# thiviyanT/torch-rgcn

Measured on AMD Instinct MI355X. Metric: edges/s/GPU (fwd+bwd) 2-layer RGCN, 1M nodes/10M edges/50 rels, h=16, higher is better.
Workload: dtype f32; 1 GPU; S1: N=1000000 nodes, E=10000000 base triples, R0=50 relations (layer R=101), M=21000000 messages/layer, hidden=16, 2 NC layers (horizontal, vertical), fwd+bwd, learnable X

## Files before the change

include/rgcn_hip.h:

```cpp
#ifndef RGCN_HIP_H
#define RGCN_HIP_H

#include <stdint.h>

#ifdef __cplusplus
extern "C" {
#endif

#define RGCN_API __attribute__((visibility("default")))

#define RGCN_OK 0
#define RGCN_EINVAL 1
#define RGCN_ENOMEM 2
#define RGCN_ERANGE 3
#define RGCN_EHIP 4
#define RGCN_EUNSUPPORTED 5

#define RGCN_CHUNK 16

RGCN_API const char *rgcn_version(void);
RGCN_API const char *rgcn_last_error(void);
RGCN_API const char *rgcn_csrc_sha(void);
RGCN_API int rgcn_poison_lds(void *stream);
RGCN_API int rgcn_set_option(const char *name, int32_t value);
RGCN_API int rgcn_get_option(const char *name, int32_t *value);


RGCN_API int rgcn_add_inverse_and_self_host(const int64_t *triples, int64_t E, int64_t N, int64_t R0,
                                            int64_t *out);

RGCN_API int rgcn_lp_augment_host(const int64_t *triples, int64_t E, int64_t N, int64_t R0,
                                  const uint8_t *keep, int64_t *out, int64_t *M_out, int64_t *n_self);

RGCN_API int rgcn_edge_norm_host(const int64_t *triples_plus, int64_t M, int64_t N, int64_t R, int vertical,
                                 int64_t n_swap, int64_t i_tail, float *val);

RGCN_API int rgcn_plan_count_host(const int32_t *dst, const int32_t *rel, int64_t M, int64_t n_dst, int32_t R,
                                  int32_t tile_rows, int32_t max_item_chunks, int64_t *m_pad,
                                  int64_t *n_chunks, int64_t *n_tiles, int64_t *n_items);
RGCN_API int rgcn_plan_fill_host(const int32_t *dst, const int32_t *src, const int32_t *rel, const float *val,
                                 int64_t M, int64_t n_dst, int64_t n_src, int32_t R, int32_t tile_rows,
                                 int32_t max_item_chunks, int32_t *p_src, int32_t *p_dst, float *p_val,
                                 int32_t *p_perm, int32_t *chunk_rel, int32_t *tile_ptr, int32_t *items,
                                 int32_t *run_ptr, int32_t *p_pack);

#define RGCN_U_SHARED 1
#define RGCN_U_FIRST 2
RGCN_API int rgcn_plan_units_host(const int32_t *tile_ptr, int64_t n_tiles, int32_t max_unit_chunks,
                                  int32_t *units, int64_t *n_units, int64_t *n_split);

RGCN_API int rgcn_synthetic_triples_host(int64_t N, int64_t R0, int64_t E, uint64_t seed, int64_t *out);

RGCN_API int rgcn_edge_neighborhood_host(const int64_t *triples, int64_t E, int64_t N, int64_t sample_size,
                                         uint64_t seed, int64_t *picked_edges);

RGCN_API int rgcn_dev_split_triples(const int64_t *triples_plus, int64_t M, int64_t N, int32_t R, int32_t *s,
                                    int32_t *p, int32_t *o, int32_t *err_flag, void *stream);
RGCN_API int rgcn_dev_lp_expand(const int64_t *triples, int64_t E, int64_t N, int32_t R0, const uint8_t *keep,
                                int32_t *s, int32_t *p, int32_t *o, uint8_t *alive, int32_t *err_flag, void *stream);
RGCN_API int rgcn_dev_edge_norm(const int32_t *s, const int32_t *p, const int32_t *o, const uint8_t *alive, int64_t M,
                                int64_t N, int32_t R, int vertical, int64_t n_swap, int32_t *table, float *val,
                                void *stream);
RGCN_API int rgcn_dev_plan_count(const int32_t *dst, const int32_t *rel, const uint8_t *alive, int64_t M, int64_t n_dst,
                                 int32_t R, int32_t tile_rows, int32_t *cells, int32_t *bucket_cnt,
                                 int32_t *bucket_base, int32_t *scan_tmp, int32_t *cells_tmp, void *stream);
RGCN_API int rgcn_dev_plan_fill(const int32_t *dst, const int32_t *src, const int32_t *rel, const float *val,
                                const uint8_t *alive, int64_t M, int64_t n_dst, int64_t n_src, int32_t R,
                                int32_t tile_rows, int32_t *cells, const int32_t *bucket_cnt,
                                const int32_t *bucket_base, int32_t *p_src, int32_t *p_dst, float *p_val,
                                int32_t *p_pack, int32_t *chunk_rel, int32_t *tile_ptr, int32_t *run_ptr,
                                const int32_t *aux, int32_t *p_aux, int32_t *msg_slot, int64_t n_chunks,
                                void *stream);
RGCN_API int rgcn_dev_csr_pair(const int32_t *a, const int32_t *b, const int32_t *rel, const float *val, const uint8_t *alive,
                               int64_t M, int64_t N, int32_t *rowbuf, int32_t *scan_tmp, int32_t *e_other, int32_t *e_rel,
                               float *e_val, void *stream);
RGCN_API int rgcn_dev_plan_finish_nosync(const int32_t *bucket_base, int64_t n_tiles, int32_t R, int64_t m_pad_ub,
                                         int32_t *p_src, int32_t *p_dst, float *p_val, int32_t *p_pack, int32_t *p_aux,
                                         const int32_t *tile_ptr, int32_t *units, int32_t *items, int64_t n_items_ub,
                                         int32_t max_item_chunks, void *stream);

RGCN_API int rgcn_basis_aggregate_f32(const float *X, const float *comps, float *out, const int32_t *rowptr,
                                      const int32_t *p_src, const int32_t *p_rel, const float *p_val,
                                      int64_t n_rows, int32_t R, int32_t B, int32_t d, int32_t n_b_in,
                                      void *stream);
RGCN_API int rgcn_basis_dcomps_f32(const float *X, const float *D, float *dcomps, const int32_t *p_src,
                                   const int32_t *p_dst, const float *p_val, const int32_t *chunk_rel,
                                   const int32_t *items, int64_t n_items, int32_t R, int32_t B, int32_t d,
                                   int32_t n_copies, void *stream);
RGCN_API int rgcn_basis_dcomps_csr_supported(int32_t R, int32_t B, int32_t d);
RGCN_API int rgcn_basis_dcomps_csr_f32(const float *X, const float *D, float *dcomps, const int32_t *rowptr, const int32_t *p_src,
                                       const int32_t *p_rel, const float *p_val, int64_t n_rows, int32_t R, int32_t B, int32_t d,
                                       void *workspace, void *stream);
RGCN_API int64_t rgcn_basis_sum_workspace_bytes(int32_t R, int32_t B);


#define RGCN_F_RELU 1
#define RGCN_F_WPACKED 2
RGCN_API int rgcn_spmm_f32(const float *X, const float *W, const float *bias, float *out, const int32_t *p_src,
                           const int32_t *p_dst, const float *p_val, const int32_t *p_pack,
                           const int32_t *chunk_rel, const int32_t *units, int64_t n_units, int64_t n_split,
                           int32_t tile_rows, int64_t n_dst, int64_t n_src, int32_t R, int32_t d_in,
                           int32_t d_out, int32_t flags, void *stream);

RGCN_API int rgcn_pack_w16_f32(const float *W, float *Wp, int32_t R, void *stream);
RGCN_API int rgcn_pack_w_blocks_f32(const float *W, float *Wp, int32_t R, int32_t d_in, int32_t d_out, void *stream);

RGCN_API int rgcn_spmm_scatter_f32(const float *X, const float *Wp, float *Y, const int32_t *p_src,
                                   const float *p_val, const int32_t *p_pos, const int32_t *chunk_rel,
                                   const int32_t *items, int64_t n_items, int32_t d, void *stream);
RGCN_API int rgcn_segment_sum_f32(const float *Y, const int32_t *rowptr, const float *bias, float *out,
                                  int64_t n_rows, int32_t d, int32_t flags, void *stream);
RGCN_API int rgcn_segment_gather_sum_f32(const float *Y, const int32_t *perm, const int32_t *rowptr, const float *bias,
                                         float *out, int64_t n_rows, int32_t d, int32_t flags, void *stream);
RGCN_API int rgcn_segment_gather_sum_units_f32(const float *Y, const int32_t *perm, const int32_t *units, int64_t n_units,
                                               int64_t n_split, const float *bias, float *out, int64_t n_rows, int32_t d,
                                               int32_t flags, void *stream);

RGCN_API int rgcn_wgrad_f32(const float *X, const float *G, float *dW, const int32_t *p_src,
                            const int32_t *p_dst, const float *p_val, const int32_t *chunk_rel,
                            const int32_t *items, int64_t n_items, int64_t n_dst, int64_t n_src, int32_t R,
                            int32_t d_in, int32_t d_out, void *stream);

RGCN_API int rgcn_wgrad_tiled_f32(const float *X, const float *G, float *dW, const int32_t *p_src,
                                  const int32_t *p_dst, const float *p_val, const int32_t *chunk_rel,
                                  const int32_t *run_ptr, int64_t n_tiles, int32_t tile_rows, int64_t n_dst,
                                  int64_t n_src, int32_t R, int32_t d_in, int32_t d_out,
                                  int32_t tiles_per_item, void *stream);

#define RGCN_F_DW_ATOMIC 4
#define RGCN_F_TRANSPOSE_W 8
#define RGCN_F_DIAG4 16
#define RGCN_F_PARTIAL 32
#define RGCN_F_ACCUMULATE 64
RGCN_API int64_t rgcn_bwd_fused_scratch_floats(int64_t n_tiles, int32_t R);
RGCN_API int64_t rgcn_bwd_lean_slot_bytes(int64_t n_chunks);
RGCN_API int rgcn_bwd_lean_prepare_f32(const int32_t *p_pack, const int32_t *chunk_rel, int64_t n_chunks, void *slots, int32_t *hdr,
                                       void *stream);
RGCN_API int rgcn_bwd_lean_prepare_unpacked_f32(const int32_t *p_src, const int32_t *p_dst, const float *p_val, int32_t tile_rows,
                                                const int32_t *chunk_rel, int64_t n_chunks, void *slots, int32_t *hdr, void *stream);
RGCN_API int rgcn_bwd_lean_supported(int32_t tile_rows);
RGCN_API int rgcn_bwd_lean_f32(const float *G, const float *X, const float *Wt_packed, float *dX, float *dW, float *scratch,
                               const void *slots, const int32_t *hdr, const int32_t *run_ptr, int64_t n_tiles, int32_t tile_rows,
                               int64_t n_dst, int32_t R, int32_t flags, void *stream);
RGCN_API int32_t rgcn_bwd_blk_max_rows(int32_t R, int32_t flags);
RGCN_API int rgcn_bwd_blk_supported(int32_t tile_rows, int32_t R, int32_t flags);
RGCN_API int64_t rgcn_bwd_blk_rec_bytes(int64_t n_chunks);
RGCN_API int rgcn_bwd_blk_prepare_f32(const int32_t *p_pack, const int32_t *p_src, const int32_t *p_dst, const float *p_val,
                                      int32_t tile_rows, const int32_t *chunk_rel, int64_t n_chunks, void *rec, void *stream);
RGCN_API int rgcn_bwd_blk_f32(const float *G, const float *X, const float *Wt_packed, float *dX, float *dW, const void *rec,
                              const int32_t *run_ptr, int64_t n_tiles, int32_t tile_rows, int64_t n_dst, int32_t R, int32_t flags,
                              float *dbias, int64_t n_src, const int32_t *units, int64_t n_units, int64_t n_split, void *stream);
RGCN_API int32_t rgcn_bwd_own_waves(void);
RGCN_API int32_t rgcn_bwd_own_units(void);
RGCN_API int32_t rgcn_bwd_own_max_rows(void);
RGCN_API int rgcn_bwd_own_f32(const float *G, const float *X, const float *Wt_packed, float *dX, float *dW, const void *rec,
                              const int32_t *own_ptr, const int32_t *unit_rel, int64_t n_tiles, int32_t tile_rows, int64_t n_dst,
                              int32_t R, int32_t flags, float *dbias, int64_t n_src, void *stream);
RGCN_API int rgcn_bwd_own_bf16(const uint16_t *G, const uint16_t *X, const float *Wt_packed, uint16_t *dX, float *dW, const void *rec,
                               const int32_t *own_ptr, const int32_t *unit_rel, int64_t n_tiles, int32_t tile_rows, int64_t n_dst,
                               int32_t R, int32_t flags, float *dbias, int64_t n_src, void *stream);
RGCN_API int64_t rgcn_softwin_tmp_bytes(int64_t n);
RGCN_API int rgcn_softwin_order(const int32_t *dst, const int32_t *src, const int32_t *rel, const uint8_t *alive, int64_t M, int64_t n_dst,
                                int64_t n_src, int32_t R, int32_t tile_rows, uint64_t *keys, uint64_t *keys_sorted, int32_t *order,
                                int32_t *order_sorted, int32_t *bucket_cnt, int32_t *bucket_base, int32_t *bucket_first, void *tmp,
                                int64_t tmp_bytes, void *stream);
RGCN_API int rgcn_softwin_fill(const int32_t *dst, const int32_t *src, const float *val, const uint64_t *keys_sorted, const int32_t *order_sorted,
                               int64_t n_live, int64_t n_dst, int64_t n_src, int32_t R, int32_t tile_rows, const int32_t *bucket_base,
                               const int32_t *bucket_first, int64_t m_pad, const int32_t *parts, const int32_t *unit_base,
                               const int32_t *unit_owner, const int32_t *unit_local, int32_t own_waves, int32_t *s_src, int32_t *s_dst, float *s_val,
                               uint64_t *ckeys, uint64_t *ckeys_sorted, int32_t *cidx, int32_t *cidx_sorted, int32_t *crel, int32_t *group_cnt,
                               int32_t *p_src, int32_t *p_dst, float *p_val, int32_t *chunk_rel, int32_t *group_ptr, void *tmp, int64_t tmp_bytes,
                               void *stream);
RGCN_API int32_t rgcn_spmm_blk_max_rows(void);
RGCN_API int rgcn_spmm_blk_f32(const float *X, const float *W_packed, const float *bias, float *out, const void *rec,
                               const int32_t *run_ptr, int64_t n_tiles, int32_t tile_rows, int64_t n_dst, int32_t R, int32_t flags,
                               const int32_t *units, int64_t n_units, int64_t n_split, void *stream);
RGCN_API int rgcn_spmm_blk_bf16(const uint16_t *X, const float *W_packed, const float *bias, uint16_t *out, float *scratch, const void *rec,
                                const int32_t *run_ptr, int64_t n_tiles, int32_t tile_rows, int64_t n_dst, int64_t n_src, int32_t R,
                                int32_t flags, const int32_t *units, int64_t n_units, int64_t n_split, void *stream);
RGCN_API int rgcn_spmm_bf16(const uint16_t *X, const float *W_packed, const float *bias, uint16_t *out, float *scratch,
                            const int32_t *p_pack, const int32_t *chunk_rel, const int32_t *units, int64_t n_units, int64_t n_split,
                            int32_t tile_rows, int64_t n_dst, int64_t n_src, int32_t d_in, int32_t d_out, int32_t flags, void *stream);
RGCN_API int rgcn_wgrad_bf16(const uint16_t *X, const uint16_t *G, float *dW, const int32_t *p_src, const int32_t *p_dst,
                             const float *p_val, const int32_t *chunk_rel, const int32_t *items, int64_t n_items, int32_t R,
                             int32_t d_in, int32_t d_out, void *stream);
RGCN_API int rgcn_colsum_bf16(const uint16_t *G, float *db, float *scratch, int64_t n, int32_t d, void *stream);
RGCN_API int rgcn_bwd_scatter_dw_f32(const float *G, const float *X, const float *Wt_packed, float *Y, float *dW,
                                     const int32_t *p_src, const int32_t *p_dst, const float *p_val,
                                     const int32_t *chunk_rel, const int32_t *items, int64_t n_items, int32_t R, int32_t d,
                                     int32_t flags, void *stream);
RGCN_API int rgcn_pack_w16t_f32(const float *W, float *Wp, int32_t R, void *stream);
RGCN_API int rgcn_pack_w16_pair_f32(const float *W, float *Wp, float *Wtp, int32_t R, void *stream);

RGCN_API int rgcn_featureless_fwd_f32(const float *table, const float *bias, float *out, const int32_t *p_src,
                                      const int32_t *p_dst, const float *p_val, const int32_t *chunk_rel,
                                      const int32_t *units, int64_t n_units, int64_t n_split, int32_t tile_rows,
                                      int64_t n_dst, int64_t n_src, int32_t R, int32_t d_out, void *stream);

RGCN_API int rgcn_spmm_csr_d16_supported(int32_t R);
RGCN_API int rgcn_spmm_csr_d16_f32(const float *X, const float *W, const float *bias, float *out, const int32_t *units, int64_t n_units,
                                   int64_t n_split, const int32_t *e_src, const int32_t *e_rel, const float *e_val, int64_t n_rows,
                                   int32_t R, int32_t flags, void *stream);
RGCN_API int rgcn_block_supported(int32_t bi, int32_t bo);
RGCN_API int rgcn_block_spmm_f32(const float *X, const float *blocks, const float *bias, float *out, const int32_t *units,
                                 const int32_t *rowptr, int64_t n_units, int64_t n_split, const int32_t *e_src,
                                 const int32_t *e_rel, const float *e_val, int64_t n_rows, int32_t n_rel_blocks, int32_t nb,
                                 int32_t bi, int32_t bo, int32_t flags, void *stream);

RGCN_API int rgcn_block_wgrad_f32(const float *X, const float *G, float *dblocks, const int32_t *p_src, const int32_t *p_dst,
                                  const float *p_val, const int32_t *chunk_rel, const int32_t *items, int64_t n_items,
                                  int32_t n_rel_blocks, int32_t nb, int32_t bi, int32_t bo, void *stream);

RGCN_API int rgcn_diag_spmm_f32(const float *X, const float *w, const float *bias, float *out, const int32_t *units,
                                int64_t n_units, int64_t n_split, const int32_t *e_src, const int32_t *e_rel,
                                const float *e_val, int64_t n_rows, int32_t R, int32_t d, void *stream);

RGCN_API int rgcn_diag_wgrad_f32(const float *X, const float *G, float *dw, const int32_t *p_src, const int32_t *p_dst,
                                 const float *p_val, const int32_t *chunk_rel, const int32_t *items, int64_t n_items,
                                 int32_t R, int32_t d, void *stream);

RGCN_API int rgcn_featureless_wgrad_f32(const float *G, float *dtable, const int32_t *p_src,
                                        const int32_t *p_dst, const float *p_val, const int32_t *chunk_rel,
                                        int64_t n_chunks, int64_t n_dst, int64_t n_src, int32_t R,
                                        int32_t d_out, void *stream);
RGCN_API int rgcn_featureless_csr_fwd_f32(const float *table, const float *bias, float *out, const int32_t *units, int64_t n_units,
                                          int64_t n_split, const int32_t *e_src, const int32_t *e_rel, const float *e_val,
                                          int64_t n_rows, int64_t n_src, int32_t R, int32_t d, int32_t relu, void *stream);
RGCN_API int rgcn_featureless_csr_wgrad_f32(const float *G, float *dtable, const int32_t *rowptr, const int32_t *e_src,
                                            const int32_t *e_rel, const float *e_val, int64_t n_entries, int64_t n_rows, int64_t n_src,
                                            int32_t R, int32_t d, void *stream);

RGCN_API int64_t rgcn_colsum_scratch_floats(int64_t n, int32_t d);
RGCN_API int rgcn_colsum_f32(const float *G, float *db, float *scratch, int64_t n, int32_t d, void *stream);

RGCN_API int rgcn_fbasis_fwd_f32(const float *bases, const float *comps, float *Y, const int32_t *e_rel,
                                 const float *e_val, const int32_t *units, int64_t n_units, int64_t n_nodes,
                                 int32_t R, int32_t B, int32_t d, int32_t basis_major, void *stream);
RGCN_API int rgcn_fbasis_bwd_f32(const float *bases, const float *comps, const float *G, float *dbases, float *T,
                                 const int32_t *e_dst, const int32_t *e_rel, const float *e_val,
                                 const int32_t *units, int64_t n_units, int64_t n_split, int64_t n_nodes, int32_t R,
                                 int32_t B, int32_t d, int32_t basis_major, void *stream);
RGCN_API int rgcn_fbasis_small_supported(int32_t R, int32_t B, int32_t d);
RGCN_API int rgcn_fbasis_small_bwd_f32(const float *G, const float *table, const float *comps, float *dbases, float *dcomps,
                                       const int32_t *rowptr, const int32_t *p_src, const int32_t *p_rel, const float *p_val,
                                       int64_t n_rows, int32_t R, int32_t B, int32_t d, int32_t basis_major, void *stream);
RGCN_API int rgcn_fbasis_bwd_dc_supported(int32_t R, int32_t B, int32_t d);
RGCN_API int rgcn_fbasis_bwd_dc_f32(const float *bases, const float *comps, const float *G, float *dbases, float *dcomps,
                                    const int32_t *e_dst, const int32_t *e_rel, const float *e_val, const int32_t *units,
                                    int64_t n_units, int64_t n_split, int64_t n_nodes, int32_t R, int32_t B, int32_t d,
                                    int32_t basis_major, void *stream);
RGCN_API int rgcn_gather_rows_sum_f32(const float *Y, const int32_t *perm, const int32_t *units, int64_t n_units,
                                      int64_t n_split, const float *bias, float *out, int64_t n_rows, int32_t w,
                                      int32_t relu, void *stream);

RGCN_API int rgcn_fbasis_tile_supported(int32_t R, int32_t B, int32_t d, int64_t n_nodes);
RGCN_API int rgcn_fbasis_tile_ystride(int32_t d);
RGCN_API int rgcn_fbasis_tile_fwd_f32(const float *bases, const float *comps, float *Y, const int32_t *rowptr, const int32_t *e_rel,
                                      const float *e_val, int64_t n_messages, int64_t n_nodes, int32_t R, int32_t B, int32_t d,
                                      int32_t mode, void *stream);
RGCN_API int rgcn_gather_rows_sum4_f32(const float *Y, int32_t ys, const int32_t *perm, const int32_t *units, int64_t n_units,
                                       int64_t n_split, const float *bias, float *out, int64_t n_rows, int32_t w, int32_t out_stride,
                                       int32_t relu, void *stream);
RGCN_API int rgcn_fbasis_tile_bwd_f32(const float *bases, const float *comps, const float *G, int32_t g_stride, float *dbases, float *dcomps,
                                      const int32_t *rowptr, const int32_t *e_dst, const int32_t *e_rel, const float *e_val,
                                      int64_t n_messages, int64_t n_nodes, int32_t R, int32_t B, int32_t d, int32_t mode, void *stream);
RGCN_API int rgcn_fbasis_tile_bwd_fused_gn(int32_t R, int32_t B, int32_t d, int64_t n_nodes);

RGCN_API int rgcn_fbasis_tile_fwd_bf16(const uint16_t *bases, const float *comps, float *Y, const int32_t *rowptr, const int32_t *e_rel,
                                       const float *e_val, int64_t n_messages, int64_t n_nodes, int32_t R, int32_t B, int32_t d,
                                       int32_t mode, void *stream);
RGCN_API int rgcn_gather_rows_sum4_bf16(const float *Y, int32_t ys, const int32_t *perm, const int32_t *units, int64_t n_units,
                                        int64_t n_split, const float *bias, uint16_t *out, float *scratch, int64_t n_rows, int32_t w,
                                        int32_t out_stride, int32_t relu, void *stream);
RGCN_API int rgcn_fbasis_tile_bwd_bf16(const uint16_t *bases, const float *comps, const uint16_t *G, int32_t g_stride, uint16_t *dbases,
                                       float *dcomps, const int32_t *rowptr, const int32_t *e_dst, const int32_t *e_rel, const float *e_val,
                                       int64_t n_messages, int64_t n_nodes, int32_t R, int32_t B, int32_t d, int32_t mode, void *stream);

RGCN_API int rgcn_ce_head_f32(const float *logits, const int32_t *row_label, const int32_t *lab_rows, float *loss, float *dlogits,
                              int64_t N, int32_t C, int32_t ld, int32_t n_lab, void *stream);

RGCN_API int rgcn_bce_head_workspace_bytes(void);
RGCN_API int rgcn_bce_head_f32(const float *scores, const float *labels, float *loss, float *dscores, void *workspace, int64_t T,
                               void *stream);

RGCN_API int rgcn_resize3_f32(const float *src, float *dst, int64_t A, int32_t B, int32_t C, int32_t Bd, int32_t Cd, const float *src1,
                              float *dst1, int32_t n1, int32_t n1d, void *stream);

#define RGCN_G_TRANS_A 1
#define RGCN_G_TRANS_B 2
RGCN_API int64_t rgcn_gemm_scratch_floats(int64_t M, int64_t N, int64_t K, int32_t split_k);
RGCN_API int rgcn_gemm_f32(const float *A, const float *B, const float *bias, float *C, float *scratch, int64_t M,
                           int64_t N, int64_t K, int64_t lda, int64_t ldb, int64_t ldc, int32_t flags, int32_t split_k,
                           void *stream);

RGCN_API int rgcn_rel_rows_f32(const float *Xs, const float *W, float *Y, const int32_t *p_src, const float *p_val,
                               const int32_t *chunk_rel, const int32_t *items, int64_t n_items, int32_t R, int32_t d_in,
                               int32_t d_out, void *stream);
RGCN_API int rgcn_rel_wgrad_f32(const float *Xs, const float *G, float *dW, const int32_t *p_src, const int32_t *p_dst,
                                const float *p_val, const int32_t *chunk_rel, const int32_t *items, int64_t n_items,
                                int32_t R, int32_t d_in, int32_t d_out, void *stream);
RGCN_API int rgcn_segment_gather_sum_wide_f32(const float *Y, const int32_t *perm, const int32_t *rowptr, const float *bias,
                                              float *out, int64_t n_rows, int32_t d, int32_t flags, void *stream);

RGCN_API int rgcn_distmult_fwd_f32(const int64_t *triples, int64_t T, const float *nodes, const float *rel,
                                   const float *sbias, const float *pbias, const float *obias, float *scores,
                                   int64_t n_nodes, int32_t n_rel, int32_t d, int32_t *err_flag, int32_t *rank_counts,
                                   int32_t *ranks, void *stream);
RGCN_API int rgcn_distmult_csr_place(const int64_t *triples, int64_t T, int64_t N, int32_t n_rel, const int32_t *ranks,
                                     int32_t *rank_counts, int32_t *scan_tmp, const float *gs, int32_t *entries, void *stream);
RGCN_API int rgcn_distmult_bwd_f32(const int64_t *triples, int64_t T, const float *nodes, const float *rel,
                                   const float *gs, float *dnodes, float *drel, float *dsbias, float *dpbias,
                                   float *dobias, int64_t n_nodes, int32_t n_rel, int32_t d, void *stream);
RGCN_API int rgcn_distmult_bwd_nodes_f32(const int32_t *rowptr_s, const int32_t *rowptr_o, const int32_t *entries, const float *nodes,
                                         const float *rel, float *dnodes, int64_t n_nodes, int32_t d, void *stream);

RGCN_API int rgcn_distmult_bwd_all_supported(int32_t n_rel, int32_t d);
RGCN_API int rgcn_distmult_bwd_all_f32(const int32_t *rowptr_s, const int32_t *rowptr_o, const int32_t *entries, const float *nodes,
                                       const float *rel, float *dnodes, float *drel, float *dsbias, float *dpbias, float *dobias,
                                       int64_t n_nodes, int32_t n_rel, int32_t d, void *stream);

RGCN_API int rgcn_distmult_score_all_f32(const int64_t *batch, int64_t Q, int32_t head, const float *nodes,
                                         const float *rel, const float *sbias, const float *pbias,
                                         const float *obias, float *qvec, float *qbias, float *scores,
                                         int64_t n_nodes, int32_t n_rel, int32_t d, void *stream);
RGCN_API int rgcn_rank_filter_f32(float *scores, int64_t Q, int64_t n_nodes, const int32_t *filt_q,
                                  const int32_t *filt_n, int64_t F, void *stream);
RGCN_API int rgcn_rank_count_f32(const float *scores, const int64_t *batch, int64_t Q, int32_t head,
                                 int64_t n_nodes, int64_t *greater, int64_t *ties, void *stream);

#ifdef __cplusplus
}
#endif
#endif
```

torch-rgcn_amd/csrc/rgcn_bwd_blk.hip:

```cpp
#include <stdlib.h>
#include <string.h>

#include <algorithm>

#include "rgcn_device.h"

namespace {

constexpr int BLK_NW = 16;
#ifndef RGCN_BLK_FWD_U
#define RGCN_BLK_FWD_U 1
#endif
constexpr int BLK_FWD_U = RGCN_BLK_FWD_U;
#ifndef RGCN_BLK_FWD_NW
#define RGCN_BLK_FWD_NW 16
#endif
constexpr int BLK_FWD_NW = RGCN_BLK_FWD_NW;
constexpr int BLK_FWD_TQS = 16 / BLK_FWD_NW;
#ifndef RGCN_BLK_BWD_U
#define RGCN_BLK_BWD_U 3
#endif
constexpr int BLK_BWD_U = RGCN_BLK_BWD_U;
constexpr int BLK_REC = 176;
constexpr int BLK_REC_ROWS = 128;
// ... 63 lines not shown
  extern __shared__ __attribute__((aligned(16))) char lds[];
  const int tid = threadIdx.x;
  const int wave = __builtin_amdgcn_readfirstlane(tid >> 6), lane = tid & 63;
  const unsigned xt_off = (unsigned)tile_rows * 128u;
  const unsigned xs_off = (unsigned)tile_rows * 192u;
  float4 *dxz = reinterpret_cast<float4 *>(lds);
  const double2 *dxd2 = reinterpret_cast<const double2 *>(lds);
  float4 *xt4 = reinterpret_cast<float4 *>(lds + xt_off);
  float *xs = reinterpret_cast<float *>(lds + xs_off) + wave * BW_SCR2;
  constexpr int DWR = DIAG4 ? 64 : 256;
  float *dwl = reinterpret_cast<float *>(lds + xs_off) + NW * BW_SCR2;
  int *ctl = reinterpret_cast<int *>(dwl + (size_t)R * DWR);
  int *dirty = ctl + 4;

  auto unit_of = [&](int u) {
    if (units) return units[u];
    return int4{u, run_ptr[(size_t)u * (R + 1)], run_ptr[(size_t)u * (R + 1) + R], 0};
  };
  int un = blockIdx.x;
  int4 unit = unit_of(un);
  int t = __builtin_amdgcn_readfirstlane(unit.x);
  int row0 = t * tile_rows;
  int nrows = min(tile_rows, n_dst - row0);
  int c0 = __builtin_amdgcn_readfirstlane(unit.y);
  int c1 = __builtin_amdgcn_readfirstlane(unit.z);
  int shared = __builtin_amdgcn_readfirstlane(unit.w) & RGCN_U_SHARED;
  int nq = (c1 - c0 + U - 1) / U;
  auto static_quads = [](int n) { return max(1, min(4, (3 * n) / (4 * BLK_NW))); };
  int ns = static_quads(nq);
  float4 gs = make_float4(0.f, 0.f, 0.f, 0.f);
  const long long g_n4 = dbias ? (long long)n_src * 4 : 0, g_step = (long long)gridDim.x * NT;
  long long g_i = (long long)blockIdx.x * NT + tid;
  {
#pragma unroll
    for (int q = 0; q < TQ; ++q) {
      const int idx = tid + q * NT;
      if (idx < tile_rows * 4) {
        float4 x0 = make_float4(0.f, 0.f, 0.f, 0.f);
        if (idx < nrows * 4) x0 = reinterpret_cast<const float4 *>(X + (size_t)row0 * 16)[idx];
        xt4[idx] = x0;
      }
    }
    for (int i = tid; i < tile_rows * 8; i += NT) dxz[i] = make_float4(0.f, 0.f, 0.f, 0.f);
    for (int i = tid; i < R * (DWR / 4); i += NT) reinterpret_cast<float4 *>(dwl)[i] = make_float4(0.f, 0.f, 0.f, 0.f);
    for (int i = tid; i < R + 4; i += NT) ctl[i] = i == 0 ? NW * (ns + 1) : 0;
  }
  __syncthreads();

  const int m = lane & 15, k = lane >> 4;
  const unsigned kofs = (unsigned)k << 4;
  const unsigned dx_lane = (unsigned)m * 8u;
  const unsigned xrd = xt_off + (unsigned)m * 4u;
  float *xs_wr = xs + m * 16 + 4 * ((k + (m >> 2)) & 3);
  const float *xs_rd = xs + (4 * k) * 16 + 4 * (((m >> 2) + k) & 3) + (m & 3);
  const unsigned slot_lane = (unsigned)m * 8u;
  const unsigned rows_lane = (unsigned)BLK_REC_ROWS + (unsigned)k * 8u;
  const unsigned w_lane = (unsigned)lane * 16u;

  f32x4 hold = f32x4{0.f, 0.f, 0.f, 0.f};
  int cur_r = -1;
  auto flush_hold = [&]() {
    if (cur_r >= 0 && (ABL & 4)) {
      *reinterpret_cast<f32x4 *>(dwl + (size_t)cur_r * 256 + lane * 4) = hold;
    } else if (cur_r >= 0) {
      if (DIAG4) {
        if ((m >> 2) == k) lds_cas_add4(dwl + (size_t)cur_r * 64 + (4 * k + (m & 3)) * 4, hold);
      } else {
        lds_cas_add4(dwl + (size_t)cur_r * 256 + lane * 4, hold);
      }
      if (lane == 0) lds_st(dirty + cur_r, 1);
    }
  };

  uint2 sl_n[U], rw_n[U];
  int hd_n[U];
  auto request_idx = [&](int c, int last) {
#pragma unroll
    for (int j = 0; j < U; ++j) {
      const int cc = min(c + j, last);
      const char *r = rec + (size_t)cc * BLK_REC;
      sl_n[j] = *reinterpret_cast<const uint2 *>(r + slot_lane);
      rw_n[j] = *reinterpret_cast<const uint2 *>(r + rows_lane);
      hd_n[j] = *reinterpret_cast<const int *>(r + BLK_REC_HDR);
    }
  };
  int q_cur = wave * ns, q_nxt = 1 < ns ? wave * ns + 1 : NW * ns + wave, q_pos = 2;
  if (q_cur < nq) request_idx(c0 + q_cur * U, c1 - 1);
  BLK_DBG(const long long dbg_t0 = BLK_T(); long long dbg_wait = 0; long long dbg_epi = 0; long long dbg_ta = 0; long long dbg_tb = 0;)

  for (;;) {
    const int last = c1 - 1;
    while (q_cur < nq) {
      const int c = c0 + q_cur * U;
      unsigned w0_[U];
      uint2 rw_[U];
      float v_[U];
      int hd_[U];
      float4 g_[U], w_[U];
#pragma unroll
      for (int j = 0; j < U; ++j) {
        w0_[j] = sl_n[j].x;
        rw_[j] = rw_n[j];
        v_[j] = (c + j <= last) ? __builtin_bit_cast(float, sl_n[j].y) : 0.f;
        hd_[j] = __builtin_amdgcn_readfirstlane(hd_n[j]);
      }
#pragma unroll
      for (int j = 0; j < U; ++j) asm volatile("" : "+v"(w0_[j]), "+v"(v_[j]));
      __builtin_amdgcn_sched_barrier(0);
#pragma unroll
      for (int j = 0; j < U; ++j) {
        const unsigned og = w0_[j] | kofs;
        g_[j] = *reinterpret_cast<const float4 *>(reinterpret_cast<const char *>(G) + og);
        w_[j] = *reinterpret_cast<const float4 *>(reinterpret_cast<const char *>(Wtp) + (size_t)hd_[j] * 1024 + w_lane);
      }
      __builtin_amdgcn_sched_barrier(0);
      if (q_nxt < nq) request_idx(c0 + q_nxt * U, last);
      int q_nn = q_pos < ns ? wave * ns + q_pos : NW * ns + wave;
      if (q_pos > ns && lane == 0) q_nn = __hip_atomic_fetch_add(ctl, 1, __ATOMIC_RELAXED, __HIP_MEMORY_SCOPE_WORKGROUP);
      ++q_pos;
      __builtin_amdgcn_sched_barrier(0);
      if (ABL & 16) {
#pragma unroll
        for (int j = 0; j < U; ++j) asm volatile("" :: "v"(g_[j].x), "v"(g_[j].y), "v"(g_[j].z), "v"(g_[j].w), "v"(w_[j].x), "v"(w_[j].w), "v"(rw_[j].x), "v"(rw_[j].y), "v"(v_[j]));
        q_cur = q_nxt;
        q_nxt = __builtin_amdgcn_readfirstlane(q_nn);
        continue;
      }
      f32x4 sc[U], acc[U];
#pragma unroll
      for (int j = 0; j < U; ++j) {
        sc[j] = f32x4{g_[j].x * v_[j], g_[j].y * v_[j], g_[j].z * v_[j], g_[j].w * v_[j]};
        acc[j] = f32x4{0.f, 0.f, 0.f, 0.f};
      }
#pragma unroll
      for (int j = 0; j < U; ++j) acc[j] = __builtin_amdgcn_mfma_f32_16x16x4f32(sc[j][0], w_[j].x, acc[j], 0, 0, 0);
#pragma unroll
      for (int j = 0; j < U; ++j) acc[j] = __builtin_amdgcn_mfma_f32_16x16x4f32(sc[j][1], w_[j].y, acc[j], 0, 0, 0);
#pragma unroll
      for (int j = 0; j < U; ++j) acc[j] = __builtin_amdgcn_mfma_f32_16x16x4f32(sc[j][2], w_[j].z, acc[j], 0, 0, 0);
#pragma unroll
      for (int j = 0; j < U; ++j) acc[j] = __builtin_amdgcn_mfma_f32_16x16x4f32(sc[j][3], w_[j].w, acc[j], 0, 0, 0);
      unsigned ro[U][4];
#pragma unroll
      for (int j = 0; j < U; ++j) {
        ro[j][0] = rw_[j].x & 0xFFFFu;
        ro[j][1] = rw_[j].x >> 16;
        ro[j][2] = rw_[j].y & 0xFFFFu;
        ro[j][3] = rw_[j].y >> 16;
      }
      if (!(ABL & 2)) {
        f32x4 aw[U];
#pragma unroll
        for (int h = 0; h < U; h += 2) {
          float bv[2][4], av[2][4];
#pragma unroll
          for (int jj = 0; jj < 2; ++jj) {
            const int j = h + jj;
            if (j >= U) break;
            if (ABL & 32) {
#pragma unroll
              for (int t4 = 0; t4 < 4; ++t4) { bv[jj][t4] = sc[j][t4]; av[jj][t4] = __builtin_bit_cast(float, ro[j][t4]); }
            } else {
            asm volatile("" ::: "memory");
            *reinterpret_cast<f32x4 *>(xs_wr) = sc[j];
            asm volatile("" ::: "memory");
#pragma unroll
            for (int t4 = 0; t4 < 4; ++t4) bv[jj][t4] = xs_rd[16 * t4];
#pragma unroll
            for (int t4 = 0; t4 < 4; ++t4) av[jj][t4] = *reinterpret_cast<const float *>(lds + (xrd + ro[j][t4]));
            asm volatile("" ::: "memory");
            }
          }
#pragma unroll
          for (int jj = 0; jj < 2; ++jj)
            if (h + jj < U) aw[h + jj] = f32x4{0.f, 0.f, 0.f, 0.f};
#pragma unroll
          for (int t4 = 0; t4 < 4; ++t4)
#pragma unroll
            for (int jj = 0; jj < 2; ++jj)
              if (h + jj < U) aw[h + jj] = __builtin_amdgcn_mfma_f32_16x16x4f32(av[jj][t4], bv[jj][t4], aw[h + jj], 0, 0, 0);
        }
#pragma unroll
        for (int j = 0; j < U; ++j) {
          if (c + j > last) break;
          const int rj = hd_[j];
          if (rj != cur_r) {
            flush_hold();
            cur_r = rj;
            hold = aw[j];
          } else {
            hold += aw[j];
          }
        }
      }
      if (ABL & 8) {
#pragma unroll
        for (int j = 0; j < U; ++j) asm volatile("" :: "v"(acc[j][0]), "v"(acc[j][1]), "v"(acc[j][2]), "v"(acc[j][3]));
      } else {
#pragma unroll
        for (int j = 0; j < U; ++j)
#pragma unroll
          for (int e = 0; e < 4; ++e)
            __hip_atomic_fetch_add(static_cast<double *>(__builtin_assume_aligned(lds + (dx_lane + 2u * ro[j][e]), 8)), (double)acc[j][e], __ATOMIC_RELAXED,
                                   __HIP_MEMORY_SCOPE_WORKGROUP);
      }
      __builtin_amdgcn_sched_barrier(0);
      q_cur = q_nxt;
      q_nxt = __builtin_amdgcn_readfirstlane(q_nn);
    }
    flush_hold();
    cur_r = -1;
    const int unn = un + (int)gridDim.x;
    float4 xn[TQ];
#pragma unroll
    for (int q = 0; q < TQ; ++q) xn[q] = make_float4(0.f, 0.f, 0.f, 0.f);
    int c0n = 0, c1n = 0, nqn = 0, row0n = 0, nrn = 0, tn = 0, sharedn = 0, nsn = 1;
    if (unn < n_units) {
      const int4 unx = unit_of(unn);
      tn = __builtin_amdgcn_readfirstlane(unx.x);
      row0n = tn * tile_rows;
      nrn = min(tile_rows, n_dst - row0n);
      c0n = __builtin_amdgcn_readfirstlane(unx.y);
      c1n = __builtin_amdgcn_readfirstlane(unx.z);
      sharedn = __builtin_amdgcn_readfirstlane(unx.w) & RGCN_U_SHARED;
      nqn = (c1n - c0n + U - 1) / U;
      nsn = static_quads(nqn);
#pragma unroll
      for (int q = 0; q < TQ; ++q)
        if (tid + q * NT < nrn * 4) xn[q] = reinterpret_cast<const float4 *>(X + (size_t)row0n * 16)[tid + q * NT];
      if (wave * nsn < nqn) request_idx(c0n + wave * nsn * U, c1n - 1);
    }
    float4 gn = make_float4(0.f, 0.f, 0.f, 0.f);
    if (g_i < g_n4) gn = reinterpret_cast<const float4 *>(G)[g_i];
    g_i += g_step;
    BLK_DBG(dbg_ta = BLK_T();)
    lds_barrier();
    BLK_DBG(dbg_tb = BLK_T(); dbg_wait += dbg_tb - dbg_ta;)
    gs.x += gn.x; gs.y += gn.y; gs.z += gn.z; gs.w += gn.w;
#pragma unroll
    for (int q = 0; q < TQ; ++q) asm volatile("" : "+v"(xn[q].x), "+v"(xn[q].y), "+v"(xn[q].z), "+v"(xn[q].w));
#pragma unroll
    for (int q = 0; q < TQ; ++q) {
      const int idx = tid + q * NT;
      if (idx < nrows * 4) {
        const double2 d0 = dxd2[2 * idx], d1 = dxd2[2 * idx + 1];
        float4 a = make_float4((float)d0.x, (float)d0.y, (float)d1.x, (float)d1.y);
        if (RELU) {
          const float4 x = xt4[idx];
          a.x = x.x > 0.f ? a.x : 0.f; a.y = x.y > 0.f ? a.y : 0.f; a.z = x.z > 0.f ? a.z : 0.f; a.w = x.w > 0.f ? a.w : 0.f;
        }
        float4 *o = reinterpret_cast<float4 *>(dX + (size_t)row0 * 16) + idx;
        if (shared) {
          atomicAdd(&o->x, a.x); atomicAdd(&o->y, a.y); atomicAdd(&o->z, a.z); atomicAdd(&o->w, a.w);
        } else {
          *o = a;
        }
      }
    }
    if (unn >= n_units) break;
#pragma unroll
    for (int q = 0; q < TQ; ++q) {
      const int idx = tid + q * NT;
      if (idx < tile_rows * 4) {
        dxz[2 * idx] = make_float4(0.f, 0.f, 0.f, 0.f);
        dxz[2 * idx + 1] = make_float4(0.f, 0.f, 0.f, 0.f);
        xt4[idx] = xn[q];
      }
    }
    if (tid == 0) ctl[0] = NW * (nsn + 1);
    lds_barrier();
    BLK_DBG(dbg_epi += BLK_T() - dbg_tb;)
    un = unn; t = tn; row0 = row0n; nrows = nrn; c0 = c0n; c1 = c1n; nq = nqn; shared = sharedn;
    ns = nsn;
    q_cur = wave * ns; q_nxt = 1 < ns ? wave * ns + 1 : NW * ns + wave; q_pos = 2;
  }
  BLK_DBG(if (lane == 0 && blockIdx.x < 256) { unsigned long long *d = rgcn_blk_dbg + 4 * (blockIdx.x * BLK_NW + wave); d[0] += (unsigned long long)dbg_wait;
                                               d[1] += (unsigned long long)dbg_epi; d[2] += (unsigned long long)(BLK_T() - dbg_t0); d[3] += 1ull; })
  if (dbias) {
    for (; g_i < g_n4; g_i += g_step) {
      const float4 gn = reinterpret_cast<const float4 *>(G)[g_i];
      gs.x += gn.x; gs.y += gn.y; gs.z += gn.z; gs.w += gn.w;
    }
#pragma unroll
    for (int sft = 4; sft < 64; sft <<= 1) {
      gs.x += __shfl_xor(gs.x, sft); gs.y += __shfl_xor(gs.y, sft); gs.z += __shfl_xor(gs.z, sft); gs.w += __shfl_xor(gs.w, sft);
    }
    if (lane < 4) *reinterpret_cast<float4 *>(xs + 4 * lane) = gs;
    __syncthreads();
    if (tid < 16) {
      float a = 0.f;
      const float *all = reinterpret_cast<const float *>(lds + xs_off);
      for (int i = 0; i < NW; ++i) a += all[i * BW_SCR2 + tid];
      atomicAdd(dbias + tid, a);
    }
  }
  for (int i = tid; i < R * DWR; i += NT) {
    const int r = i / DWR, e = i & 3;
    const int ln = DIAG4 ? 16 * ((i >> 4) & 3) + 4 * ((i >> 4) & 3) + ((i >> 2) & 3) : (i >> 2) & 63;
    if (lds_ld(dirty + r)) atomicAdd(dWout + (size_t)r * 256 + (4 * (ln >> 4) + e) * 16 + (ln & 15), dwl[i]);
  }
}


template <bool RELU, int TQ, int BF = 0>
__global__ __launch_bounds__(64 * BLK_FWD_NW) void spmm_blk_d16_kernel(
    const float *__restrict__ X, const float *__restrict__ Wp, const float *__restrict__ bias, float *__restrict__ out,
    const char *__restrict__ rec, const int *__restrict__ run_ptr, int n_tiles, int tile_rows, int n_dst, int R,
    const int4 *__restrict__ units, int n_units) {
  constexpr int U = BLK_FWD_U, NW = BLK_FWD_NW, NT = 64 * BLK_FWD_NW;
  extern __shared__ __attribute__((aligned(16))) char lds[];
  const int tid = threadIdx.x;
  const int wave = __builtin_amdgcn_readfirstlane(tid >> 6), lane = tid & 63;
  float4 *tz = reinterpret_cast<float4 *>(lds);
  const double2 *td2 = reinterpret_cast<const double2 *>(lds);
  int *ctl = reinterpret_cast<int *>(lds + (size_t)tile_rows * 128u);

  auto unit_of = [&](int u) {
    if (units) return units[u];
    return int4{u, run_ptr[(size_t)u * (R + 1)], run_ptr[(size_t)u * (R + 1) + R], 0};
  };
  auto static_quads = [](int n) { return max(1, min(4, (3 * n) / (4 * BLK_FWD_NW))); };
  int un = blockIdx.x;
  int4 unit = unit_of(un);
  int row0 = __builtin_amdgcn_readfirstlane(unit.x) * tile_rows;
  int nrows = min(tile_rows, n_dst - row0);
  int c0 = __builtin_amdgcn_readfirstlane(unit.y), c1 = __builtin_amdgcn_readfirstlane(unit.z);
  int uflags = __builtin_amdgcn_readfirstlane(unit.w);
  int nq = (c1 - c0 + U - 1) / U;
  int ns = static_quads(nq);
  for (int i = tid; i < tile_rows * 8; i += NT) tz[i] = make_float4(0.f, 0.f, 0.f, 0.f);
  if (tid == 0) ctl[0] = NW * (ns + 1);
  __syncthreads();

  const int m = lane & 15, k = lane >> 4;
  const unsigned kofs = (unsigned)k << 4;
  const unsigned t_lane = (unsigned)m * 8u;
  const unsigned slot_lane = (unsigned)m * 8u;
  const unsigned rows_lane = (unsigned)BLK_REC_ROWS + (unsigned)k * 8u;
  const unsigned w_lane = (unsigned)lane * 16u;
  float4 bv = make_float4(0.f, 0.f, 0.f, 0.f);
  if (bias) bv = reinterpret_cast<const float4 *>(bias)[tid & 3];

  uint2 sl_n[U], rw_n[U];
  int hd_n[U];
  auto request_idx = [&](int c, int last) {
#pragma unroll
    for (int j = 0; j < U; ++j) {
      const int cc = min(c + j, last);
      const char *r = rec + (size_t)cc * BLK_REC;
      sl_n[j] = *reinterpret_cast<const uint2 *>(r + slot_lane);
      rw_n[j] = *reinterpret_cast<const uint2 *>(r + rows_lane);
      hd_n[j] = *reinterpret_cast<const int *>(r + BLK_REC_HDR);
    }
  };
  int q_cur = wave * ns, q_nxt = 1 < ns ? wave * ns + 1 : NW * ns + wave, q_pos = 2;
  if (q_cur < nq) request_idx(c0 + q_cur * U, c1 - 1);

  for (;;) {
    const int last = c1 - 1;
    while (q_cur < nq) {
      const int c = c0 + q_cur * U;
      unsigned w0_[U];
      uint2 rw_[U];
      float v_[U];
      int hd_[U];
      float4 g_[U], w_[U];
#pragma unroll
      for (int j = 0; j < U; ++j) {
        w0_[j] = sl_n[j].x;
        rw_[j] = rw_n[j];
        v_[j] = (c + j <= last) ? __builtin_bit_cast(float, sl_n[j].y) : 0.f;
        hd_[j] = __builtin_amdgcn_readfirstlane(hd_n[j]);
      }
#pragma unroll
      for (int j = 0; j < U; ++j) asm volatile("" : "+v"(w0_[j]), "+v"(v_[j]));
      __builtin_amdgcn_sched_barrier(0);
#pragma unroll
      for (int j = 0; j < U; ++j) {
        if constexpr ((BF & 1) != 0) {
          g_[j] = bf16x4_widen(*reinterpret_cast<const uint2 *>(reinterpret_cast<const char *>(X) + ((w0_[j] >> 1) | (kofs >> 1))));
        } else {
          const unsigned og = w0_[j] | kofs;
          g_[j] = *reinterpret_cast<const float4 *>(reinterpret_cast<const char *>(X) + og);
        }
        w_[j] = *reinterpret_cast<const float4 *>(reinterpret_cast<const char *>(Wp) + (size_t)hd_[j] * 1024 + w_lane);
      }
      __builtin_amdgcn_sched_barrier(0);
      if (q_nxt < nq) request_idx(c0 + q_nxt * U, last);
      int q_nn = q_pos < ns ? wave * ns + q_pos : NW * ns + wave;
      if (q_pos > ns && lane == 0) q_nn = __hip_atomic_fetch_add(ctl, 1, __ATOMIC_RELAXED, __HIP_MEMORY_SCOPE_WORKGROUP);
      ++q_pos;
      __builtin_amdgcn_sched_barrier(0);
      f32x4 sc[U], acc[U];
#pragma unroll
      for (int j = 0; j < U; ++j) {
        sc[j] = f32x4{g_[j].x * v_[j], g_[j].y * v_[j], g_[j].z * v_[j], g_[j].w * v_[j]};
        acc[j] = f32x4{0.f, 0.f, 0.f, 0.f};
      }
#pragma unroll
      for (int j = 0; j < U; ++j) acc[j] = __builtin_amdgcn_mfma_f32_16x16x4f32(sc[j][0], w_[j].x, acc[j], 0, 0, 0);
#pragma unroll
      for (int j = 0; j < U; ++j) acc[j] = __builtin_amdgcn_mfma_f32_16x16x4f32(sc[j][1], w_[j].y, acc[j], 0, 0, 0);
#pragma unroll
      for (int j = 0; j < U; ++j) acc[j] = __builtin_amdgcn_mfma_f32_16x16x4f32(sc[j][2], w_[j].z, acc[j], 0, 0, 0);
#pragma unroll
      for (int j = 0; j < U; ++j) acc[j] = __builtin_amdgcn_mfma_f32_16x16x4f32(sc[j][3], w_[j].w, acc[j], 0, 0, 0);
#pragma unroll
      for (int j = 0; j < U; ++j) {
        const unsigned ro[4] = {rw_[j].x & 0xFFFFu, rw_[j].x >> 16, rw_[j].y & 0xFFFFu, rw_[j].y >> 16};
#pragma unroll
        for (int e = 0; e < 4; ++e)
          __hip_atomic_fetch_add(static_cast<double *>(__builtin_assume_aligned(lds + (t_lane + 2u * ro[e]), 8)), (double)acc[j][e], __ATOMIC_RELAXED,
                                 __HIP_MEMORY_SCOPE_WORKGROUP);
      }
      __builtin_amdgcn_sched_barrier(0);
      q_cur = q_nxt;
      q_nxt = __builtin_amdgcn_readfirstlane(q_nn);
    }
    const int unn = un + (int)gridDim.x;
    int c0n = 0, c1n = 0, nqn = 0, row0n = 0, nrn = 0, flagsn = 0, nsn = 1;
    if (unn < n_units) {
      const int4 unx = unit_of(unn);
      row0n = __builtin_amdgcn_readfirstlane(unx.x) * tile_rows;
      nrn = min(tile_rows, n_dst - row0n);
      c0n = __builtin_amdgcn_readfirstlane(unx.y);
      c1n = __builtin_amdgcn_readfirstlane(unx.z);
      flagsn = __builtin_amdgcn_readfirstlane(unx.w);
      nqn = (c1n - c0n + U - 1) / U;
      nsn = static_quads(nqn);
      if (wave * nsn < nqn) request_idx(c0n + wave * nsn * U, c1n - 1);
    }
    lds_barrier();
#pragma unroll
    for (int j = 0; j < U; ++j) asm volatile("" : "+v"(sl_n[j].x), "+v"(sl_n[j].y), "+v"(rw_n[j].x), "+v"(rw_n[j].y), "+v"(hd_n[j]));
    const bool shared = uflags & RGCN_U_SHARED;
    const bool with_bias = !shared || (uflags & RGCN_U_FIRST);
#pragma unroll
    for (int q = 0; q < TQ; ++q) {
      const int idx = tid + q * NT;
      if (idx < nrows * 4) {
        const double2 d0 = td2[2 * idx], d1 = td2[2 * idx + 1];
        float4 a = make_float4((float)d0.x, (float)d0.y, (float)d1.x, (float)d1.y);
        if (with_bias) { a.x += bv.x; a.y += bv.y; a.z += bv.z; a.w += bv.w; }
        if constexpr ((BF & 2) != 0) {
          if (RELU) { a.x = fmaxf(a.x, 0.f); a.y = fmaxf(a.y, 0.f); a.z = fmaxf(a.z, 0.f); a.w = fmaxf(a.w, 0.f); }
          reinterpret_cast<uint2 *>(out)[(size_t)row0 * 4 + idx] = bf16x4_round(a);
        } else {
        float4 *o = reinterpret_cast<float4 *>(out + (size_t)row0 * 16) + idx;
        if (shared) {
          atomicAdd(&o->x, a.x); atomicAdd(&o->y, a.y); atomicAdd(&o->z, a.z); atomicAdd(&o->w, a.w);
        } else {
          if (RELU) { a.x = fmaxf(a.x, 0.f); a.y = fmaxf(a.y, 0.f); a.z = fmaxf(a.z, 0.f); a.w = fmaxf(a.w, 0.f); }
          *o = a;
        }
        }
      }
    }
    if (unn >= n_units) break;
#pragma unroll
    for (int q = 0; q < TQ; ++q) {
      const int idx = tid + q * NT;
      if (idx < tile_rows * 4) {
        tz[2 * idx] = make_float4(0.f, 0.f, 0.f, 0.f);
        tz[2 * idx + 1] = make_float4(0.f, 0.f, 0.f, 0.f);
      }
    }
    if (tid == 0) ctl[0] = NW * (nsn + 1);
    lds_barrier();
    un = unn; row0 = row0n; nrows = nrn; c0 = c0n; c1 = c1n; nq = nqn; uflags = flagsn;
    ns = nsn;
    q_cur = wave * ns; q_nxt = 1 < ns ? wave * ns + 1 : NW * ns + wave; q_pos = 2;
  }
}


}

extern "C" int64_t rgcn_bwd_blk_rec_bytes(int64_t n_chunks) { return n_chunks * (int64_t)BLK_REC; }

extern "C" int rgcn_bwd_blk_prepare_f32(const int32_t *p_pack, const int32_t *p_src, const int32_t *p_dst, const float *p_val,
                                        int32_t tile_rows, const int32_t *chunk_rel, int64_t n_chunks, void *rec, void *stream) {
  if (n_chunks < 0 || tile_rows <= 0 || tile_rows > 1023 || (!p_pack && n_chunks && (!p_src || !p_dst || !p_val)) ||
      (p_pack && tile_rows > 255) || (n_chunks && (!chunk_rel || !rec))) {
    rgcn_set_error("bwd_blk_prepare: bad argument");
    return RGCN_EINVAL;
  }
  if (!n_chunks) return RGCN_OK;
  const long long n = n_chunks * RGCN_CHUNK;
  hipLaunchKernelGGL(bwd_blk_prep_kernel, dim3((unsigned)((n + WG - 1) / WG)), dim3(WG), 0, (hipStream_t)stream,
                     reinterpret_cast<const int2 *>(p_pack), p_src, p_dst, p_val, tile_rows, chunk_rel, static_cast<char *>(rec),
                     (long long)n_chunks);
  HIP_TRY(hipGetLastError());
  return RGCN_OK;
}

extern "C" int32_t rgcn_bwd_blk_max_rows(int32_t R, int32_t flags) {
  if (R <= 0 || R >= 0xFFFF) return 0;
  const long long fixed = (long long)bwd_blk_lds(R, (flags & RGCN_F_DIAG4) != 0, 0);
  const long long rows = (BLK_LDS_MAX - fixed) / 192;
  return (int32_t)std::max<long long>(0, std::min<long long>(512, rows));
}

extern "C" int rgcn_bwd_blk_supported(int32_t tile_rows, int32_t R, int32_t flags) {
  return tile_rows > 0 && tile_rows <= rgcn_bwd_blk_max_rows(R, flags);
}

extern "C" int rgcn_bwd_blk_f32(const float *G, const float *X, const float *Wt_packed, float *dX, float *dW, const void *rec,
                                const int32_t *run_ptr, int64_t n_tiles, int32_t tile_rows, int64_t n_dst, int32_t R, int32_t flags,
                                float *dbias, int64_t n_src, const int32_t *units, int64_t n_units, int64_t n_split, void *stream) {
  if (!G || !X || !Wt_packed || !dX || !dW || !rec || !run_ptr || n_tiles <= 0 || tile_rows <= 0 || n_dst <= 0 || R <= 0 ||
      (units && ((n_units < n_tiles && !(flags & (RGCN_F_ACCUMULATE | RGCN_F_PARTIAL))) || n_split < 0 || n_units > INT32_MAX || n_units <= 0))) {
    rgcn_set_error("bwd_blk: bad argument");
    return RGCN_EINVAL;
  }
  if ((flags & (RGCN_F_ACCUMULATE | RGCN_F_PARTIAL)) && (!units || n_split)) { rgcn_set_error("bwd_blk: a slab (RGCN_F_PARTIAL / RGCN_F_ACCUMULATE) is an explicit list of whole-tile work units"); return RGCN_EINVAL; }
  if (!units) { n_units = n_tiles; n_split = 0; }
  if (!rgcn_bwd_blk_supported(tile_rows, R, flags)) {
    rgcn_set_error("bwd_blk: tile_rows = %d / R = %d: 192 bytes per row + 16 KiB + R KiB (R / 4 KiB with RGCN_F_DIAG4) of LDS do not fit (at most %d rows)",
                   tile_rows, R, rgcn_bwd_blk_max_rows(R, flags));
    return RGCN_EUNSUPPORTED;
  }
  const bool relu = (flags & RGCN_F_RELU) != 0, diag4 = (flags & RGCN_F_DIAG4) != 0;
  const int tq = tile_rows > 256 ? 2 : 1;
  const size_t lds = bwd_blk_lds(R, diag4, tile_rows);
  hipStream_t st = (hipStream_t)stream;
  static int n_cu = 0;
  if (!n_cu) {
    int dev = 0, v = 0;
    HIP_TRY(hipGetDevice(&dev));
    HIP_TRY(hipDeviceGetAttribute(&v, hipDeviceAttributeMultiprocessorCount, dev));
    n_cu = v > 0 ? v : 256;
  }
  if (dbias && (n_src <= 0 || n_src >= (int64_t(1) << 29))) { rgcn_set_error("bwd_blk: dbias needs 0 < n_src < 2^29"); return RGCN_EINVAL; }
  if (flags & RGCN_F_ACCUMULATE) {
  } else if (dbias == dW + (size_t)R * 256) {
    HIP_TRY(zero_async(dW, ((size_t)R * 256 + 16) * sizeof(float), st));
  } else {
    HIP_TRY(zero_async(dW, (size_t)R * 256 * sizeof(float), st));
    if (dbias) HIP_TRY(zero_async(dbias, 16 * sizeof(float), st));
  }
  if (n_split) HIP_TRY(zero_async(dX, (size_t)n_dst * 16 * sizeof(float), st));
  const unsigned n_blocks = (unsigned)std::min<int64_t>(n_units, n_cu);
  auto launch = [&](auto kern, bool &raised) -> hipError_t {
    if (lds > 64 * 1024 && !raised) {
      hipError_t e = hipFuncSetAttribute(reinterpret_cast<const void *>(kern), hipFuncAttributeMaxDynamicSharedMemorySize, BLK_LDS_MAX);
      if (e != hipSuccess) return e;
      raised = true;
    }
    hipLaunchKernelGGL(kern, dim3(n_blocks), dim3(64 * BLK_NW), lds, st, G, X, Wt_packed, dX, dW, static_cast<const char *>(rec), run_ptr,
                       (int)n_tiles, tile_rows, (int)n_dst, R, dbias, (int)n_src, reinterpret_cast<const int4 *>(units), (int)n_units);
    return hipGetLastError();
  };
#ifdef RGCN_ABLATIONS
  {
    const int ABLV = rgcn_option_value(RGCN_OPT_BWD_ABL);
    static bool a0 = false, a1 = false, a2 = false, a3 = false, a4 = false, a5 = false, a6 = false, a7 = false;
    if (tq != 1 || diag4) { rgcn_set_error("bwd_blk (ablation library): only dense weights on tiles of up to 256 rows"); return RGCN_EUNSUPPORTED; }
    if (ABLV == 2) HIP_TRY(launch(bwd_blk_d16_kernel<false, false, 1, 2>, a0));
    else if (ABLV == 8) HIP_TRY(launch(bwd_blk_d16_kernel<false, false, 1, 8>, a1));
    else if (ABLV == 10) HIP_TRY(launch(bwd_blk_d16_kernel<false, false, 1, 10>, a2));
    else if (ABLV == 16) HIP_TRY(launch(bwd_blk_d16_kernel<false, false, 1, 16>, a3));
    else if (ABLV == 4) HIP_TRY(launch(bwd_blk_d16_kernel<false, false, 1, 4>, a4));
    else if (ABLV == 32) HIP_TRY(launch(bwd_blk_d16_kernel<false, false, 1, 32>, a5));
    else if (ABLV == 36) HIP_TRY(launch(bwd_blk_d16_kernel<false, false, 1, 36>, a6));
    else HIP_TRY(launch(bwd_blk_d16_kernel<false, false, 1, 0>, a7));
    return RGCN_OK;
  }
#else
  static bool r0 = false, r1 = false, r2 = false, r3 = false, r4 = false, r5 = false, r6 = false, r7 = false;
  if (tq == 2 && diag4 && relu) HIP_TRY(launch(bwd_blk_d16_kernel<true, true, 2>, r0));
  else if (tq == 2 && diag4) HIP_TRY(launch(bwd_blk_d16_kernel<false, true, 2>, r1));
  else if (tq == 2 && relu) HIP_TRY(launch(bwd_blk_d16_kernel<true, false, 2>, r2));
  else if (tq == 2) HIP_TRY(launch(bwd_blk_d16_kernel<false, false, 2>, r3));
  else if (diag4 && relu) HIP_TRY(launch(bwd_blk_d16_kernel<true, true, 1>, r4));
  else if (diag4) HIP_TRY(launch(bwd_blk_d16_kernel<false, true, 1>, r5));
  else if (relu) HIP_TRY(launch(bwd_blk_d16_kernel<true, false, 1>, r6));
  else HIP_TRY(launch(bwd_blk_d16_kernel<false, false, 1>, r7));
#endif
  return RGCN_OK;
}

extern "C" int32_t rgcn_spmm_blk_max_rows(void) { return 1023; }

extern "C" int rgcn_spmm_blk_f32(const float *X, const float *W_packed, const float *bias, float *out, const void *rec,
                                 const int32_t *run_ptr, int64_t n_tiles, int32_t tile_rows, int64_t n_dst, int32_t R, int32_t flags,
                                 const int32_t *units, int64_t n_units, int64_t n_split, void *stream) {
  if (!X || !W_packed || !out || !rec || !run_ptr || n_tiles <= 0 || tile_rows <= 0 || n_dst <= 0 || R <= 0 || n_dst > INT32_MAX ||
      (units && (n_units < n_tiles || n_split < 0 || n_units > INT32_MAX))) {
    rgcn_set_error("spmm_blk: bad argument");
    return RGCN_EINVAL;
  }
  if (tile_rows > rgcn_spmm_blk_max_rows()) { rgcn_set_error("spmm_blk: tiles of at most %d rows (got %d)", rgcn_spmm_blk_max_rows(), tile_rows); return RGCN_EUNSUPPORTED; }
  if (!units) { n_units = n_tiles; n_split = 0; }
  const bool relu = (flags & RGCN_F_RELU) != 0;
  if (relu && n_split) { rgcn_set_error("spmm_blk: relu in the epilogue needs tiles that are not cut into shared pieces"); return RGCN_EUNSUPPORTED; }
  hipStream_t st = (hipStream_t)stream;
  static int n_cu = 0;
  if (!n_cu) {
    int dev = 0, v = 0;
    HIP_TRY(hipGetDevice(&dev));
    HIP_TRY(hipDeviceGetAttribute(&v, hipDeviceAttributeMultiprocessorCount, dev));
    n_cu = v > 0 ? v : 256;
  }
  if (n_split) HIP_TRY(zero_async(out, (size_t)n_dst * 16 * sizeof(float), st));
  const size_t lds = (size_t)tile_rows * 128 + 64;
  const unsigned n_blocks = (unsigned)std::min<int64_t>(n_units, n_cu);
  auto launch = [&](auto kern, bool &raised) -> hipError_t {
    if (lds > 64 * 1024 && !raised) {
      hipError_t e = hipFuncSetAttribute(reinterpret_cast<const void *>(kern), hipFuncAttributeMaxDynamicSharedMemorySize, BLK_LDS_MAX);
      if (e != hipSuccess) return e;
      raised = true;
    }
    hipLaunchKernelGGL(kern, dim3(n_blocks), dim3(64 * BLK_FWD_NW), lds, st, X, W_packed, bias, out, static_cast<const char *>(rec), run_ptr, (int)n_tiles,
                       tile_rows, (int)n_dst, R, reinterpret_cast<const int4 *>(units), (int)n_units);
    return hipGetLastError();
  };
  static bool r[8] = {false, false, false, false, false, false, false, false};
  const int tq = (tile_rows + 255) / 256;
  if (relu) {
    if (tq == 1) HIP_TRY(launch(spmm_blk_d16_kernel<true, 1 * BLK_FWD_TQS>, r[0]));
    else if (tq == 2) HIP_TRY(launch(spmm_blk_d16_kernel<true, 2 * BLK_FWD_TQS>, r[1]));
    else if (tq == 3) HIP_TRY(launch(spmm_blk_d16_kernel<true, 3 * BLK_FWD_TQS>, r[2]));
    else HIP_TRY(launch(spmm_blk_d16_kernel<true, 4 * BLK_FWD_TQS>, r[3]));
  } else {
    if (tq == 1) HIP_TRY(launch(spmm_blk_d16_kernel<false, 1 * BLK_FWD_TQS>, r[4]));
    else if (tq == 2) HIP_TRY(launch(spmm_blk_d16_kernel<false, 2 * BLK_FWD_TQS>, r[5]));
    else if (tq == 3) HIP_TRY(launch(spmm_blk_d16_kernel<false, 3 * BLK_FWD_TQS>, r[6]));
    else HIP_TRY(launch(spmm_blk_d16_kernel<false, 4 * BLK_FWD_TQS>, r[7]));
  }
  return RGCN_OK;
}

namespace {
__global__ __launch_bounds__(WG) void round_rows_bf16_kernel(const float4 *__restrict__ src, uint2 *__restrict__ dst, long long n4) {
  for (long long i = (long long)blockIdx.x * WG + threadIdx.x; i < n4; i += (long long)gridDim.x * WG) dst[i] = bf16x4_round(src[i]);
}
}

extern "C" int rgcn_spmm_blk_bf16(const uint16_t *X, const float *W_packed, const float *bias, uint16_t *out, float *scratch, const void *rec,
                                  const int32_t *run_ptr, int64_t n_tiles, int32_t tile_rows, int64_t n_dst, int64_t n_src, int32_t R,
                                  int32_t flags, const int32_t *units, int64_t n_units, int64_t n_split, void *stream) {
  if (!X || !W_packed || !out || !rec || !run_ptr || n_tiles <= 0 || tile_rows <= 0 || n_dst <= 0 || R <= 0 || n_dst > INT32_MAX ||
      n_src <= 0 || n_src >= (int64_t(1) << 26) || (units && (n_units < n_tiles || n_split < 0 || n_units > INT32_MAX))) {
    rgcn_set_error("spmm_blk_bf16: bad argument (the records address source rows as src << 6 in 32 bits: n_src < 2^26)");
    return RGCN_EINVAL;
  }
  if (tile_rows > rgcn_spmm_blk_max_rows()) { rgcn_set_error("spmm_blk_bf16: tiles of at most %d rows (got %d)", rgcn_spmm_blk_max_rows(), tile_rows); return RGCN_EUNSUPPORTED; }
  if (!units) { n_units = n_tiles; n_split = 0; }
  const bool relu = (flags & RGCN_F_RELU) != 0;
  if (relu && n_split) { rgcn_set_error("spmm_blk_bf16: relu in the epilogue needs tiles that are not cut into shared pieces"); return RGCN_EUNSUPPORTED; }
  if (n_split && !scratch) { rgcn_set_error("spmm_blk_bf16: a plan with hub pieces needs the fp32 scratch (n_dst x 16 floats)"); return RGCN_EINVAL; }
  hipStream_t st = (hipStream_t)stream;
  static int n_cu = 0;
  if (!n_cu) {
    int dev = 0, v = 0;
    HIP_TRY(hipGetDevice(&dev));
    HIP_TRY(hipDeviceGetAttribute(&v, hipDeviceAttributeMultiprocessorCount, dev));
    n_cu = v > 0 ? v : 256;
  }
  float *dst32 = n_split ? scratch : reinterpret_cast<float *>(out);
  if (n_split) HIP_TRY(zero_async(scratch, (size_t)n_dst * 16 * sizeof(float), st));
  const size_t lds = (size_t)tile_rows * 128 + 64;
  const unsigned n_blocks = (unsigned)std::min<int64_t>(n_units, n_cu);
  const float *Xf = reinterpret_cast<const float *>(X);
  auto launch = [&](auto kern, bool &raised) -> hipError_t {
    if (lds > 64 * 1024 && !raised) {
      hipError_t e = hipFuncSetAttribute(reinterpret_cast<const void *>(kern), hipFuncAttributeMaxDynamicSharedMemorySize, BLK_LDS_MAX);
      if (e != hipSuccess) return e;
      raised = true;
    }
    hipLaunchKernelGGL(kern, dim3(n_blocks), dim3(64 * BLK_FWD_NW), lds, st, Xf, W_packed, bias, dst32, static_cast<const char *>(rec), run_ptr,
                       (int)n_tiles, tile_rows, (int)n_dst, R, reinterpret_cast<const int4 *>(units), (int)n_units);
    return hipGetLastError();
  };
  static bool r[12] = {false, false, false, false, false, false, false, false, false, false, false, false};
  const int tq = (tile_rows + 255) / 256;
  if (n_split) {
    if (tq == 1) HIP_TRY(launch(spmm_blk_d16_kernel<false, 1 * BLK_FWD_TQS, 1>, r[0]));
    else if (tq == 2) HIP_TRY(launch(spmm_blk_d16_kernel<false, 2 * BLK_FWD_TQS, 1>, r[1]));
    else if (tq == 3) HIP_TRY(launch(spmm_blk_d16_kernel<false, 3 * BLK_FWD_TQS, 1>, r[2]));
    else HIP_TRY(launch(spmm_blk_d16_kernel<false, 4 * BLK_FWD_TQS, 1>, r[3]));
    const long long n4 = n_dst * 4;
    hipLaunchKernelGGL(round_rows_bf16_kernel, dim3((unsigned)std::min<long long>((n4 + WG - 1) / WG, 4096)), dim3(WG), 0, st,
                       reinterpret_cast<const float4 *>(scratch), reinterpret_cast<uint2 *>(out), n4);
    HIP_TRY(hipGetLastError());
  } else if (relu) {
    if (tq == 1) HIP_TRY(launch(spmm_blk_d16_kernel<true, 1 * BLK_FWD_TQS, 3>, r[4]));
    else if (tq == 2) HIP_TRY(launch(spmm_blk_d16_kernel<true, 2 * BLK_FWD_TQS, 3>, r[5]));
    else if (tq == 3) HIP_TRY(launch(spmm_blk_d16_kernel<true, 3 * BLK_FWD_TQS, 3>, r[6]));
    else HIP_TRY(launch(spmm_blk_d16_kernel<true, 4 * BLK_FWD_TQS, 3>, r[7]));
  } else {
    if (tq == 1) HIP_TRY(launch(spmm_blk_d16_kernel<false, 1 * BLK_FWD_TQS, 3>, r[8]));
    else if (tq == 2) HIP_TRY(launch(spmm_blk_d16_kernel<false, 2 * BLK_FWD_TQS, 3>, r[9]));
    else if (tq == 3) HIP_TRY(launch(spmm_blk_d16_kernel<false, 3 * BLK_FWD_TQS, 3>, r[10]));
    else HIP_TRY(launch(spmm_blk_d16_kernel<false, 4 * BLK_FWD_TQS, 3>, r[11]));
  }
  return RGCN_OK;
}

#ifdef RGCN_ABLATIONS
extern "C" __attribute__((visibility("default"))) int rgcn_blk_debug_read(unsigned long long *out4, int reset) {
  static unsigned long long h[4 * BLK_DBG_WAVES];
  HIP_TRY(hipDeviceSynchronize());
  HIP_TRY(hipMemcpyFromSymbol(h, HIP_SYMBOL(rgcn_blk_dbg), sizeof(h)));
  for (int i = 0; i < 4; ++i) out4[i] = 0;
  for (int w = 0; w < BLK_DBG_WAVES; ++w)
    for (int i = 0; i < 4; ++i) out4[i] += h[4 * w + i];
  if (reset) { memset(h, 0, sizeof(h)); HIP_TRY(hipMemcpyToSymbol(HIP_SYMBOL(rgcn_blk_dbg), h, sizeof(h))); }
  return RGCN_OK;
}
#endif
```

torch-rgcn_amd/csrc/rgcn_bwd_own.hip:

```cpp
#include <stdlib.h>
#include <string.h>

#include <algorithm>

#include "rgcn_device.h"

namespace {

constexpr int OWN_REC = 176;
constexpr int OWN_REC_ROWS = 128;
constexpr int OWN_REC_HDR = 160;
constexpr int OWN_LDS_MAX = 160 * 1024;
#ifndef RGCN_OWN_NW
#define RGCN_OWN_NW 16
#define RGCN_OWN_K 8
#define RGCN_OWN_U 2
#endif
constexpr int OWN_NW = RGCN_OWN_NW;
constexpr int OWN_K = RGCN_OWN_K;
constexpr int OWN_U = RGCN_OWN_U;
constexpr int OWN_MAX_ROWS = (OWN_LDS_MAX - OWN_NW * BW_SCR2 * 4 - 64) / 192;

typedef float own_acc32 __attribute__((ext_vector_type(32)));

size_t bwd_own_lds(int rows) { return (size_t)rows * 192 + (size_t)OWN_NW * BW_SCR2 * 4 + 64; }

template <bool RELU, int NW, int K, int ABL = 0, bool BF = false>
__global__ __launch_bounds__(64 * NW) void bwd_own_d16_kernel(
    const float *__restrict__ G, const float *__restrict__ X, const float *__restrict__ Wtp, float *__restrict__ dX,
    float *__restrict__ dWout, const char *__restrict__ rec, const int *__restrict__ own_ptr, int n_tiles, int tile_rows, int n_dst,
    float *__restrict__ dbias, int n_src, const int *__restrict__ unit_rel) {
  constexpr int U = OWN_U, NT = 64 * NW;
  constexpr int TQ = (OWN_MAX_ROWS * 4 + NT - 1) / NT;
  static_assert(K <= 9, "8 indexed accumulators + 1");
  constexpr bool EXT = K == 9;
  extern __shared__ __attribute__((aligned(16))) char lds[];
  const int tid = threadIdx.x;
  const int wave = __builtin_amdgcn_readfirstlane(tid >> 6), lane = tid & 63;
  const unsigned xt_off = (unsigned)tile_rows * 128u;
  const unsigned xs_off = (unsigned)tile_rows * 192u;
  float4 *dxz = reinterpret_cast<float4 *>(lds);
  const double2 *dxd2 = reinterpret_cast<const double2 *>(lds);
  float4 *xt4 = reinterpret_cast<float4 *>(lds + xt_off);
  float *xs = reinterpret_cast<float *>(lds + xs_off) + wave * BW_SCR2;

  int t = blockIdx.x;
  int row0 = t * tile_rows;
  int nrows = min(tile_rows, n_dst - row0);
  int c0 = own_ptr[(size_t)t * NW + wave], c1 = own_ptr[(size_t)t * NW + wave + 1];
  c0 = __builtin_amdgcn_readfirstlane(c0);
  c1 = __builtin_amdgcn_readfirstlane(c1);
  float4 gs = make_float4(0.f, 0.f, 0.f, 0.f);
  const long long g_n4 = dbias ? (long long)n_src * 4 : 0, g_step = (long long)gridDim.x * NT;
  long long g_i = (long long)blockIdx.x * NT + tid;
#pragma unroll
  for (int q = 0; q < TQ; ++q) {
    const int idx = tid + q * NT;
    if (idx < tile_rows * 4) {
      float4 x0 = make_float4(0.f, 0.f, 0.f, 0.f);
      if (idx < nrows * 4) {
        if constexpr (BF) x0 = bf16x4_widen(reinterpret_cast<const uint2 *>(X)[(size_t)row0 * 4 + idx]);
        else x0 = reinterpret_cast<const float4 *>(X + (size_t)row0 * 16)[idx];
      }
      xt4[idx] = x0;
    }
  }
  for (int i = tid; i < tile_rows * 8; i += NT) dxz[i] = make_float4(0.f, 0.f, 0.f, 0.f);
  __syncthreads();

  const int m = lane & 15, k = lane >> 4;
  const unsigned kofs = (unsigned)k << 4;
  const unsigned dx_lane = (unsigned)m * 8u;
  const unsigned xrd = xt_off + (unsigned)m * 4u;
  float *xs_wr = xs + m * 16 + 4 * ((k + (m >> 2)) & 3);
  const float *xs_rd = xs + (4 * k) * 16 + 4 * (((m >> 2) + k) & 3) + (m & 3);
  const unsigned slot_lane = (unsigned)m * 8u;
  const unsigned rows_lane = (unsigned)OWN_REC_ROWS + (unsigned)k * 8u;
  const unsigned w_lane = (unsigned)lane * 16u;

  own_acc32 accs;
#pragma unroll
  for (int i = 0; i < 32; ++i) accs[i] = 0.f;
  f32x4 acc8 = f32x4{0.f, 0.f, 0.f, 0.f};

  uint2 sl_n[U], rw_n[U];
  int hd_n[U];
  auto request_idx = [&](int c, int last) {
#pragma unroll
    for (int j = 0; j < U; ++j) {
      const int cc = min(c + j, last);
      const char *r = rec + (size_t)cc * OWN_REC;
      sl_n[j] = *reinterpret_cast<const uint2 *>(r + slot_lane);
      rw_n[j] = *reinterpret_cast<const uint2 *>(r + rows_lane);
      hd_n[j] = *reinterpret_cast<const int *>(r + OWN_REC_HDR);
    }
  };
  if (c0 < c1) request_idx(c0, c1 - 1);

  for (;;) {
    const int last = c1 - 1;
    for (int c = c0; c < c1; c += U) {
      unsigned w0_[U];
      uint2 rw_[U];
      float v_[U];
      int hd_[U];
      float4 g_[U], w_[U];
#pragma unroll
      for (int j = 0; j < U; ++j) {
        w0_[j] = sl_n[j].x;
        rw_[j] = rw_n[j];
        v_[j] = (c + j <= last) ? __builtin_bit_cast(float, sl_n[j].y) : 0.f;
        hd_[j] = __builtin_amdgcn_readfirstlane(hd_n[j]);
      }
#pragma unroll
      for (int j = 0; j < U; ++j) asm volatile("" : "+v"(w0_[j]), "+v"(v_[j]));
      __builtin_amdgcn_sched_barrier(0);
#pragma unroll
      for (int j = 0; j < U; ++j) {
        if constexpr (BF) {
          g_[j] = bf16x4_widen(*reinterpret_cast<const uint2 *>(reinterpret_cast<const char *>(G) + ((w0_[j] >> 1) | (kofs >> 1))));
        } else {
          const unsigned og = w0_[j] | kofs;
          g_[j] = *reinterpret_cast<const float4 *>(reinterpret_cast<const char *>(G) + og);
        }
        w_[j] = *reinterpret_cast<const float4 *>(reinterpret_cast<const char *>(Wtp) + (size_t)(hd_[j] & 0xFFFF) * 1024 + w_lane);
      }
      __builtin_amdgcn_sched_barrier(0);
      if (c + U < c1) request_idx(c + U, last);
      __builtin_amdgcn_sched_barrier(0);
      if (ABL & 16) {
#pragma unroll
        for (int j = 0; j < U; ++j) asm volatile("" :: "v"(g_[j].x), "v"(g_[j].y), "v"(g_[j].z), "v"(g_[j].w), "v"(w_[j].x), "v"(w_[j].w), "v"(rw_[j].x), "v"(rw_[j].y), "v"(v_[j]));
        continue;
      }
      f32x4 sc[U], acc[U];
#pragma unroll
      for (int j = 0; j < U; ++j) {
        sc[j] = f32x4{g_[j].x * v_[j], g_[j].y * v_[j], g_[j].z * v_[j], g_[j].w * v_[j]};
        acc[j] = f32x4{0.f, 0.f, 0.f, 0.f};
      }
#pragma unroll
      for (int j = 0; j < U; ++j) acc[j] = __builtin_amdgcn_mfma_f32_16x16x4f32(sc[j][0], w_[j].x, acc[j], 0, 0, 0);
#pragma unroll
      for (int j = 0; j < U; ++j) acc[j] = __builtin_amdgcn_mfma_f32_16x16x4f32(sc[j][1], w_[j].y, acc[j], 0, 0, 0);
#pragma unroll
      for (int j = 0; j < U; ++j) acc[j] = __builtin_amdgcn_mfma_f32_16x16x4f32(sc[j][2], w_[j].z, acc[j], 0, 0, 0);
#pragma unroll
      for (int j = 0; j < U; ++j) acc[j] = __builtin_amdgcn_mfma_f32_16x16x4f32(sc[j][3], w_[j].w, acc[j], 0, 0, 0);
      unsigned ro[U][4];
#pragma unroll
      for (int j = 0; j < U; ++j) {
        ro[j][0] = rw_[j].x & 0xFFFFu;
        ro[j][1] = rw_[j].x >> 16;
        ro[j][2] = rw_[j].y & 0xFFFFu;
        ro[j][3] = rw_[j].y >> 16;
      }
#pragma unroll
      for (int h = 0; h < U && !(ABL & 2); h += 2) {
        constexpr int P = 2;
        float bv[P][4], av[P][4];
#pragma unroll
        for (int jj = 0; jj < P; ++jj) {
          const int j = h + jj;
          if (j >= U) break;
          asm volatile("" ::: "memory");
          *reinterpret_cast<f32x4 *>(xs_wr) = sc[j];
          asm volatile("" ::: "memory");
#pragma unroll
          for (int t4 = 0; t4 < 4; ++t4) bv[jj][t4] = xs_rd[16 * t4];
#pragma unroll
          for (int t4 = 0; t4 < 4; ++t4) av[jj][t4] = *reinterpret_cast<const float *>(lds + (xrd + ro[j][t4]));
          asm volatile("" ::: "memory");
        }
#pragma unroll
        for (int jj = 0; jj < P; ++jj) {
          if (h + jj >= U) break;
          const int lr = (ABL & 4) ? 0 : (int)((unsigned)hd_[h + jj] >> 16);
          const bool ext = EXT && lr >= 8;
          const int li = 4 * (lr & 7);
          const f32x4 in0 = f32x4{accs[li], accs[li + 1], accs[li + 2], accs[li + 3]};
          f32x4 aw = EXT ? f32x4{ext ? acc8[0] : in0[0], ext ? acc8[1] : in0[1], ext ? acc8[2] : in0[2], ext ? acc8[3] : in0[3]} : in0;
#pragma unroll
          for (int t4 = 0; t4 < 4; ++t4) aw = __builtin_amdgcn_mfma_f32_16x16x4f32(av[jj][t4], bv[jj][t4], aw, 0, 0, 0);
          accs[li] = ext ? in0[0] : aw[0];
          accs[li + 1] = ext ? in0[1] : aw[1];
          accs[li + 2] = ext ? in0[2] : aw[2];
          accs[li + 3] = ext ? in0[3] : aw[3];
          if (EXT) acc8 = f32x4{ext ? aw[0] : acc8[0], ext ? aw[1] : acc8[1], ext ? aw[2] : acc8[2], ext ? aw[3] : acc8[3]};
        }
      }
#pragma unroll
      for (int j = 0; j < U && !(ABL & 8); ++j)
#pragma unroll
        for (int e = 0; e < 4; ++e)
          __hip_atomic_fetch_add(static_cast<double *>(__builtin_assume_aligned(lds + (dx_lane + 2u * ro[j][e]), 8)), (double)acc[j][e], __ATOMIC_RELAXED,
                                 __HIP_MEMORY_SCOPE_WORKGROUP);
      __builtin_amdgcn_sched_barrier(0);
    }
    const int tn = t + (int)gridDim.x;
    int c0n = 0, c1n = 0, row0n = 0, nrn = 0;
    float4 xn[TQ];
#pragma unroll
    for (int q = 0; q < TQ; ++q) xn[q] = make_float4(0.f, 0.f, 0.f, 0.f);
    if (tn < n_tiles) {
      row0n = tn * tile_rows;
      nrn = min(tile_rows, n_dst - row0n);
      c0n = __builtin_amdgcn_readfirstlane(own_ptr[(size_t)tn * NW + wave]);
      c1n = __builtin_amdgcn_readfirstlane(own_ptr[(size_t)tn * NW + wave + 1]);
#pragma unroll
      for (int q = 0; q < TQ; ++q)
        if (tid + q * NT < nrn * 4) {
          if constexpr (BF) {
            const uint2 u = reinterpret_cast<const uint2 *>(X)[(size_t)row0n * 4 + tid + q * NT];
            xn[q] = make_float4(__uint_as_float(u.x), __uint_as_float(u.y), 0.f, 0.f);
          } else {
            xn[q] = reinterpret_cast<const float4 *>(X + (size_t)row0n * 16)[tid + q * NT];
          }
        }
      if (c0n < c1n) request_idx(c0n, c1n - 1);
    }
    float4 gn = make_float4(0.f, 0.f, 0.f, 0.f);
    if (g_i < g_n4) {
      if constexpr (BF) gn = bf16x4_widen(reinterpret_cast<const uint2 *>(G)[g_i]);
      else gn = reinterpret_cast<const float4 *>(G)[g_i];
    }
    g_i += g_step;
    lds_barrier();
    gs.x += gn.x; gs.y += gn.y; gs.z += gn.z; gs.w += gn.w;
#pragma unroll
    for (int q = 0; q < TQ; ++q) asm volatile("" : "+v"(xn[q].x), "+v"(xn[q].y), "+v"(xn[q].z), "+v"(xn[q].w));
#pragma unroll
    for (int q = 0; q < TQ; ++q) {
      const int idx = tid + q * NT;
      if (idx < nrows * 4) {
        const double2 d0 = dxd2[2 * idx], d1 = dxd2[2 * idx + 1];
        float4 a = make_float4((float)d0.x, (float)d0.y, (float)d1.x, (float)d1.y);
        if (RELU) {
          const float4 x = xt4[idx];
          a.x = x.x > 0.f ? a.x : 0.f; a.y = x.y > 0.f ? a.y : 0.f; a.z = x.z > 0.f ? a.z : 0.f; a.w = x.w > 0.f ? a.w : 0.f;
        }
        if constexpr (BF) reinterpret_cast<uint2 *>(dX)[(size_t)row0 * 4 + idx] = bf16x4_round(a);
        else reinterpret_cast<float4 *>(dX + (size_t)row0 * 16)[idx] = a;
      }
    }
    if (tn >= n_tiles) break;
#pragma unroll
    for (int q = 0; q < TQ; ++q) {
      const int idx = tid + q * NT;
      if (idx < tile_rows * 4) {
        dxz[2 * idx] = make_float4(0.f, 0.f, 0.f, 0.f);
        dxz[2 * idx + 1] = make_float4(0.f, 0.f, 0.f, 0.f);
        if constexpr (BF) xt4[idx] = bf16x4_widen(uint2{__float_as_uint(xn[q].x), __float_as_uint(xn[q].y)});
        else xt4[idx] = xn[q];
      }
    }
    lds_barrier();
    t = tn; row0 = row0n; nrows = nrn; c0 = c0n; c1 = c1n;
  }
  if (dbias) {
    for (; g_i < g_n4; g_i += g_step) {
      float4 gn;
      if constexpr (BF) gn = bf16x4_widen(reinterpret_cast<const uint2 *>(G)[g_i]);
      else gn = reinterpret_cast<const float4 *>(G)[g_i];
      gs.x += gn.x; gs.y += gn.y; gs.z += gn.z; gs.w += gn.w;
    }
#pragma unroll
    for (int sft = 4; sft < 64; sft <<= 1) {
      gs.x += __shfl_xor(gs.x, sft); gs.y += __shfl_xor(gs.y, sft); gs.z += __shfl_xor(gs.z, sft); gs.w += __shfl_xor(gs.w, sft);
    }
    __syncthreads();
    if (lane < 4) *reinterpret_cast<float4 *>(xs + 4 * lane) = gs;
    __syncthreads();
    if (tid < 16) {
      float a = 0.f;
      const float *all = reinterpret_cast<const float *>(lds + xs_off);
      for (int i = 0; i < NW; ++i) a += all[i * BW_SCR2 + tid];
      atomicAdd(dbias + tid, a);
    }
  }
#pragma unroll
  for (int li = 0; li < K; ++li) {
    const int r = __builtin_amdgcn_readfirstlane(unit_rel[wave * K + li]);
    if (r >= 0) {
      float *o = dWout + (size_t)r * 256 + (4 * k) * 16 + m;
      atomicAdd(o, li < 8 ? accs[(4 * li) & 31] : acc8[0]);
      atomicAdd(o + 16, li < 8 ? accs[(4 * li + 1) & 31] : acc8[1]);
      atomicAdd(o + 32, li < 8 ? accs[(4 * li + 2) & 31] : acc8[2]);
      atomicAdd(o + 48, li < 8 ? accs[(4 * li + 3) & 31] : acc8[3]);
    }
  }
}

}

extern "C" int32_t rgcn_bwd_own_waves(void) { return OWN_NW; }
extern "C" int32_t rgcn_bwd_own_units(void) { return OWN_NW * OWN_K; }
extern "C" int32_t rgcn_bwd_own_max_rows(void) { return OWN_MAX_ROWS; }

extern "C" int rgcn_bwd_own_f32(const float *G, const float *X, const float *Wt_packed, float *dX, float *dW, const void *rec,
                                const int32_t *own_ptr, const int32_t *unit_rel, int64_t n_tiles, int32_t tile_rows, int64_t n_dst,
                                int32_t R, int32_t flags, float *dbias, int64_t n_src, void *stream) {
  if (!G || !X || !Wt_packed || !dX || !dW || !rec || !own_ptr || !unit_rel || n_tiles <= 0 || tile_rows <= 0 || n_dst <= 0 || R <= 0 ||
      R > 0xFFFF || n_dst > INT32_MAX || n_tiles * (int64_t)OWN_NW >= INT32_MAX) {
    rgcn_set_error("bwd_own: bad argument");
    return RGCN_EINVAL;
  }
  if (tile_rows > rgcn_bwd_own_max_rows()) {
    rgcn_set_error("bwd_own: tiles of at most %d rows (got %d)", rgcn_bwd_own_max_rows(), tile_rows);
    return RGCN_EUNSUPPORTED;
  }
  if (dbias && (n_src <= 0 || n_src >= (int64_t(1) << 29))) { rgcn_set_error("bwd_own: dbias needs 0 < n_src < 2^29"); return RGCN_EINVAL; }
  hipStream_t st = (hipStream_t)stream;
  static int n_cu = 0;
  if (!n_cu) {
    int dev = 0, v = 0;
    HIP_TRY(hipGetDevice(&dev));
    HIP_TRY(hipDeviceGetAttribute(&v, hipDeviceAttributeMultiprocessorCount, dev));
    n_cu = v > 0 ? v : 256;
  }
  if (dbias == dW + (size_t)R * 256) {
    HIP_TRY(zero_async(dW, ((size_t)R * 256 + 16) * sizeof(float), st));
  } else {
    HIP_TRY(zero_async(dW, (size_t)R * 256 * sizeof(float), st));
    if (dbias) HIP_TRY(zero_async(dbias, 16 * sizeof(float), st));
  }
  const size_t lds = bwd_own_lds(tile_rows);
  const unsigned n_blocks = (unsigned)std::min<int64_t>(n_tiles, n_cu);
  auto launch = [&](auto kern, bool &raised) -> hipError_t {
    if (lds > 64 * 1024 && !raised) {
      hipError_t e = hipFuncSetAttribute(reinterpret_cast<const void *>(kern), hipFuncAttributeMaxDynamicSharedMemorySize, OWN_LDS_MAX);
      if (e != hipSuccess) return e;
      raised = true;
    }
    hipLaunchKernelGGL(kern, dim3(n_blocks), dim3(64 * OWN_NW), lds, st, G, X, Wt_packed, dX, dW, static_cast<const char *>(rec), own_ptr, (int)n_tiles,
                       tile_rows, (int)n_dst, dbias, (int)n_src, unit_rel);
    return hipGetLastError();
  };
#ifdef RGCN_ABLATIONS
  {
    const int ABLV = rgcn_option_value(RGCN_OPT_BWD_ABL);
    static bool a[8] = {false, false, false, false, false, false, false, false};
    if (ABLV == 2) HIP_TRY(launch(bwd_own_d16_kernel<false, OWN_NW, OWN_K, 2>, a[1]));
    else if (ABLV == 4) HIP_TRY(launch(bwd_own_d16_kernel<false, OWN_NW, OWN_K, 4>, a[3]));
    else if (ABLV == 8) HIP_TRY(launch(bwd_own_d16_kernel<false, OWN_NW, OWN_K, 8>, a[4]));
    else if (ABLV == 16) HIP_TRY(launch(bwd_own_d16_kernel<false, OWN_NW, OWN_K, 16>, a[5]));
    else if (ABLV == 6) HIP_TRY(launch(bwd_own_d16_kernel<false, OWN_NW, OWN_K, 6>, a[6]));
    else HIP_TRY(launch(bwd_own_d16_kernel<false, OWN_NW, OWN_K, 0>, a[7]));
    return RGCN_OK;
  }
#endif
  static bool r0 = false, r1 = false;
  if (flags & RGCN_F_RELU) HIP_TRY(launch(bwd_own_d16_kernel<true, OWN_NW, OWN_K>, r0));
  else HIP_TRY(launch(bwd_own_d16_kernel<false, OWN_NW, OWN_K>, r1));
  return RGCN_OK;
}

extern "C" int rgcn_bwd_own_bf16(const uint16_t *G, const uint16_t *X, const float *Wt_packed, uint16_t *dX, float *dW, const void *rec,
                                 const int32_t *own_ptr, const int32_t *unit_rel, int64_t n_tiles, int32_t tile_rows, int64_t n_dst,
                                 int32_t R, int32_t flags, float *dbias, int64_t n_src, void *stream) {
  if (!G || !X || !Wt_packed || !dX || !dW || !rec || !own_ptr || !unit_rel || n_tiles <= 0 || tile_rows <= 0 || n_dst <= 0 || R <= 0 ||
      R > 0xFFFF || n_dst > INT32_MAX || n_tiles * (int64_t)OWN_NW >= INT32_MAX || n_src <= 0 || n_src >= (int64_t(1) << 26) || flags != 0) {
    rgcn_set_error("bwd_own_bf16: bad argument (the records address G rows as src << 6 in 32 bits: n_src < 2^26; no flags)");
    return RGCN_EINVAL;
  }
  if (tile_rows > rgcn_bwd_own_max_rows()) {
    rgcn_set_error("bwd_own_bf16: tiles of at most %d rows (got %d)", rgcn_bwd_own_max_rows(), tile_rows);
    return RGCN_EUNSUPPORTED;
  }
  hipStream_t st = (hipStream_t)stream;
  static int n_cu = 0;
  if (!n_cu) {
    int dev = 0, v = 0;
    HIP_TRY(hipGetDevice(&dev));
    HIP_TRY(hipDeviceGetAttribute(&v, hipDeviceAttributeMultiprocessorCount, dev));
    n_cu = v > 0 ? v : 256;
  }
  if (dbias == dW + (size_t)R * 256) {
    HIP_TRY(zero_async(dW, ((size_t)R * 256 + 16) * sizeof(float), st));
  } else {
    HIP_TRY(zero_async(dW, (size_t)R * 256 * sizeof(float), st));
    if (dbias) HIP_TRY(zero_async(dbias, 16 * sizeof(float), st));
  }
  const size_t lds = bwd_own_lds(tile_rows);
  const unsigned n_blocks = (unsigned)std::min<int64_t>(n_tiles, n_cu);
  auto launch = [&](auto kern, bool &raised) -> hipError_t {
    if (lds > 64 * 1024 && !raised) {
      hipError_t e = hipFuncSetAttribute(reinterpret_cast<const void *>(kern), hipFuncAttributeMaxDynamicSharedMemorySize, OWN_LDS_MAX);
      if (e != hipSuccess) return e;
      raised = true;
    }
    hipLaunchKernelGGL(kern, dim3(n_blocks), dim3(64 * OWN_NW), lds, st, reinterpret_cast<const float *>(G), reinterpret_cast<const float *>(X),
                       Wt_packed, reinterpret_cast<float *>(dX), dW, static_cast<const char *>(rec), own_ptr, (int)n_tiles, tile_rows, (int)n_dst,
                       dbias, (int)n_src, unit_rel);
    return hipGetLastError();
  };
  static bool r1 = false;
  HIP_TRY(launch(bwd_own_d16_kernel<false, OWN_NW, OWN_K, 0, true>, r1));
  return RGCN_OK;
}
```

torch-rgcn_amd/torch_rgcn/_native.py:

```python
import ctypes
import threading
import os

import numpy as np
import torch

from . import routes

_LIB_PATH = os.environ.get("RGCN_HIP_LIB") or os.path.join(os.path.dirname(os.path.abspath(__file__)), "lib", "librgcn_hip.so")
_lib = None

OK, EINVAL, ENOMEM, ERANGE, EHIP, EUNSUPPORTED = range(6)
CHUNK = 16

c_i64, c_i32, c_int, c_void_p = ctypes.c_int64, ctypes.c_int32, ctypes.c_int, ctypes.c_void_p


class NativeLibraryError(RuntimeError):
    pass


def lib():
    global _lib
    if _lib is None:
        if not os.path.exists(_LIB_PATH):
            raise NativeLibraryError(
                f"{_LIB_PATH} not found: build it with `python -c 'import __graft_entry__ as g; g.build()'` "
                "(hipcc --offload-arch=gfx950). torch_rgcn has no CPU/eager fallback.")
        L = ctypes.CDLL(_LIB_PATH)
        L.rgcn_version.restype = ctypes.c_char_p
        L.rgcn_csrc_sha.restype = ctypes.c_char_p
        L.rgcn_bwd_fused_scratch_floats.restype = ctypes.c_int64
        L.rgcn_bwd_lean_slot_bytes.restype = ctypes.c_int64
        L.rgcn_bwd_blk_rec_bytes.restype = ctypes.c_int64
        L.rgcn_softwin_tmp_bytes.restype = ctypes.c_int64
        L.rgcn_colsum_scratch_floats.restype = ctypes.c_int64
        L.rgcn_gemm_scratch_floats.restype = ctypes.c_int64
        L.rgcn_basis_sum_workspace_bytes.restype = ctypes.c_int64
        L.rgcn_last_error.restype = ctypes.c_char_p
        _lib = L
        defaults = {}

        def sink(name, value):
            if name not in defaults:
                cur = ctypes.c_int32(0)
                L.rgcn_get_option(name.encode(), ctypes.byref(cur))
                defaults[name] = cur.value
            v = defaults[name] if value is None else value
            if L.rgcn_set_option(name.encode(), c_i32(v)) != OK:
                raise NativeLibraryError(f"route {name} = {v}: {L.rgcn_last_error().decode()}")
        routes._native_sink = sink
        routes.push_native()
    return _lib


def version():
    return lib().rgcn_version().decode()


def csrc_sha():
    return lib().rgcn_csrc_sha().decode()


def _check(rc, what):
    if rc == OK:
        return
    msg = lib().rgcn_last_error().decode()
    if rc in (ERANGE, EINVAL):
        raise AssertionError(f"{what}: {msg}")
    if rc == ENOMEM:
        raise MemoryError(f"{what}: {msg}")
    raise NativeLibraryError(f"{what}: {msg} (code {rc})")


def _np(a, dtype):
    return np.ascontiguousarray(a, dtype=dtype)


def _hp(a):
    return None if a is None else c_void_p(a.ctypes.data)


def _dp(t):
    return None if t is None else c_void_p(t.data_ptr())


_PROF = None
_PROF_ON = True


def profile_start():
    global _PROF, _PROF_ON
    _PROF, _PROF_ON = {}, True


def profile_enable(on):
    global _PROF_ON
    _PROF_ON = bool(on)


def profile_stop():
    global _PROF
    rec, _PROF = _PROF or {}, None
    torch.cuda.synchronize()
    return {k: [a.elapsed_time(b) for a, b in v] for k, v in rec.items()}


class _Timed:
    def __init__(self, name):
        self.name = name

    def __enter__(self):
        self.a = torch.cuda.Event(enable_timing=True)
        self.a.record()

    def __exit__(self, *exc):
        b = torch.cuda.Event(enable_timing=True)
        b.record()
        if _PROF is not None:
            _PROF.setdefault(self.name, []).append((self.a, b))


def _timed(name):
    return _NOCTX if (_PROF is None or not _PROF_ON or torch.cuda.is_current_stream_capturing()) else _Timed(name)


_RAW_STREAM = getattr(torch._C, "_cuda_getCurrentRawStream", None)


def _stream(device):
    if _RAW_STREAM is not None:
        idx = device.index
        return c_void_p(_RAW_STREAM(torch.cuda.current_device() if idx is None else idx))
    return c_void_p(torch.cuda.current_stream(device).cuda_stream)


class _NoCtx:
    def __enter__(self):
        return None

    def __exit__(self, *exc):
        return False


_NOCTX = _NoCtx()


def _on(device):
    idx = device.index
    if idx is None or idx == torch.cuda.current_device():
        return _NOCTX
    return torch.cuda.device(device)



def add_inverse_and_self_host(triples, num_nodes, num_rels):
    t = _np(triples, np.int64).reshape(-1, 3)
    out = np.empty((2 * t.shape[0] + num_nodes, 3), np.int64)
    _check(lib().rgcn_add_inverse_and_self_host(_hp(t), c_i64(t.shape[0]), c_i64(num_nodes), c_i64(num_rels),
                                                _hp(out)), "add_inverse_and_self")
    return out


def lp_augment_host(triples, num_nodes, num_rels, keep=None):
    t = _np(triples, np.int64).reshape(-1, 3)
    E = t.shape[0]
    out = np.empty((3 * E + num_nodes, 3), np.int64)
    k = None if keep is None else _np(keep, np.uint8)
    M, ns = c_i64(0), c_i64(0)
    _check(lib().rgcn_lp_augment_host(_hp(t), c_i64(E), c_i64(num_nodes), c_i64(num_rels), _hp(k), _hp(out),
                                      ctypes.byref(M), ctypes.byref(ns)), "lp_augment")
    return out[:M.value], ns.value


def edge_norm_host(triples_plus, num_nodes, num_rels, vertical, n_swap, i_tail):
    t = _np(triples_plus, np.int64).reshape(-1, 3)
    val = np.empty(t.shape[0], np.float32)
    _check(lib().rgcn_edge_norm_host(_hp(t), c_i64(t.shape[0]), c_i64(num_nodes), c_i64(num_rels),
                                     c_int(int(bool(vertical))), c_i64(n_swap), c_i64(i_tail), _hp(val)),
           "edge_norm")
    return val


def synthetic_triples_host(num_nodes, num_rels, num_edges, seed=0):
    out = np.empty((num_edges, 3), np.int64)
    _check(lib().rgcn_synthetic_triples_host(c_i64(num_nodes), c_i64(num_rels), c_i64(num_edges),
                                             ctypes.c_uint64(seed), _hp(out)), "synthetic_triples")
    return out


def edge_neighborhood_host(triples, num_nodes, sample_size, seed):
    triples = np.ascontiguousarray(triples, np.int64)
    out = np.empty(sample_size, np.int64)
    _check(lib().rgcn_edge_neighborhood_host(_hp(triples), c_i64(triples.shape[0]), c_i64(num_nodes),
                                             c_i64(sample_size), ctypes.c_uint64(seed), _hp(out)), "edge_neighborhood")
    return out


class HostPlan:
    __slots__ = ("src", "dst", "val", "perm", "chunk_rel", "tile_ptr", "items", "run_ptr", "pack", "units", "units_host", "_cache", "n_units", "n_split", "max_run_chunks", "n_dst", "n_src", "num_rels",
                 "tile_rows", "n_tiles", "n_chunks", "m_pad", "n_items", "n_messages")


def build_plan_host(dst, src, rel, val, n_dst, n_src, num_rels, tile_rows, max_item_chunks=64, want_perm=False,
                    want_runs=False, want_pack=False, max_unit_chunks=256):
    dst = _np(dst, np.int32)
    src = _np(src, np.int32)
    rel = _np(rel, np.int32)
    val = _np(val, np.float32)
    M = dst.shape[0]
    assert src.shape[0] == M and rel.shape[0] == M and val.shape[0] == M
    m_pad, n_chunks, n_tiles, n_items = c_i64(0), c_i64(0), c_i64(0), c_i64(0)
    L = lib()
    _check(L.rgcn_plan_count_host(_hp(dst), _hp(rel), c_i64(M), c_i64(n_dst), c_i32(num_rels), c_i32(tile_rows),
                                  c_i32(max_item_chunks), ctypes.byref(m_pad), ctypes.byref(n_chunks),
                                  ctypes.byref(n_tiles), ctypes.byref(n_items)), "plan_count")
    p = HostPlan()
    p.n_dst, p.n_src, p.num_rels, p.tile_rows = n_dst, n_src, num_rels, tile_rows
    p.n_tiles, p.n_chunks, p.m_pad, p.n_items, p.n_messages = n_tiles.value, n_chunks.value, m_pad.value, n_items.value, M
    p.src = np.empty(max(p.m_pad, 1), np.int32)
    p.dst = np.empty(max(p.m_pad, 1), np.int32)
    p.val = np.empty(max(p.m_pad, 1), np.float32)
    p.perm = np.empty(max(p.m_pad, 1), np.int32) if want_perm else None
    p.chunk_rel = np.empty(max(p.n_chunks, 1), np.int32)
    p.tile_ptr = np.zeros(p.n_tiles + 1, np.int32)
    p.items = np.empty((max(p.n_items, 1), 2), np.int32)
    p.run_ptr = np.zeros(max(p.n_tiles, 1) * (num_rels + 1), np.int32) if want_runs else None
    can_pack = want_pack and n_src < (1 << 24) and tile_rows <= 255
    p.pack = np.empty((max(p.m_pad, 1), 2), np.int32) if can_pack else None
    _check(L.rgcn_plan_fill_host(_hp(dst), _hp(src), _hp(rel), _hp(val), c_i64(M), c_i64(n_dst), c_i64(n_src),
                                 c_i32(num_rels), c_i32(tile_rows), c_i32(max_item_chunks), _hp(p.src), _hp(p.dst),
                                 _hp(p.val), _hp(p.perm), _hp(p.chunk_rel), _hp(p.tile_ptr), _hp(p.items),
                                 _hp(p.run_ptr), _hp(p.pack)), "plan_fill")
    nu, ns = c_i64(0), c_i64(0)
    _check(L.rgcn_plan_units_host(_hp(p.tile_ptr), c_i64(p.n_tiles), c_i32(max_unit_chunks), None, ctypes.byref(nu),
                                  ctypes.byref(ns)), "plan_units")
    p.n_units, p.n_split = nu.value, ns.value
    p.units = np.zeros((max(p.n_units, 1), 4), np.int32)
    p.units_host = p.units
    p._cache = {}
    _check(L.rgcn_plan_units_host(_hp(p.tile_ptr), c_i64(p.n_tiles), c_i32(max_unit_chunks), _hp(p.units),
                                  ctypes.byref(nu), ctypes.byref(ns)), "plan_units")
    if p.n_chunks:
        cr = p.chunk_rel[:p.n_chunks]
        edges = np.flatnonzero(np.diff(cr) != 0)
        runs = np.diff(np.concatenate(([-1], edges, [p.n_chunks - 1])))
        p.max_run_chunks = int(runs.max())
    else:
        p.max_run_chunks = 0
    return p



class DevicePlan:

    def __init__(self, hp, device):
        self.device = torch.device(device)
        up = lambda a: torch.from_numpy(a).to(self.device, non_blocking=False)
        self.src, self.dst, self.val = up(hp.src), up(hp.dst), up(hp.val)
        self.chunk_rel, self.tile_ptr, self.items = up(hp.chunk_rel), up(hp.tile_ptr), up(hp.items)
        self.run_ptr = None if hp.run_ptr is None else up(hp.run_ptr)
        self.pack = None if hp.pack is None else up(hp.pack)
        self.units = up(hp.units)
        self.units_host = hp.units
        for k in ("n_dst", "n_src", "num_rels", "tile_rows", "n_tiles", "n_chunks", "m_pad", "n_items", "n_messages",
                  "n_units", "n_split", "max_run_chunks"):
            setattr(self, k, getattr(hp, k))

    def nbytes(self):
        return sum(t.numel() * t.element_size() for t in (self.src, self.dst, self.val, self.chunk_rel,
                                                           self.tile_ptr, self.items))



def _i32(n, device):
    return torch.empty(max(int(n), 1), dtype=torch.int32, device=device)


_DEFERRED = []
_PINNED_FREE = []


def _deferred_mode():
    return routes.get("deferred_checks", "0") == "1"


def dev_check_err(err_flag, what, exc=AssertionError):
    if not _deferred_mode():
        if int(err_flag.item()):
            raise exc(f"{what}: node or relation index out of range")
        return
    if torch.cuda.is_current_stream_capturing():
        return
    host = _PINNED_FREE.pop() if _PINNED_FREE else torch.empty(1, dtype=torch.int32, pin_memory=True)
    host.copy_(err_flag[:1], non_blocking=True)
    ev = torch.cuda.Event()
    ev.record()
    _DEFERRED.append((ev, host, what, exc))
    check_deferred_errors(wait=False)


def check_deferred_errors(wait=True):
    keep = []
    err = None
    for ev, host, what, exc in _DEFERRED:
        if wait:
            ev.synchronize()
        if ev.query():
            if int(host[0]) and err is None:
                err = exc(f"{what}: node or relation index out of range")
            _PINNED_FREE.append(host)
        else:
            keep.append((ev, host, what, exc))
    _DEFERRED[:] = keep
    if err is not None:
        raise err


def dev_split_triples(triples_plus, num_nodes, num_rels):
    t = triples_plus.contiguous()
    M, dev = t.shape[0], t.device
    s, p, o, err = _i32(M, dev), _i32(M, dev), _i32(M, dev), _i32(1, dev)
    with _on(dev):
        _check(lib().rgcn_dev_split_triples(_dp(t), c_i64(M), c_i64(num_nodes), c_i32(num_rels), _dp(s), _dp(p), _dp(o),
                                            _dp(err), _stream(dev)), "dev_split_triples")
    return s[:M], p[:M], o[:M], err


def dev_lp_expand(triples, num_nodes, num_rels0, keep):
    t = triples.contiguous()
    E, dev = t.shape[0], t.device
    M = 3 * E + num_nodes
    s, p, o, err = _i32(M, dev), _i32(M, dev), _i32(M, dev), _i32(1, dev)
    alive = torch.empty(M, dtype=torch.uint8, device=dev)
    k = None if keep is None else keep.to(torch.uint8).contiguous()
    with _on(dev):
        _check(lib().rgcn_dev_lp_expand(_dp(t), c_i64(E), c_i64(num_nodes), c_i32(num_rels0), _dp(k), _dp(s), _dp(p),
                                        _dp(o), _dp(alive), _dp(err), _stream(dev)), "dev_lp_expand")
    return s, p, o, alive, err


def dev_edge_norm(s, p, o, alive, num_nodes, num_rels, vertical, n_swap):
    M, dev = s.shape[0], s.device
    table = _i32(num_nodes * num_rels, dev)
    val = torch.empty(max(M, 1), dtype=torch.float32, device=dev)
    with _on(dev):
        _check(lib().rgcn_dev_edge_norm(_dp(s), _dp(p), _dp(o), _dp(alive), c_i64(M), c_i64(num_nodes), c_i32(num_rels),
                                        c_int(int(bool(vertical))), c_i64(n_swap), _dp(table), _dp(val), _stream(dev)),
               "dev_edge_norm")
    return val[:M]


class BuiltPlan:
    """Same fields as DevicePlan, produced on the device."""


def build_plan_device(dst, src, rel, val, alive, n_dst, n_src, num_rels, tile_rows, n_live, max_item_chunks=64,
                      want_runs=False, want_pack=False, max_unit_chunks=256, aux=None, sync_free=False):
    dev = dst.device
    M = dst.shape[0]
    n_tiles = (n_dst + tile_rows - 1) // tile_rows
    nbk = n_tiles * num_rels
    cells = _i32(nbk * tile_rows, dev)
    tall = tile_rows > 1024
    cells_tmp = _i32(nbk * tile_rows, dev) if tall else None
    bucket_cnt, bucket_base = _i32(nbk, dev), _i32(nbk + 1, dev)
    scan_tmp = _i32(max(nbk, nbk * tile_rows if tall else 0) // 1024 + 4, dev)
    L = lib()
    with _on(dev):
        _check(L.rgcn_dev_plan_count(_dp(dst), _dp(rel), _dp(alive), c_i64(M), c_i64(n_dst), c_i32(num_rels),
                                     c_i32(tile_rows), _dp(cells), _dp(bucket_cnt), _dp(bucket_base), _dp(scan_tmp),
                                     _dp(cells_tmp), _stream(dev)), "dev_plan_count")
    if sync_free:
        m_pad = (M + 15 * min(nbk, M) + CHUNK - 1) // CHUNK * CHUNK
    else:
        m_pad = int(bucket_base[nbk].item())
    p = BuiltPlan()
    p.device = dev
    p.n_dst, p.n_src, p.num_rels, p.tile_rows = n_dst, n_src, num_rels, tile_rows
    p.n_tiles, p.m_pad, p.n_chunks, p.n_messages = n_tiles, m_pad, m_pad // CHUNK, int(n_live)
    p.src, p.dst = _i32(m_pad, dev), _i32(m_pad, dev)
    p.val = torch.empty(max(m_pad, 1), dtype=torch.float32, device=dev)
    can_pack = want_pack and n_src < (1 << 24) and tile_rows <= 255
    p.pack = torch.empty((max(m_pad, 1), 2), dtype=torch.int32, device=dev) if can_pack else None
    p.chunk_rel = _i32(p.n_chunks, dev)
    p.tile_ptr = _i32(n_tiles + 1, dev)
    p.run_ptr = _i32(n_tiles * (num_rels + 1), dev) if want_runs else None
    p.aux = _i32(m_pad, dev) if aux is not None else None
    with _on(dev):
        _check(L.rgcn_dev_plan_fill(_dp(dst), _dp(src), _dp(rel), _dp(val), _dp(alive), c_i64(M), c_i64(n_dst),
                                    c_i64(n_src), c_i32(num_rels), c_i32(tile_rows), _dp(cells), _dp(bucket_cnt),
                                    _dp(bucket_base), _dp(p.src), _dp(p.dst), _dp(p.val), _dp(p.pack), _dp(p.chunk_rel),
                                    _dp(p.tile_ptr), _dp(p.run_ptr), _dp(aux), _dp(p.aux), None, c_i64(p.n_chunks),
                                    _stream(dev)), "dev_plan_fill")
    if sync_free:
        p.n_units, p.n_split, p.units_host = n_tiles, 0, None
        p.units = torch.empty((max(n_tiles, 1), 4), dtype=torch.int32, device=dev)
        p.max_run_chunks = 1 << 30
        if n_tiles == 1:
            p.n_items = p.n_chunks // max_item_chunks + num_rels
            p.items = torch.empty((max(p.n_items, 1), 2), dtype=torch.int32, device=dev)
        else:
            p.n_items, p.items = 0, None
        with _on(dev):
            _check(L.rgcn_dev_plan_finish_nosync(_dp(bucket_base), c_i64(n_tiles), c_i32(num_rels), c_i64(m_pad), _dp(p.src),
                                                 _dp(p.dst), _dp(p.val), _dp(p.pack), _dp(p.aux), _dp(p.tile_ptr), _dp(p.units),
                                                 _dp(p.items), c_i64(max(p.n_items, 1)), c_i32(max_item_chunks), _stream(dev)),
                   "dev_plan_finish_nosync")
        if p.items is None:
            p.items = _i32(2, dev).view(1, 2)
        return p
    tp_host = p.tile_ptr[:n_tiles + 1].cpu().numpy()
    nu, ns = c_i64(0), c_i64(0)
    _check(L.rgcn_plan_units_host(_hp(tp_host), c_i64(n_tiles), c_i32(max_unit_chunks), None, ctypes.byref(nu),
                                  ctypes.byref(ns)), "plan_units")
    units = np.zeros((max(nu.value, 1), 4), np.int32)
    _check(L.rgcn_plan_units_host(_hp(tp_host), c_i64(n_tiles), c_i32(max_unit_chunks), _hp(units), ctypes.byref(nu),
                                  ctypes.byref(ns)), "plan_units")
    p.n_units, p.n_split = nu.value, ns.value
    p.units_host = units
    p.units = torch.from_numpy(units).to(dev)
    p.max_run_chunks = int((int(bucket_cnt[:nbk].max().item()) + CHUNK - 1) // CHUNK) if nbk else 0
    if n_tiles == 1:
        base = (bucket_base[:nbk + 1].cpu().numpy() // CHUNK).astype(np.int64)
        items = [(c, min(c + max_item_chunks, base[r + 1])) for r in range(num_rels)
                 for c in range(base[r], base[r + 1], max_item_chunks)]
        p.n_items = len(items)
        p.items = torch.tensor(items if items else [[0, 0]], dtype=torch.int32, device=dev)
    else:
        p.n_items, p.items = 0, _i32(2, dev).view(1, 2)
    return p


def own_relations(counts, n_waves, per_wave):
    import heapq
    counts = np.asarray(counts, dtype=np.int64)
    R = len(counts)
    slots = n_waves * per_wave
    if R > slots:
        return None
    parts = np.ones(R, np.int64)
    target = max(1.0, float(counts.sum()) / n_waves)
    heap = [(-float(counts[r]), r) for r in range(R)]
    heapq.heapify(heap)
    units = R
    while units < slots and heap:
        size, r = heap[0]
        if -size <= 0.5 * target:
            break
        parts[r] += 1
        units += 1
        heapq.heapreplace(heap, (-float(counts[r]) / parts[r], r))
    unit_base = np.cumsum(parts) - parts
    U = int(parts.sum())
    usize = np.concatenate([np.full(parts[r], counts[r] / parts[r]) for r in range(R)]) if R else np.zeros(0)
    urel = np.repeat(np.arange(R), parts)
    load, used = [0.0] * n_waves, [0] * n_waves
    owner, local = np.zeros(U, np.int64), np.zeros(U, np.int64)
    unit_rel = np.full(slots, -1, np.int32)
    for u in sorted(range(U), key=lambda u: (-usize[u], u)):
        w = min((i for i in range(n_waves) if used[i] < per_wave), key=lambda i: (load[i], i))
        owner[u], local[u] = w, used[w]
        unit_rel[w * per_wave + used[w]] = urel[u]
        used[w] += 1
        load[w] += usize[u]
    mean = max(1.0, float(sum(load)) / n_waves)
    return parts, unit_base, owner, local, unit_rel, max(load) / mean


def build_softwin_plan_device(dst, src, rel, val, alive, n_dst, n_src, num_rels, tile_rows, own_waves=0, own_per_wave=0):
    dev = dst.device
    M = dst.shape[0]
    n_tiles = (n_dst + tile_rows - 1) // tile_rows
    nbk = n_tiles * num_rels
    n_groups = n_tiles * max(own_waves, 1)
    L = lib()
    tmp_bytes = int(L.rgcn_softwin_tmp_bytes(c_i64(max(M, nbk + 1, n_groups + 1, M // CHUNK + min(nbk, M) + 1))))
    tmp = torch.empty(tmp_bytes, dtype=torch.uint8, device=dev)
    keys = torch.empty(2 * max(M, 1), dtype=torch.int64, device=dev)
    order = torch.empty(2 * max(M, 1), dtype=torch.int32, device=dev)
    bucket_cnt, bucket_base, bucket_first = _i32(nbk + 1, dev), _i32(nbk + 1, dev), _i32(nbk + 1, dev)
    with _on(dev):
        _check(L.rgcn_softwin_order(_dp(dst), _dp(src), _dp(rel), _dp(alive), c_i64(M), c_i64(n_dst), c_i64(n_src), c_i32(num_rels), c_i32(tile_rows),
                                    _dp(keys[:max(M, 1)]), _dp(keys[max(M, 1):]), _dp(order[:max(M, 1)]), _dp(order[max(M, 1):]), _dp(bucket_cnt),
                                    _dp(bucket_base), _dp(bucket_first), _dp(tmp), c_i64(tmp_bytes), _stream(dev)), "softwin_order")
    rel_counts = bucket_cnt[:nbk].view(n_tiles, num_rels).sum(0, dtype=torch.int64)
    host = torch.cat([bucket_base[nbk:nbk + 1].long(), bucket_first[nbk:nbk + 1].long(), bucket_cnt[:nbk].max().view(1).long(), rel_counts]).cpu().numpy()
    m_pad, n_live, max_cnt = int(host[0]), int(host[1]), int(host[2])
    own = None
    if own_waves:
        own = own_relations(host[3:], own_waves, own_per_wave)
        if own is None:
            return None
    n_chunks = m_pad // CHUNK
    p = BuiltPlan()
    p.device = dev
    p.n_dst, p.n_src, p.num_rels, p.tile_rows = n_dst, n_src, num_rels, tile_rows
    p.n_tiles, p.m_pad, p.n_chunks, p.n_messages = n_tiles, m_pad, n_chunks, n_live
    p.src, p.dst = _i32(m_pad, dev), _i32(m_pad, dev)
    p.val = torch.empty(max(m_pad, 1), dtype=torch.float32, device=dev)
    p.chunk_rel = _i32(n_chunks, dev)
    group_ptr = _i32(n_groups + 1, dev)
    stage = _i32(2 * max(m_pad, 1), dev)
    stage_val = torch.empty(max(m_pad, 1), dtype=torch.float32, device=dev)
    ckeys = torch.empty(2 * max(n_chunks, 1), dtype=torch.int64, device=dev)
    cidx, crel, group_cnt = _i32(2 * max(n_chunks, 1), dev), _i32(n_chunks, dev), _i32(n_groups + 1, dev)
    tabs = [None] * 4
    if own is not None:
        tabs = [torch.from_numpy(np.ascontiguousarray(a, dtype=np.int32)).to(dev) for a in own[:4]]
    nc1, mp1 = max(n_chunks, 1), max(m_pad, 1)
    with _on(dev):
        _check(L.rgcn_softwin_fill(_dp(dst), _dp(src), _dp(val), _dp(keys[max(M, 1):]), _dp(order[max(M, 1):]), c_i64(n_live), c_i64(n_dst), c_i64(n_src),
                                   c_i32(num_rels), c_i32(tile_rows), _dp(bucket_base), _dp(bucket_first), c_i64(m_pad), _dp(tabs[0]), _dp(tabs[1]),
                                   _dp(tabs[2]), _dp(tabs[3]), c_i32(own_waves), _dp(stage[:mp1]), _dp(stage[mp1:]), _dp(stage_val), _dp(ckeys[:nc1]),
                                   _dp(ckeys[nc1:]), _dp(cidx[:nc1]), _dp(cidx[nc1:]), _dp(crel), _dp(group_cnt), _dp(p.src), _dp(p.dst), _dp(p.val),
                                   _dp(p.chunk_rel), _dp(group_ptr), _dp(tmp), c_i64(tmp_bytes), _stream(dev)), "softwin_fill")
    p.tile_ptr = group_ptr[::max(own_waves, 1)].contiguous()
    p.run_ptr = torch.zeros(n_tiles * (num_rels + 1), dtype=torch.int32, device=dev)
    p.run_ptr[0::num_rels + 1] = p.tile_ptr[:-1]
    p.run_ptr[num_rels::num_rels + 1] = p.tile_ptr[1:]
    if own is not None:
        p.own_ptr = group_ptr
        p.unit_rel = torch.from_numpy(own[4]).to(dev)
        p.own_waves, p.own_per_wave, p.own_balance = own_waves, own_per_wave, float(own[5])
    p.pack, p.aux = None, None
    p.soft_windows = True
    p.units_host = np.zeros((0, 4), np.int32)
    p.n_units, p.n_split, p.units = n_tiles, 0, None
    p.n_items, p.items = 0, _i32(2, dev).view(1, 2)
    p.max_run_chunks = (max_cnt + CHUNK - 1) // CHUNK
    return p


def build_softwin_plan(dst, src, rel, val, alive, n_dst, n_src, num_rels, tile_rows, own_waves=0, own_per_wave=0):
    dev = dst.device
    if dev.type == "cuda" and routes.get("softwin_build", "device") != "torch":
        return build_softwin_plan_device(dst, src, rel, val, alive, n_dst, n_src, num_rels, tile_rows, own_waves, own_per_wave)
    M = dst.shape[0]
    n_tiles = (n_dst + tile_rows - 1) // tile_rows
    nbk = n_tiles * num_rels
    live = None if alive is None else (alive != 0)
    d64, s64, r64 = dst.long(), src.long(), rel.long()
    bucket = torch.div(d64, tile_rows, rounding_mode="floor") * num_rels + r64
    key = bucket * n_src + s64
    if live is not None:
        key = torch.where(live, key, torch.full_like(key, nbk * n_src))
    perm = torch.argsort(key)
    n_live = M if live is None else int(live.sum().item())
    perm = perm[:n_live]
    bs = bucket[perm]
    cnt = torch.bincount(bs, minlength=nbk)
    padded = (cnt + (CHUNK - 1)) // CHUNK * CHUNK
    base = torch.cumsum(padded, 0) - padded
    first = torch.cumsum(cnt, 0) - cnt
    slot = base[bs] + (torch.arange(n_live, device=dev) - first[bs])
    m_pad = int(padded.sum().item())
    n_chunks = m_pad // CHUNK
    S = torch.zeros(max(m_pad, 1), dtype=torch.int32, device=dev)
    D = torch.full((max(m_pad, 1),), -1, dtype=torch.int32, device=dev)
    V = torch.zeros(max(m_pad, 1), dtype=torch.float32, device=dev)
    S[slot], D[slot], V[slot] = src[perm].to(torch.int32), dst[perm].to(torch.int32), val[perm]
    cb = torch.repeat_interleave(torch.arange(nbk, device=dev), padded // CHUNK, output_size=n_chunks)
    ctile = torch.div(cb, num_rels, rounding_mode="floor")
    own = None
    if own_waves:
        live_rel = r64 if live is None else r64[live]
        own = own_relations(torch.bincount(live_rel, minlength=num_rels).cpu().numpy(), own_waves, own_per_wave)
        if own is None:
            return None
        parts_t, ubase_t = torch.from_numpy(own[0]).to(dev), torch.from_numpy(own[1]).to(dev)
        owner_t, local_t = torch.from_numpy(own[2]).to(dev), torch.from_numpy(own[3]).to(dev)
        crel0 = cb % num_rels
        first_chunk = torch.cumsum(padded // CHUNK, 0) - padded // CHUNK
        cunit = ubase_t[crel0] + (torch.arange(n_chunks, device=dev) - first_chunk[cb]) % parts_t[crel0]
        cgroup = ctile * own_waves + owner_t[cunit]
    else:
        cgroup = ctile
    cperm = torch.argsort(cgroup * n_src + S[:m_pad:CHUNK].long())
    idx = (cperm[:, None] * CHUNK + torch.arange(CHUNK, device=dev)[None, :]).reshape(-1)
    p = BuiltPlan()
    p.device = dev
    p.n_dst, p.n_src, p.num_rels, p.tile_rows = n_dst, n_src, num_rels, tile_rows
    p.n_tiles, p.m_pad, p.n_chunks, p.n_messages = n_tiles, m_pad, n_chunks, n_live
    if m_pad:
        p.src, p.dst, p.val = S[idx].contiguous(), D[idx].contiguous(), V[idx].contiguous()
    else:
        p.src, p.dst, p.val = S, D, V
    crel = cb % num_rels
    if own is not None:
        crel = crel | (local_t[cunit] << 16)
        gcnt = torch.bincount(cgroup, minlength=n_tiles * own_waves)
        p.own_ptr = torch.cat([torch.zeros(1, dtype=torch.int64, device=dev), torch.cumsum(gcnt, 0)]).to(torch.int32)
        p.unit_rel = torch.from_numpy(own[4]).to(dev)
        p.own_waves, p.own_per_wave, p.own_balance = own_waves, own_per_wave, float(own[5])
    p.chunk_rel = crel[cperm].to(torch.int32).contiguous() if n_chunks else _i32(0, dev)
    tcnt = torch.bincount(ctile, minlength=n_tiles)
    tend = torch.cumsum(tcnt, 0)
    p.tile_ptr = torch.cat([torch.zeros(1, dtype=torch.int64, device=dev), tend]).to(torch.int32)
    p.run_ptr = torch.zeros(n_tiles * (num_rels + 1), dtype=torch.int32, device=dev)
    p.run_ptr[0::num_rels + 1] = (tend - tcnt).to(torch.int32)
    p.run_ptr[num_rels::num_rels + 1] = tend.to(torch.int32)
    p.pack, p.aux = None, None
    p.soft_windows = True
    p.units_host = np.zeros((0, 4), np.int32)
    p.n_units, p.n_split, p.units = n_tiles, 0, None
    p.n_items, p.items = 0, _i32(2, dev).view(1, 2)
    p.max_run_chunks = int(padded.max().item()) // CHUNK if nbk else 0
    return p


class CsrPlan:
    """destination-major CSR (rowptr, src, rel, val) built on the device: the layout of the basis kernels"""


def build_csr_device(dst, src, rel, val, alive, n_rows, sync_free=False, want_slot=True):
    dev = dst.device
    M = dst.shape[0]
    rowbuf = torch.zeros(n_rows + 2, dtype=torch.int32, device=dev)
    cells, cells_tmp = rowbuf[1:], _i32(n_rows + 1, dev)
    bucket_cnt, bucket_base, scan_tmp = _i32(1, dev), _i32(2, dev), _i32(n_rows // 1024 + 4, dev)
    L = lib()
    with _on(dev):
        _check(L.rgcn_dev_plan_count(_dp(dst), None, _dp(alive), c_i64(M), c_i64(n_rows), c_i32(1), c_i32(n_rows),
                                     _dp(cells), _dp(bucket_cnt), _dp(bucket_base), _dp(scan_tmp), _dp(cells_tmp),
                                     _stream(dev)), "dev_plan_count")
    m_pad = (M + CHUNK - 1) // CHUNK * CHUNK
    p = CsrPlan()
    p.n_rows = n_rows
    p.msg_slot = torch.full((max(M, 1),), -1, dtype=torch.int32, device=dev)[:M] if want_slot else None
    p.n_messages = None
    p.src, pdst, p.rel = _i32(m_pad, dev), _i32(m_pad, dev), _i32(m_pad, dev)
    p.val = torch.empty(max(m_pad, 1), dtype=torch.float32, device=dev)
    tile_ptr = _i32(2, dev)
    with _on(dev):
        _check(L.rgcn_dev_plan_fill(_dp(dst), _dp(src), None, _dp(val), _dp(alive), c_i64(M), c_i64(n_rows),
                                    c_i64(n_rows), c_i32(1), c_i32(n_rows), _dp(cells), _dp(bucket_cnt), _dp(bucket_base),
                                    _dp(p.src), _dp(pdst), _dp(p.val), None, None, _dp(tile_ptr), None,
                                    _dp(rel), _dp(p.rel), _dp(p.msg_slot), c_i64(m_pad // CHUNK), _stream(dev)),
               "dev_plan_fill")
    p.rowptr = rowbuf[: n_rows + 1]
    p.sync_free = sync_free
    p.units = None
    return p


def build_csr_pair_device(a, b, rel, val, alive, n_rows):
    dev = a.device
    M = a.shape[0]
    rowbuf = _i32(2 * n_rows + 2, dev)
    scan_tmp = _i32((2 * n_rows + 1) // 1024 + 4, dev)
    e_other, e_rel = _i32(2 * M, dev), _i32(2 * M, dev)
    e_val = torch.empty(max(2 * M, 1), dtype=torch.float32, device=dev)
    with _on(dev):
        _check(lib().rgcn_dev_csr_pair(_dp(a), _dp(b), _dp(rel), _dp(val), _dp(alive), c_i64(M), c_i64(n_rows), _dp(rowbuf),
                                       _dp(scan_tmp), _dp(e_other), _dp(e_rel), _dp(e_val), _stream(dev)), "dev_csr_pair")
    out = []
    for k in range(2):
        p = CsrPlan()
        p.n_rows = n_rows
        p.msg_slot, p.n_messages = None, None
        p.src, p.rel, p.val = e_other, e_rel, e_val
        p.rowptr = rowbuf[k * (n_rows + 1): k * (n_rows + 1) + n_rows + 1]
        p.sync_free, p.per_call, p.units = True, True, None
        out.append(p)
    return out[0], out[1]


def row_units(rowptr, n_rows, max_len):
    dev = rowptr.device
    rp = rowptr[: n_rows + 1].to(torch.int64)
    deg = rp[1:] - rp[:-1]
    pieces = torch.clamp((deg + max_len - 1) // max_len, min=1)
    n_units = int(pieces.sum().item())
    row = torch.repeat_interleave(torch.arange(n_rows, device=dev), pieces, output_size=n_units)
    first = torch.cumsum(pieces, 0) - pieces
    k = torch.arange(n_units, device=dev) - first[row]
    begin = rp[row] + k * max_len
    end = torch.minimum(begin + max_len, rp[row + 1])
    shared = pieces[row] > 1
    flags = shared.to(torch.int64) * 1 + (shared & (k == 0)).to(torch.int64) * 2
    units = torch.stack([row, begin, end, flags], dim=1).to(torch.int32).contiguous()
    return units, n_units, int(shared.sum().item())


class FBasisPlan:
    __slots__ = ("e_dst", "e_rel", "e_val", "n_messages", "units_src", "perm_dst", "units_dst", "perm_rel", "units_rel",
                 "n_nodes", "num_rels", "rowptr_src", "max_src_degree")


def build_fbasis_plan(csr_src, csr_dst, n_nodes, num_rels, max_len=1024):
    p = FBasisPlan()
    M = int(csr_src.rowptr[n_nodes].item())
    p.n_messages, p.n_nodes, p.num_rels = M, n_nodes, num_rels
    p.e_dst, p.e_rel, p.e_val = csr_src.src, csr_src.rel, csr_src.val
    p.rowptr_src = csr_src.rowptr
    rp = csr_src.rowptr[: n_nodes + 1]
    p.max_src_degree = int((rp[1:] - rp[:-1]).max().item()) if n_nodes > 0 else 0
    p.units_src = row_units(csr_src.rowptr, n_nodes, max_len)
    live = csr_src.msg_slot >= 0
    perm = torch.zeros(max(M, 1), dtype=torch.int32, device=csr_src.rowptr.device)
    perm[csr_dst.msg_slot[live].long()] = csr_src.msg_slot[live]
    p.perm_dst = perm
    p.units_dst = row_units(csr_dst.rowptr, n_nodes, max_len)
    rel = csr_src.rel[:M].long()
    p.perm_rel = torch.argsort(rel, stable=True).to(torch.int32)
    rel_ptr = torch.zeros(num_rels + 1, dtype=torch.int64, device=rel.device)
    rel_ptr[1:] = torch.cumsum(torch.bincount(rel, minlength=num_rels), 0)
    p.units_rel = row_units(rel_ptr, num_rels, int(min(2 * max_len, max(64, M // 16384))))
    return p


def fbasis_supported(B, d):
    if B < 4:
        return False
    dp = 4
    while dp < d and dp < 64:
        dp <<= 1
    ngrp = 64 // dp
    return d <= 16 and B <= 64 and 4 * ((B + 4 * ngrp - 1) // (4 * ngrp)) <= 16


def fbasis_fwd(table, comps, bias, plan, basis_major=False, relu=False):
    bases = table
    _req(bases, "bases"); _req(comps, "comps"); _req(bias, "bias")
    N, B, d = (bases.shape[1], bases.shape[0], bases.shape[2]) if basis_major else bases.shape
    dev = bases.device
    Y = torch.empty(max(plan.n_messages, 1), d, device=dev, dtype=torch.float32)
    out = torch.empty(N, d, device=dev, dtype=torch.float32)
    units, n_units, _ = plan.units_src
    with _on(dev), _timed("fbasis_fwd"):
        _check(lib().rgcn_fbasis_fwd_f32(_dp(bases), _dp(comps), _dp(Y), _dp(plan.e_rel), _dp(plan.e_val), _dp(units),
                                         c_i64(n_units), c_i64(N), c_i32(comps.shape[0]), c_i32(B), c_i32(d),
                                         c_i32(1 if basis_major else 0), _stream(dev)), "fbasis_fwd")
        units, n_units, n_split = plan.units_dst
        fused = bool(relu) and n_split == 0
        _check(lib().rgcn_gather_rows_sum_f32(_dp(Y), _dp(plan.perm_dst), _dp(units), c_i64(n_units), c_i64(n_split),
                                              _dp(bias), _dp(out), c_i64(N), c_i32(d), c_i32(1 if fused else 0), _stream(dev)), "gather_rows_sum")
    return (out, fused) if relu else out


def fbasis_bwd(table, comps, g, plan, need_bases=True, need_comps=True, basis_major=False):
    bases = table
    _req(bases, "bases"); _req(comps, "comps"); _req(g, "grad")
    N, B, d = (bases.shape[1], bases.shape[0], bases.shape[2]) if basis_major else bases.shape
    R = comps.shape[0]
    dev = bases.device
    dB = torch.empty_like(bases) if need_bases else None
    dC = torch.empty(R, B, device=dev, dtype=torch.float32) if need_comps else None
    units, n_units, n_split = plan.units_src
    if need_comps and not routes.flag("deterministic") and \
            lib().rgcn_fbasis_bwd_dc_supported(c_i32(R), c_i32(B), c_i32(d)):
        with _on(dev), _timed("fbasis_bwd"):
            _check(lib().rgcn_fbasis_bwd_dc_f32(_dp(bases), _dp(comps), _dp(g), _dp(dB), _dp(dC), _dp(plan.e_dst), _dp(plan.e_rel),
                                                _dp(plan.e_val), _dp(units), c_i64(n_units), c_i64(n_split), c_i64(N), c_i32(R),
                                                c_i32(B), c_i32(d), c_i32(1 if basis_major else 0), _stream(dev)), "fbasis_bwd_dc")
# ... 345 lines not shown
        live = dst >= 0
        inv = torch.zeros(max(n_msg, 1), dtype=torch.int32, device=dev)
        inv[aux[live].long()] = torch.arange(p.m_pad, device=dev, dtype=torch.int32)[live]
        p._inv = inv
    return p._inv


def _segment_gather_sum(Y, perm, csr, bias, out, relu):
    units, n_units, n_split = _csr_units(csr)
    if units is not None and n_split:
        _check(lib().rgcn_segment_gather_sum_units_f32(_dp(Y), _dp(perm), _dp(units), c_i64(n_units), c_i64(n_split), _dp(bias), _dp(out),
                                                       c_i64(csr.n_rows), c_i32(16), c_i32(0), _stream(Y.device)), "segment_gather_sum_units")
        return relu
    _check(lib().rgcn_segment_gather_sum_f32(_dp(Y), _dp(perm), _dp(csr.rowptr), _dp(bias), _dp(out), c_i64(csr.n_rows), c_i32(16),
                                             c_i32(F_RELU if relu else 0), _stream(Y.device)), "segment_gather_sum")
    return False


def spmm_two_pass(X, W, bias, scatter_plan, csr, relu=False):
    _req(X, "features"); _req(W, "weights"); _req(bias, "bias")
    Wp = pack_w16(W)
    p = scatter_plan
    n_msg = int(csr.rowptr[-1].item()) if csr.n_messages is None else csr.n_messages
    out = torch.empty((csr.n_rows, 16), device=X.device, dtype=torch.float32)
    gather = routes.get("twopass", "gather") == "gather"
    if gather:
        _slot_perm(p, n_msg, X.device)
        Y = torch.empty((max(p.dst.shape[0], 1), 16), device=X.device, dtype=torch.float32)
    else:
        Y = torch.empty((max(n_msg, 1), 16), device=X.device, dtype=torch.float32)
    with _on(X.device), _timed("spmm_scatter"):
        _check(lib().rgcn_spmm_scatter_f32(_dp(X), _dp(Wp), _dp(Y), _dp(p.src), _dp(p.val), None if gather else _dp(p.aux),
                                           _dp(p.chunk_rel), _dp(p.items), c_i64(p.n_items), c_i32(16), _stream(X.device)),
               "spmm_scatter")
    with _on(X.device), _timed("segment_sum"):
        if gather:
            relu = _segment_gather_sum(Y, p._inv, csr, bias, out, relu)
        else:
            _check(lib().rgcn_segment_sum_f32(_dp(Y), _dp(csr.rowptr), _dp(bias), _dp(out), c_i64(csr.n_rows), c_i32(16),
                                              c_i32(F_RELU if relu else 0), _stream(X.device)), "segment_sum")
            relu = False
    return out.relu_() if relu else out


def spmm_wide_two_pass(X, W, bias, scatter_plan, csr, relu=False):
    _req(X, "features"); _req(W, "weights"); _req(bias, "bias")
    p, dev = scatter_plan, X.device
    R, d_in, d_out = W.shape
    n_msg = int(csr.rowptr[-1].item()) if csr.n_messages is None else csr.n_messages
    perm = _slot_perm(p, n_msg, dev)
    Y = torch.empty((max(p.dst.shape[0], 1), d_out), device=dev, dtype=torch.float32)
    out = torch.empty((csr.n_rows, d_out), device=dev, dtype=torch.float32)
    with _on(dev), _timed("rel_rows"):
        _check(lib().rgcn_rel_rows_f32(_dp(X), _dp(W), _dp(Y), _dp(p.src), _dp(p.val), _dp(p.chunk_rel), _dp(p.items),
                                       c_i64(p.n_items), c_i32(R), c_i32(d_in), c_i32(d_out), _stream(dev)), "rel_rows")
    with _on(dev), _timed("segment_sum_wide"):
        _check(lib().rgcn_segment_gather_sum_wide_f32(_dp(Y), _dp(perm), _dp(csr.rowptr), _dp(bias), _dp(out), c_i64(csr.n_rows),
                                                      c_i32(d_out), c_i32(F_RELU if relu else 0), _stream(dev)),
               "segment_gather_sum_wide")
    return out


def wgrad_wide(X, G, scatter_plan, num_rels):
    _req(X, "features"); _req(G, "grad_output")
    p = scatter_plan
    dW = torch.empty((num_rels, X.shape[1], G.shape[1]), device=X.device, dtype=torch.float32)
    with _on(X.device), _timed("rel_wgrad"):
        _check(lib().rgcn_rel_wgrad_f32(_dp(X), _dp(G), _dp(dW), _dp(p.src), _dp(p.dst), _dp(p.val), _dp(p.chunk_rel),
                                        _dp(p.items), c_i64(p.n_items), c_i32(num_rels), c_i32(X.shape[1]), c_i32(G.shape[1]),
                                        _stream(X.device)), "rel_wgrad")
    return dW


def bwd_two_pass_fused(G, X, W, scatter_plan, csr, relu=False):
    _req(G, "grad_output"); _req(X, "features"); _req(W, "weights")
    p = scatter_plan
    dev = G.device
    Wtp = pack_w16t(W)
    n_msg = int(csr.rowptr[-1].item()) if csr.n_messages is None else csr.n_messages
    _slot_perm(p, n_msg, dev)
    Y = torch.empty((max(p.dst.shape[0], 1), 16), device=dev, dtype=torch.float32)
    dW = torch.empty_like(W)
    dX = torch.empty((csr.n_rows, 16), device=dev, dtype=torch.float32)
    with _on(dev), _timed("bwd_scatter_dw"):
        _check(lib().rgcn_bwd_scatter_dw_f32(_dp(G), _dp(X), _dp(Wtp), _dp(Y), _dp(dW), _dp(p.src), _dp(p.dst), _dp(p.val),
                                             _dp(p.chunk_rel), _dp(p.items), c_i64(p.n_items), c_i32(W.shape[0]), c_i32(16),
                                             c_i32(F_RELU if relu else 0), _stream(dev)), "bwd_scatter_dw")
    with _on(dev), _timed("segment_sum"):
        _segment_gather_sum(Y, p._inv, csr, None, dX, False)
    return dX, dW


def wgrad(X, G, plan, num_rels):
    _req(X, "features"); _req(G, "grad_output")
    d_in, d_out = X.shape[1], G.shape[1]
    assert X.shape[0] == plan.n_src and G.shape[0] == plan.n_dst
    dW = torch.empty((num_rels, d_in, d_out), device=X.device, dtype=torch.float32)
    with _on(X.device), _timed("wgrad"):
        _check(lib().rgcn_wgrad_f32(_dp(X), _dp(G), _dp(dW), _dp(plan.src), _dp(plan.dst), _dp(plan.val),
                                    _dp(plan.chunk_rel), _dp(plan.items), c_i64(plan.n_items), c_i64(plan.n_dst),
                                    c_i64(plan.n_src), c_i32(num_rels), c_i32(d_in), c_i32(d_out),
                                    _stream(X.device)), "wgrad")
    return dW


def wgrad_tiled(X, G, plan, num_rels, tiles_per_item=4):
    _req(X, "features"); _req(G, "grad_output")
    assert plan.run_ptr is not None and X.shape[0] == plan.n_src and G.shape[0] == plan.n_dst
    dW = torch.empty((num_rels, X.shape[1], G.shape[1]), device=X.device, dtype=torch.float32)
    with _on(X.device), _timed("wgrad"):
        _check(lib().rgcn_wgrad_tiled_f32(_dp(X), _dp(G), _dp(dW), _dp(plan.src), _dp(plan.dst), _dp(plan.val),
                                          _dp(plan.chunk_rel), _dp(plan.run_ptr), c_i64(plan.n_tiles),
                                          c_i32(plan.tile_rows), c_i64(plan.n_dst), c_i64(plan.n_src),
                                          c_i32(num_rels), c_i32(X.shape[1]), c_i32(G.shape[1]),
                                          c_i32(tiles_per_item), _stream(X.device)), "wgrad_tiled")
    return dW


F_DW_ATOMIC = 4
F_TRANSPOSE_W = 8


def pack_w16t(W):
    return _packed_w16(W)[1]


def bwd_route():
    return routes.get("bwd_kernel", "blk")


_BLK_MIN_NODES = 32768
_BLK_MIN_NODES_SPARSE = 4096


def bwd_blk_rows(n_nodes, num_rels, deterministic=False, device=None, diag4=False, sparse=False):
    if bwd_route() != "blk" or deterministic or n_nodes < (_BLK_MIN_NODES_SPARSE if sparse else _BLK_MIN_NODES):
        return 0
    cap = int(lib().rgcn_bwd_blk_max_rows(c_i32(num_rels), c_i32(F_DIAG4 if diag4 else 0)))
    cap = min(cap, int(routes.get("bwd_blk_cap", "512")))
    if cap < 64:
        return 0
    n_cu = torch.cuda.get_device_properties(device if device is not None else torch.cuda.current_device()).multi_processor_count
    per_cu = -(-n_nodes // (n_cu * cap))
    rows = -(-n_nodes // (n_cu * per_cu))
    return max(rows, min(cap, 128))


def poison_lds(device=None):
    dev = torch.device("cuda", torch.cuda.current_device()) if device is None else torch.device(device)
    with _on(dev):
        _check(lib().rgcn_poison_lds(_stream(dev)), "poison_lds")


def spmm_blk_rows(n_nodes, device=None):
    if n_nodes < _BLK_MIN_NODES or routes.get("spmm_csr", "1") == "0":
        return 0
    cap = min(1000, int(lib().rgcn_spmm_blk_max_rows()), int(routes.get("fwd_rows_cap", "1000")))
    n_cu = torch.cuda.get_device_properties(device if device is not None else torch.cuda.current_device()).multi_processor_count
    per_cu = -(-n_nodes // (n_cu * cap))
    return -(-n_nodes // (n_cu * per_cu))


def spmm_blk(X, W, bias, plan, relu=False):
    _req(X, "features"); _req(W, "weights"); _req(bias, "bias")
    assert W.shape[1:] == (16, 16) and X.shape == (plan.n_src, 16)
    dev = X.device
    Wp = pack_w16(W)
    out = torch.empty((plan.n_dst, 16), device=dev, dtype=torch.float32)
    rec = _blk_rec(plan)
    units, n_units, n_split = _blk_units(plan)
    if relu and n_split:
        raise NativeLibraryError("spmm_blk: relu in the epilogue needs a plan without hub pieces")
    with _on(dev), _timed("spmm_blk"):
        _check(lib().rgcn_spmm_blk_f32(_dp(X), _dp(Wp), _dp(bias), _dp(out), _dp(rec), _dp(plan.run_ptr), c_i64(plan.n_tiles),
                                       c_i32(plan.tile_rows), c_i64(plan.n_dst), c_i32(W.shape[0]), c_i32(F_RELU if relu else 0),
                                       _dp(units), c_i64(n_units), c_i64(n_split), _stream(dev)), "spmm_blk")
    return out


def spmm_bf16(X, W, bias, plan, relu=False):
    _req(X, "features", torch.bfloat16); _req(W, "weights"); _req(bias, "bias")
    R, d_in, d_out = W.shape
    assert X.shape == (plan.n_src, d_in) and R == plan.num_rels and plan.pack is not None
    Wp = pack_w16(W) if (d_in, d_out) == (16, 16) else pack_w_blocks(W)
    out = torch.empty((plan.n_dst, d_out), device=X.device, dtype=torch.bfloat16)
    scratch = torch.empty((plan.n_dst, d_out), device=X.device, dtype=torch.float32) if plan.n_split else None
    fused = relu and not plan.n_split
    with _on(X.device), _timed("spmm_bf16"):
        _check(lib().rgcn_spmm_bf16(_dp(X), _dp(Wp), _dp(bias), _dp(out), _dp(scratch), _dp(plan.pack), _dp(plan.chunk_rel), _dp(plan.units),
                                    c_i64(plan.n_units), c_i64(plan.n_split), c_i32(plan.tile_rows), c_i64(plan.n_dst), c_i64(plan.n_src),
                                    c_i32(d_in), c_i32(d_out), c_i32(F_RELU if fused else 0), _stream(X.device)), "spmm_bf16")
    return torch.relu_(out) if (relu and not fused) else out


def wgrad_bf16(X, G, plan, num_rels):
    _req(X, "features", torch.bfloat16); _req(G, "grad_output", torch.bfloat16)
    d_in, d_out = X.shape[1], G.shape[1]
    dW = torch.empty((num_rels, d_in, d_out), device=X.device, dtype=torch.float32)
    with _on(X.device), _timed("wgrad_bf16"):
        _check(lib().rgcn_wgrad_bf16(_dp(X), _dp(G), _dp(dW), _dp(plan.src), _dp(plan.dst), _dp(plan.val), _dp(plan.chunk_rel),
                                     _dp(plan.items), c_i64(plan.n_items), c_i32(num_rels), c_i32(d_in), c_i32(d_out),
                                     _stream(X.device)), "wgrad_bf16")
    return dW


def colsum_bf16(G):
    _req(G, "grad_output", torch.bfloat16)
    db = torch.empty(G.shape[1], device=G.device, dtype=torch.float32)
    scratch = torch.empty(int(lib().rgcn_colsum_scratch_floats(c_i64(G.shape[0]), c_i32(G.shape[1]))), device=G.device, dtype=torch.float32)
    with _on(G.device), _timed("colsum_bf16"):
        _check(lib().rgcn_colsum_bf16(_dp(G), _dp(db), _dp(scratch), c_i64(G.shape[0]), c_i32(G.shape[1]), _stream(G.device)), "colsum_bf16")
    return db


def spmm_blk_bf16(X, W, bias, plan, relu=False):
    _req(X, "features", torch.bfloat16); _req(W, "weights"); _req(bias, "bias")
    assert W.shape[1:] == (16, 16) and X.shape == (plan.n_src, 16)
    dev = X.device
    Wp = pack_w16(W)
    out = torch.empty((plan.n_dst, 16), device=dev, dtype=torch.bfloat16)
    rec = _blk_rec(plan)
    units, n_units, n_split = _blk_units(plan)
    if relu and n_split:
        raise NativeLibraryError("spmm_blk_bf16: relu in the epilogue needs a plan without hub pieces")
    scratch = torch.empty((plan.n_dst, 16), device=dev, dtype=torch.float32) if n_split else None
    with _on(dev), _timed("spmm_blk_bf16"):
        _check(lib().rgcn_spmm_blk_bf16(_dp(X), _dp(Wp), _dp(bias), _dp(out), _dp(scratch), _dp(rec), _dp(plan.run_ptr), c_i64(plan.n_tiles),
                                        c_i32(plan.tile_rows), c_i64(plan.n_dst), c_i64(plan.n_src), c_i32(W.shape[0]),
                                        c_i32(F_RELU if relu else 0), _dp(units), c_i64(n_units), c_i64(n_split), _stream(dev)), "spmm_blk_bf16")
    return out


def _bwd_blk_plan(plan, diag4=False):
    return (plan.tile_rows > 160 or (plan.tile_rows > 64 and bwd_route() == "blk")) and \
        bool(lib().rgcn_bwd_blk_supported(c_i32(plan.tile_rows), c_i32(plan.num_rels), c_i32(F_DIAG4 if diag4 else 0)))


def bwd_fused_ok(plan, diag4=False):
    if plan.run_ptr is None or plan.n_tiles <= 0 or plan.n_src >= (1 << 24):
        return False
    if _bwd_blk_plan(plan, diag4):
        return True
    return plan.pack is not None and plan.n_split == 0 and plan.n_units == plan.n_tiles and \
        bool(lib().rgcn_bwd_lean_supported(c_i32(plan.tile_rows))) and plan.num_rels < 65536


def _blk_units(plan):
    cached = getattr(plan, "_blk_units", None)
    if cached is None:
        if getattr(plan, "units_host", None) is None:
            cached = (None, plan.n_tiles, 0)
        else:
            mean = max(1, plan.n_chunks // max(plan.n_tiles, 1))
            cached = row_units(plan.tile_ptr, plan.n_tiles, max(256, 2 * mean))
            if cached[2] == 0:
                cached = (None, plan.n_tiles, 0)
        plan._blk_units = cached
    return cached


def _lean_plan(plan):
    lean = getattr(plan, "_lean", None)
    if lean is None:
        n_chunks = plan.chunk_rel.shape[0]
        dev = plan.chunk_rel.device
        slots = torch.empty(int(lib().rgcn_bwd_lean_slot_bytes(c_i64(n_chunks))) + 16, device=dev, dtype=torch.uint8)
        hdr = torch.empty(max(n_chunks, 1), device=dev, dtype=torch.int32)
        with _on(dev):
            if plan.pack is not None:
                _check(lib().rgcn_bwd_lean_prepare_f32(_dp(plan.pack), _dp(plan.chunk_rel), c_i64(n_chunks), _dp(slots), _dp(hdr), _stream(dev)),
                       "bwd_lean_prepare")
            else:
                _check(lib().rgcn_bwd_lean_prepare_unpacked_f32(_dp(plan.src), _dp(plan.dst), _dp(plan.val), c_i32(plan.tile_rows),
                                                                _dp(plan.chunk_rel), c_i64(n_chunks), _dp(slots), _dp(hdr), _stream(dev)),
                       "bwd_lean_prepare_unpacked")
        lean = plan._lean = (slots, hdr)
    return lean


def _blk_rec(plan):
    rec = getattr(plan, "_blk_rec", None)
    if rec is None:
        n_chunks = plan.chunk_rel.shape[0]
        dev = plan.chunk_rel.device
        rec = torch.empty(int(lib().rgcn_bwd_blk_rec_bytes(c_i64(n_chunks))) + 16, device=dev, dtype=torch.uint8)
        packed = plan.pack is not None and plan.tile_rows <= 255
        with _on(dev):
            _check(lib().rgcn_bwd_blk_prepare_f32(_dp(plan.pack) if packed else None, _dp(plan.src), _dp(plan.dst), _dp(plan.val),
                                                  c_i32(plan.tile_rows), _dp(plan.chunk_rel), c_i64(n_chunks), _dp(rec), _stream(dev)),
                   "bwd_blk_prepare")
        plan._blk_rec = rec
    return rec


def bwd_own_geometry():
    L = lib()
    nw = int(L.rgcn_bwd_own_waves())
    return nw, int(L.rgcn_bwd_own_units()) // nw, int(L.rgcn_bwd_own_max_rows())


def bwd_own_rows(n_nodes, device=None):
    if n_nodes < _BLK_MIN_NODES:
        return 0
    cap = min(bwd_own_geometry()[2], int(routes.get("own_rows_cap", "789")))
    n_cu = torch.cuda.get_device_properties(device if device is not None else torch.cuda.current_device()).multi_processor_count
    per_cu = -(-n_nodes // (n_cu * cap))
    return -(-n_nodes // (n_cu * per_cu))


def bwd_own(G, X, W, plan, relu=False, want_db=False):
    _req(G, "grad_output"); _req(X, "features"); _req(W, "weights")
    assert W.shape[1:] == (16, 16) and G.shape == (plan.n_src, 16) and X.shape == (plan.n_dst, 16) and W.shape[0] == plan.num_rels
    assert getattr(plan, "own_ptr", None) is not None, "bwd_own: a plan made with build_softwin_plan(own_waves=...)"
    dev = G.device
    Wtp = pack_w16t(W)
    dX = torch.empty((plan.n_dst, 16), device=dev, dtype=torch.float32)
    buf = torch.empty(W.numel() + 16, device=dev, dtype=torch.float32)
    dW, db = buf[:W.numel()].view_as(W), buf[W.numel():]
    rec = _blk_rec(plan)
    with _on(dev), _timed("bwd_fused"):
        _check(lib().rgcn_bwd_own_f32(_dp(G), _dp(X), _dp(Wtp), _dp(dX), _dp(dW), _dp(rec), _dp(plan.own_ptr), _dp(plan.unit_rel),
                                      c_i64(plan.n_tiles), c_i32(plan.tile_rows), c_i64(plan.n_dst), c_i32(W.shape[0]),
                                      c_i32(F_RELU if relu else 0), _dp(db) if want_db else None, c_i64(plan.n_src), _stream(dev)), "bwd_own")
    return (dX, dW, db if want_db else None)


def bwd_own_bf16(G, X, W, plan, relu=False, want_db=False):
    _req(G, "grad_output", torch.bfloat16); _req(X, "features", torch.bfloat16); _req(W, "weights")
    assert W.shape[1:] == (16, 16) and G.shape == (plan.n_src, 16) and X.shape == (plan.n_dst, 16) and W.shape[0] == plan.num_rels
    assert getattr(plan, "own_ptr", None) is not None, "bwd_own_bf16: a plan made with build_softwin_plan(own_waves=...)"
    dev = G.device
    Wtp = pack_w16t(W)
    dX = torch.empty((plan.n_dst, 16), device=dev, dtype=torch.bfloat16)
    buf = torch.empty(W.numel() + 16, device=dev, dtype=torch.float32)
    dW, db = buf[:W.numel()].view_as(W), buf[W.numel():]
    rec = _blk_rec(plan)
    with _on(dev), _timed("bwd_own_bf16"):
        _check(lib().rgcn_bwd_own_bf16(_dp(G), _dp(X), _dp(Wtp), _dp(dX), _dp(dW), _dp(rec), _dp(plan.own_ptr), _dp(plan.unit_rel),
                                       c_i64(plan.n_tiles), c_i32(plan.tile_rows), c_i64(plan.n_dst), c_i32(W.shape[0]),
                                       c_i32(F_RELU if relu else 0), _dp(db) if want_db else None, c_i64(plan.n_src), _stream(dev)), "bwd_own_bf16")
    return (dX, dW, db if want_db else None)


def bwd_fused_relu_ok(plan, diag4=False):
    return bool(_bwd_blk_plan(plan, diag4)) or bwd_fused_ok(plan, diag4)


def bwd_fused(G, X, W, plan, atomic=False, relu=False, want_db=False, diag4=False):
    _req(G, "grad_output"); _req(X, "features"); _req(W, "weights")
    assert W.shape[1:] == (16, 16) and G.shape == (plan.n_src, 16) and X.shape == (plan.n_dst, 16)
    dev = G.device
    Wtp = pack_w16t(W)
    dX = torch.empty((plan.n_dst, 16), device=dev, dtype=torch.float32)
    blk = _bwd_blk_plan(plan, diag4)
    if diag4 and not blk:
        raise NativeLibraryError("bwd_fused: diag4 needs the block-tile kernel (plan of tall tiles, non-deterministic mode)")
    db = None
    if blk and want_db:
        buf = torch.empty(W.numel() + 16, device=dev, dtype=torch.float32)
        dW, db = buf[:W.numel()].view_as(W), buf[W.numel():]
    else:
        dW = torch.empty_like(W)
    ret = (lambda: (dX, dW, db)) if want_db else (lambda: (dX, dW))
    scratch = None
    if not atomic:
        n = int(lib().rgcn_bwd_fused_scratch_floats(c_i64(plan.n_tiles), c_i32(W.shape[0])))
        scratch = torch.empty(n, device=dev, dtype=torch.float32)
    if blk:
        if not atomic:
            raise NativeLibraryError("bwd_fused: the block-tile plan (tall tiles) has no bit-reproducible kernel")
        rec = _blk_rec(plan)
        units, n_units, n_split = _blk_units(plan)
        with _on(dev), _timed("bwd_fused"):
            _check(lib().rgcn_bwd_blk_f32(_dp(G), _dp(X), _dp(Wtp), _dp(dX), _dp(dW), _dp(rec), _dp(plan.run_ptr),
                                          c_i64(plan.n_tiles), c_i32(plan.tile_rows), c_i64(plan.n_dst), c_i32(W.shape[0]),
                                          c_i32((F_RELU if relu else 0) | (F_DIAG4 if diag4 else 0)), _dp(db), c_i64(plan.n_src),
                                          _dp(units), c_i64(n_units), c_i64(n_split), _stream(dev)), "bwd_blk")
        return ret()
    if not (lib().rgcn_bwd_lean_supported(c_i32(plan.tile_rows)) and W.shape[0] < 65536):
        raise NativeLibraryError(f"bwd_fused: no fused kernel for wave-owned tiles of {plan.tile_rows} rows (bwd_fused_ok)")
    slots, hdr = _lean_plan(plan)
    with _on(dev), _timed("bwd_fused"):
        _check(lib().rgcn_bwd_lean_f32(_dp(G), _dp(X), _dp(Wtp), _dp(dX), _dp(dW), _dp(scratch), _dp(slots), _dp(hdr),
                                       _dp(plan.run_ptr), c_i64(plan.n_tiles), c_i32(plan.tile_rows), c_i64(plan.n_dst),
                                       c_i32(W.shape[0]), c_i32((F_DW_ATOMIC if atomic else 0) | (1 if relu else 0)),
                                       _stream(dev)), "bwd_lean")
    return ret()


def bwd_fused_slabs_ok(plan):
    return bool(_bwd_blk_plan(plan)) and _blk_units(plan)[2] == 0 and getattr(plan, "tile_ptr", None) is not None


def bwd_fused_slabs(G, X, W, plan, n_slabs, after_slab):
    _req(G, "grad_output"); _req(X, "features"); _req(W, "weights")
    assert W.shape[1:] == (16, 16) and bwd_fused_slabs_ok(plan)
    dev = G.device
    Wtp = pack_w16t(W)
    dX = torch.empty((plan.n_dst, 16), device=dev, dtype=torch.float32)
    buf = torch.empty(W.numel() + 16, device=dev, dtype=torch.float32)
    dW, db = buf[:W.numel()].view_as(W), buf[W.numel():]
    rec = _blk_rec(plan)
    tiles = getattr(plan, "_blk_tile_units", None)
    if tiles is None:
        tiles = plan._blk_tile_units = row_units(plan.tile_ptr, plan.n_tiles, 1 << 30)[0]
    cuts = sorted({(plan.n_tiles * k) // n_slabs for k in range(n_slabs + 1)})
    for i, (ta, tb) in enumerate(zip(cuts[:-1], cuts[1:])):
        with _on(dev), _timed("bwd_fused"):
            _check(lib().rgcn_bwd_blk_f32(_dp(G), _dp(X), _dp(Wtp), _dp(dX), _dp(dW), _dp(rec), _dp(plan.run_ptr),
                                          c_i64(plan.n_tiles), c_i32(plan.tile_rows), c_i64(plan.n_dst), c_i32(W.shape[0]),
                                          c_i32(F_PARTIAL if i == 0 else F_ACCUMULATE), _dp(db) if i == 0 else None, c_i64(plan.n_src),
                                          c_void_p(tiles.data_ptr() + 16 * ta), c_i64(tb - ta), c_i64(0), _stream(dev)), "bwd_blk")
        after_slab(dX, ta * plan.tile_rows, min(plan.n_dst, tb * plan.tile_rows))
    return dX, dW, db


def featureless_fwd(table, bias, plan):
    _req(table, "weights"); _req(bias, "bias")
    R, n_src, d = table.shape
    assert R == plan.num_rels and n_src == plan.n_src
    out = torch.empty((plan.n_dst, d), device=table.device, dtype=torch.float32)
    with _on(table.device), _timed("featureless_fwd"):
        _check(lib().rgcn_featureless_fwd_f32(_dp(table), _dp(bias), _dp(out), _dp(plan.src), _dp(plan.dst),
                                              _dp(plan.val), _dp(plan.chunk_rel), _dp(plan.units),
                                              c_i64(plan.n_units), c_i64(plan.n_split), c_i32(plan.tile_rows), c_i64(plan.n_dst),
                                              c_i64(n_src), c_i32(R), c_i32(d), _stream(table.device)),
               "featureless_fwd")
    return out


def featureless_csr_fwd(table, bias, csr, relu=False):
    _req(table, "weights"); _req(bias, "bias")
    R, n_src, d = table.shape
    units, n_units, n_split = _csr_units(csr)
    assert units is not None, "the CSR featureless kernels serve static graphs"
    out = torch.empty((csr.n_rows, d), device=table.device, dtype=torch.float32)
    fused = bool(relu) and n_split == 0
    with _on(table.device), _timed("featureless_csr_fwd"):
        _check(lib().rgcn_featureless_csr_fwd_f32(_dp(table), _dp(bias), _dp(out), _dp(units), c_i64(n_units), c_i64(n_split),
                                                  _dp(csr.src), _dp(csr.rel), _dp(csr.val), c_i64(csr.n_rows), c_i64(n_src),
                                                  c_i32(R), c_i32(d), c_i32(1 if fused else 0), _stream(table.device)), "featureless_csr_fwd")
    return (out, fused) if relu else out


def featureless_csr_wgrad(G, csr, num_rels, n_src):
    _req(G, "grad_output")
    d = G.shape[1]
    if getattr(csr, "n_entries", None) is None:
        csr.n_entries = int(csr.rowptr[-1].item())
    dT = torch.empty((num_rels, n_src, d), device=G.device, dtype=torch.float32)
    with _on(G.device), _timed("featureless_csr_wgrad"):
        _check(lib().rgcn_featureless_csr_wgrad_f32(_dp(G), _dp(dT), _dp(csr.rowptr), _dp(csr.src), _dp(csr.rel), _dp(csr.val),
                                                    c_i64(csr.n_entries), c_i64(csr.n_rows), c_i64(n_src), c_i32(num_rels), c_i32(d),
                                                    _stream(G.device)), "featureless_csr_wgrad")
    return dT


def _csr_units(csr):
    if getattr(csr, "sync_free", False) or getattr(csr, "per_call", False):
        return None, csr.n_rows, 0
    if routes.get("deterministic", "0") == "1":
        if getattr(csr, "units_whole", None) is None:
            csr.units_whole = row_units(csr.rowptr, csr.n_rows, 1 << 30)
        return csr.units_whole
    if getattr(csr, "units", None) is None:
        csr.units = row_units(csr.rowptr, csr.n_rows, 512)
    return csr.units


def _empty_csr_out(csr, width, bias, relu, device):
    out = torch.zeros((csr.n_rows, width), device=device, dtype=torch.float32)
    if bias is not None:
        out += bias
    return out.relu_() if relu else out


def block_supported(bi, bo):
    return bool(lib().rgcn_block_supported(c_i32(bi), c_i32(bo)))


def block_spmm(X, blocks, bias, csr, transposed=False, relu=False):
    _req(X, "features"); _req(blocks, "blocks"); _req(bias, "bias")
    Rb, nb, bi, bo = blocks.shape
    assert X.shape[1] == nb * (bo if transposed else bi)
    if csr.src.numel() == 0:
        return _empty_csr_out(csr, nb * (bi if transposed else bo), bias, relu, X.device)
    units, n_units, n_split = _csr_units(csr)
    fuse_relu = relu and n_split == 0
    out = torch.empty((csr.n_rows, nb * (bi if transposed else bo)), device=X.device, dtype=torch.float32)
    flags = (F_TRANSPOSE_W if transposed else 0) | (F_RELU if fuse_relu else 0)
    with _on(X.device), _timed("block_spmm"):
        _check(lib().rgcn_block_spmm_f32(_dp(X), _dp(blocks), _dp(bias), _dp(out), _dp(units), _dp(csr.rowptr), c_i64(n_units),
                                         c_i64(n_split), _dp(csr.src), _dp(csr.rel), _dp(csr.val), c_i64(csr.n_rows), c_i32(Rb),
                                         c_i32(nb), c_i32(bi), c_i32(bo), c_i32(flags), _stream(X.device)), "block_spmm")
    if relu and not fuse_relu:
        out.relu_()
    return out


def spmm_csr_d16_ok(csr, R):
    return not getattr(csr, "sync_free", False) and not getattr(csr, "per_call", False) and \
        bool(lib().rgcn_spmm_csr_d16_supported(c_i32(R)))


def spmm_csr_d16(X, W, bias, csr, relu=False):
    _req(X, "features"); _req(W, "weights"); _req(bias, "bias")
    assert X.shape[1] == 16 and tuple(W.shape[1:]) == (16, 16)
    num_rels = getattr(csr, "num_rels", None)
    assert num_rels is None or W.shape[0] == num_rels, f"weights of {W.shape[0]} relations on a graph of {num_rels}: the kernel indexes its LDS table by the entries' relation"
    if csr.src.numel() == 0:
        return _empty_csr_out(csr, 16, bias, relu, X.device)
    units, n_units, n_split = _csr_units(csr)
    fuse_relu = relu and n_split == 0
    out = torch.empty((csr.n_rows, 16), device=X.device, dtype=torch.float32)
    with _on(X.device), _timed("spmm_csr"):
        _check(lib().rgcn_spmm_csr_d16_f32(_dp(X), _dp(W), _dp(bias), _dp(out), _dp(units), c_i64(n_units), c_i64(n_split),
                                           _dp(csr.src), _dp(csr.rel), _dp(csr.val), c_i64(csr.n_rows), c_i32(W.shape[0]),
                                           c_i32(F_RELU if fuse_relu else 0), _stream(X.device)), "spmm_csr_d16")
    if relu and not fuse_relu:
        out.relu_()
    return out


def block_wgrad(X, G, scatter_plan, shape):
    _req(X, "features"); _req(G, "grad_output")
    p = scatter_plan
    Rb, nb, bi, bo = shape
    dB = torch.empty(shape, device=X.device, dtype=torch.float32)
    with _on(X.device), _timed("block_wgrad"):
        _check(lib().rgcn_block_wgrad_f32(_dp(X), _dp(G), _dp(dB), _dp(p.src), _dp(p.dst), _dp(p.val), _dp(p.chunk_rel),
                                          _dp(p.items), c_i64(p.n_items), c_i32(Rb), c_i32(nb), c_i32(bi), c_i32(bo),
                                          _stream(X.device)), "block_wgrad")
    return dB


def diag_spmm(X, w, bias, csr):
    _req(X, "features"); _req(w, "weights"); _req(bias, "bias")
    R, d = w.shape
    assert X.shape[1] == d
    units, n_units, n_split = _csr_units(csr)
    assert units is not None, "the diagonal layer is not part of the sync-free LP step"
    out = torch.empty((csr.n_rows, d), device=X.device, dtype=torch.float32)
    with _on(X.device), _timed("diag_spmm"):
        _check(lib().rgcn_diag_spmm_f32(_dp(X), _dp(w), _dp(bias), _dp(out), _dp(units), c_i64(n_units), c_i64(n_split),
                                        _dp(csr.src), _dp(csr.rel), _dp(csr.val), c_i64(csr.n_rows), c_i32(R), c_i32(d),
                                        _stream(X.device)), "diag_spmm")
    return out


def diag_wgrad(X, G, scatter_plan, num_rels):
    _req(X, "features"); _req(G, "grad_output")
    p, d = scatter_plan, X.shape[1]
    dw = torch.empty((num_rels, d), device=X.device, dtype=torch.float32)
    with _on(X.device), _timed("diag_wgrad"):
        _check(lib().rgcn_diag_wgrad_f32(_dp(X), _dp(G), _dp(dw), _dp(p.src), _dp(p.dst), _dp(p.val), _dp(p.chunk_rel),
                                         _dp(p.items), c_i64(p.n_items), c_i32(num_rels), c_i32(d), _stream(X.device)),
               "diag_wgrad")
    return dw


def featureless_wgrad(G, plan, num_rels):
    _req(G, "grad_output")
    d = G.shape[1]
    dT = torch.empty((num_rels, plan.n_src, d), device=G.device, dtype=torch.float32)
    with _on(G.device), _timed("featureless_wgrad"):
        _check(lib().rgcn_featureless_wgrad_f32(_dp(G), _dp(dT), _dp(plan.src), _dp(plan.dst), _dp(plan.val),
                                                _dp(plan.chunk_rel), c_i64(plan.n_chunks), c_i64(plan.n_dst),
                                                c_i64(plan.n_src), c_i32(num_rels), c_i32(d), _stream(G.device)),
               "featureless_wgrad")
    return dT


def colsum(G):
    _req(G, "grad_output")
    db = torch.empty(G.shape[1], device=G.device, dtype=torch.float32)
    scratch = torch.empty(int(lib().rgcn_colsum_scratch_floats(c_i64(G.shape[0]), c_i32(G.shape[1]))), device=G.device,
                          dtype=torch.float32)
    with _on(G.device), _timed("colsum"):
        _check(lib().rgcn_colsum_f32(_dp(G), _dp(db), _dp(scratch), c_i64(G.shape[0]), c_i32(G.shape[1]),
                                     _stream(G.device)), "colsum")
    return db


def resize3(src, shape, src1=None, n1d=None):
    _req(src, "tensor"); _req(src1, "vector")
    s3 = src if src.dim() == 3 else src.unsqueeze(0)
    A, B, C = s3.shape
    Bd, Cd = shape[-2], shape[-1]
    dst = torch.empty((A, Bd, Cd) if src.dim() == 3 else (Bd, Cd), device=src.device, dtype=torch.float32)
    dst1 = None if src1 is None else torch.empty(n1d, device=src.device, dtype=torch.float32)
    with _on(src.device):
        _check(lib().rgcn_resize3_f32(_dp(s3), _dp(dst), c_i64(A), c_i32(B), c_i32(C), c_i32(Bd), c_i32(Cd), _dp(src1), _dp(dst1),
                                      c_i32(0 if src1 is None else src1.numel()), c_i32(0 if src1 is None else n1d), _stream(src.device)),
               "resize3")
    return dst if src1 is None else (dst, dst1)


def ce_head(logits, row_label, lab_rows):
    _req(row_label, "row_label", torch.int32); _req(lab_rows, "lab_rows", torch.int32)
    assert logits.dtype == torch.float32 and logits.is_cuda and logits.dim() == 2 and logits.stride(1) == 1 and logits.data_ptr() % 16 == 0
    N, C = logits.shape
    ld = logits.stride(0) if N > 1 else C
    loss = torch.empty(1, device=logits.device, dtype=torch.float32)
    full = torch.empty((N, ld), device=logits.device, dtype=torch.float32)
    with _on(logits.device), _timed("ce_head"):
        _check(lib().rgcn_ce_head_f32(_dp(logits), _dp(row_label), _dp(lab_rows), _dp(loss), _dp(full), c_i64(N), c_i32(C), c_i32(ld),
                                      c_i32(lab_rows.shape[0]), _stream(logits.device)), "ce_head")
    return (loss, full, None) if ld == C else (loss, full[:, :C], full)


_BCE_WS = {}


def bce_head(scores, labels):
    _req(scores, "scores"); _req(labels, "labels")
    assert scores.dim() == 1 and labels.shape == scores.shape
    dev = scores.device
    if scores.shape[0] == 0:
        return torch.full((1,), float("nan"), device=dev, dtype=torch.float32), torch.empty_like(scores)
    key = (dev, torch.cuda.current_stream(dev).cuda_stream)
    ws = _BCE_WS.get(key)
    if ws is None:
        ws = _BCE_WS[key] = torch.zeros(int(lib().rgcn_bce_head_workspace_bytes()), dtype=torch.uint8, device=dev)
    loss = torch.empty(1, device=dev, dtype=torch.float32)
    ds = torch.empty_like(scores)
    with _on(dev), _timed("bce_head"):
        _check(lib().rgcn_bce_head_f32(_dp(scores), _dp(labels), _dp(loss), _dp(ds), _dp(ws), c_i64(scores.shape[0]), _stream(dev)), "bce_head")
    return loss, ds


def distmult_fwd(triples, nodes, rel, sbias, pbias, obias, ranks=False):
    _req(nodes, "nodes"); _req(rel, "relations"); _req(triples, "triples", torch.int64)
    for b, n in ((sbias, "sbias"), (pbias, "pbias"), (obias, "obias")):
        _req(b, n)
    T = triples.shape[0]
    scores = torch.empty(T, device=nodes.device, dtype=torch.float32)
    err = _i32(1, nodes.device)
    counts = rk = None
    if ranks and T:
        counts, rk = _i32(2 * nodes.shape[0] + 3, nodes.device), _i32(2 * T, nodes.device)
    with _on(nodes.device), _timed("distmult_fwd"):
        _check(lib().rgcn_distmult_fwd_f32(_dp(triples), c_i64(T), _dp(nodes), _dp(rel), _dp(sbias), _dp(pbias),
                                           _dp(obias), _dp(scores), c_i64(nodes.shape[0]), c_i32(rel.shape[0]),
                                           c_i32(nodes.shape[1]), _dp(err), _dp(counts), _dp(rk), _stream(nodes.device)),
# ... 110 lines not shown
```

Baseline: 6.632 billion edges/s.

## Replace bwd_own dW atomics with per-block partials and reduction; alternate tile traversal direction

In the owner backward kernel, each block now writes its dW and dbias partial sums to a workspace, and a second reduction kernel sums them. This removes the global atomics and the memsets that zeroed dW beforehand. Both the forward block kernel and the backward owner kernel now walk chunks in reverse order on every other tile, presumably to reuse recently cached rows across the tile boundary. The unit-partitioning planner gains an LPT-based refinement pass to balance wave loads, and the default row cap changes. These gains cost an extra kernel launch and a workspace allocation on each call.

```diff
diff --git a/include/rgcn_hip.h b/include/rgcn_hip.h
--- a/include/rgcn_hip.h
+++ b/include/rgcn_hip.h
@@ -150,15 +150,16 @@
 RGCN_API int rgcn_bwd_blk_f32(const float *G, const float *X, const float *Wt_packed, float *dX, float *dW, const void *rec,
                               const int32_t *run_ptr, int64_t n_tiles, int32_t tile_rows, int64_t n_dst, int32_t R, int32_t flags,
                               float *dbias, int64_t n_src, const int32_t *units, int64_t n_units, int64_t n_split, void *stream);
+RGCN_API int64_t rgcn_bwd_own_workspace_bytes(int64_t n_tiles);
 RGCN_API int32_t rgcn_bwd_own_waves(void);
 RGCN_API int32_t rgcn_bwd_own_units(void);
 RGCN_API int32_t rgcn_bwd_own_max_rows(void);
 RGCN_API int rgcn_bwd_own_f32(const float *G, const float *X, const float *Wt_packed, float *dX, float *dW, const void *rec,
                               const int32_t *own_ptr, const int32_t *unit_rel, int64_t n_tiles, int32_t tile_rows, int64_t n_dst,
-                              int32_t R, int32_t flags, float *dbias, int64_t n_src, void *stream);
+                              int32_t R, int32_t flags, float *dbias, int64_t n_src, void *workspace, void *stream);
 RGCN_API int rgcn_bwd_own_bf16(const uint16_t *G, const uint16_t *X, const float *Wt_packed, uint16_t *dX, float *dW, const void *rec,
                                const int32_t *own_ptr, const int32_t *unit_rel, int64_t n_tiles, int32_t tile_rows, int64_t n_dst,
-                               int32_t R, int32_t flags, float *dbias, int64_t n_src, void *stream);
+                               int32_t R, int32_t flags, float *dbias, int64_t n_src, void *workspace, void *stream);
 RGCN_API int64_t rgcn_softwin_tmp_bytes(int64_t n);
 RGCN_API int rgcn_softwin_order(const int32_t *dst, const int32_t *src, const int32_t *rel, const uint8_t *alive, int64_t M, int64_t n_dst,
                                 int64_t n_src, int32_t R, int32_t tile_rows, uint64_t *keys, uint64_t *keys_sorted, int32_t *order,
diff --git a/torch-rgcn_amd/csrc/rgcn_bwd_blk.hip b/torch-rgcn_amd/csrc/rgcn_bwd_blk.hip
--- a/torch-rgcn_amd/csrc/rgcn_bwd_blk.hip
+++ b/torch-rgcn_amd/csrc/rgcn_bwd_blk.hip
@@ -389,6 +389,9 @@
 }
 
 
+#ifndef RGCN_FWD_REVERSE
+#define RGCN_FWD_REVERSE 1
+#endif
 template <bool RELU, int TQ, int BF = 0>
 __global__ __launch_bounds__(64 * BLK_FWD_NW) void spmm_blk_d16_kernel(
     const float *__restrict__ X, const float *__restrict__ Wp, const float *__restrict__ bias, float *__restrict__ out,
@@ -441,12 +444,14 @@
     }
   };
   int q_cur = wave * ns, q_nxt = 1 < ns ? wave * ns + 1 : NW * ns + wave, q_pos = 2;
+  int rev = 0;
+  auto quad_chunk = [&](int q, int c0_, int nq_, int rev_) { return c0_ + (rev_ ? nq_ - 1 - q : q) * U; };
   if (q_cur < nq) request_idx(c0 + q_cur * U, c1 - 1);
 
   for (;;) {
     const int last = c1 - 1;
     while (q_cur < nq) {
-      const int c = c0 + q_cur * U;
+      const int c = quad_chunk(q_cur, c0, nq, rev);
       unsigned w0_[U];
       uint2 rw_[U];
       float v_[U];
@@ -473,7 +478,7 @@
         w_[j] = *reinterpret_cast<const float4 *>(reinterpret_cast<const char *>(Wp) + (size_t)hd_[j] * 1024 + w_lane);
       }
       __builtin_amdgcn_sched_barrier(0);
-      if (q_nxt < nq) request_idx(c0 + q_nxt * U, last);
+      if (q_nxt < nq) request_idx(quad_chunk(q_nxt, c0, nq, rev), last);
       int q_nn = q_pos < ns ? wave * ns + q_pos : NW * ns + wave;
       if (q_pos > ns && lane == 0) q_nn = __hip_atomic_fetch_add(ctl, 1, __ATOMIC_RELAXED, __HIP_MEMORY_SCOPE_WORKGROUP);
       ++q_pos;
@@ -506,6 +511,7 @@
     }
     const int unn = un + (int)gridDim.x;
     int c0n = 0, c1n = 0, nqn = 0, row0n = 0, nrn = 0, flagsn = 0, nsn = 1;
+    const int revn = RGCN_FWD_REVERSE ? rev ^ 1 : 0;
     if (unn < n_units) {
       const int4 unx = unit_of(unn);
       row0n = __builtin_amdgcn_readfirstlane(unx.x) * tile_rows;
@@ -515,7 +521,7 @@
       flagsn = __builtin_amdgcn_readfirstlane(unx.w);
       nqn = (c1n - c0n + U - 1) / U;
       nsn = static_quads(nqn);
-      if (wave * nsn < nqn) request_idx(c0n + wave * nsn * U, c1n - 1);
+      if (wave * nsn < nqn) request_idx(quad_chunk(wave * nsn, c0n, nqn, revn), c1n - 1);
     }
     lds_barrier();
 #pragma unroll
@@ -555,7 +561,7 @@
     if (tid == 0) ctl[0] = NW * (nsn + 1);
     lds_barrier();
     un = unn; row0 = row0n; nrows = nrn; c0 = c0n; c1 = c1n; nq = nqn; uflags = flagsn;
-    ns = nsn;
+    ns = nsn; rev = revn;
     q_cur = wave * ns; q_nxt = 1 < ns ? wave * ns + 1 : NW * ns + wave; q_pos = 2;
   }
 }
diff --git a/torch-rgcn_amd/csrc/rgcn_bwd_own.hip b/torch-rgcn_amd/csrc/rgcn_bwd_own.hip
--- a/torch-rgcn_amd/csrc/rgcn_bwd_own.hip
+++ b/torch-rgcn_amd/csrc/rgcn_bwd_own.hip
@@ -16,9 +16,14 @@
 #define RGCN_OWN_K 8
 #define RGCN_OWN_U 2
 #endif
+#ifndef RGCN_OWN_REVERSE
+#define RGCN_OWN_REVERSE 1
+#endif
 constexpr int OWN_NW = RGCN_OWN_NW;
 constexpr int OWN_K = RGCN_OWN_K;
 constexpr int OWN_U = RGCN_OWN_U;
+constexpr int OWN_UNITS = OWN_NW * OWN_K;
+constexpr int OWN_PART = OWN_UNITS * 256;
 constexpr int OWN_MAX_ROWS = (OWN_LDS_MAX - OWN_NW * BW_SCR2 * 4 - 64) / 192;
 
 typedef float own_acc32 __attribute__((ext_vector_type(32)));
@@ -28,8 +33,8 @@
 template <bool RELU, int NW, int K, int ABL = 0, bool BF = false>
 __global__ __launch_bounds__(64 * NW) void bwd_own_d16_kernel(
     const float *__restrict__ G, const float *__restrict__ X, const float *__restrict__ Wtp, float *__restrict__ dX,
-    float *__restrict__ dWout, const char *__restrict__ rec, const int *__restrict__ own_ptr, int n_tiles, int tile_rows, int n_dst,
-    float *__restrict__ dbias, int n_src, const int *__restrict__ unit_rel) {
+    float *__restrict__ part, const char *__restrict__ rec, const int *__restrict__ own_ptr, int n_tiles, int tile_rows, int n_dst,
+    float *__restrict__ part_db, int n_src, const int *__restrict__ unit_rel) {
   constexpr int U = OWN_U, NT = 64 * NW;
   constexpr int TQ = (OWN_MAX_ROWS * 4 + NT - 1) / NT;
   static_assert(K <= 9, "8 indexed accumulators + 1");
@@ -51,7 +56,7 @@
   c0 = __builtin_amdgcn_readfirstlane(c0);
   c1 = __builtin_amdgcn_readfirstlane(c1);
   float4 gs = make_float4(0.f, 0.f, 0.f, 0.f);
-  const long long g_n4 = dbias ? (long long)n_src * 4 : 0, g_step = (long long)gridDim.x * NT;
+  const long long g_n4 = part_db ? (long long)n_src * 4 : 0, g_step = (long long)gridDim.x * NT;
   long long g_i = (long long)blockIdx.x * NT + tid;
 #pragma unroll
   for (int q = 0; q < TQ; ++q) {
@@ -96,10 +101,13 @@
     }
   };
   if (c0 < c1) request_idx(c0, c1 - 1);
+  int rev = 0;
 
   for (;;) {
     const int last = c1 - 1;
-    for (int c = c0; c < c1; c += U) {
+    const int ntr = (c1 - c0 + U - 1) / U, cstep = rev ? -U : U;
+    int c = rev ? c0 + (ntr - 1) * U : c0;
+    for (int i = 0; i < ntr; ++i, c += cstep) {
       unsigned w0_[U];
       uint2 rw_[U];
       float v_[U];
@@ -126,7 +134,7 @@
         w_[j] = *reinterpret_cast<const float4 *>(reinterpret_cast<const char *>(Wtp) + (size_t)(hd_[j] & 0xFFFF) * 1024 + w_lane);
       }
       __builtin_amdgcn_sched_barrier(0);
-      if (c + U < c1) request_idx(c + U, last);
+      if (i + 1 < ntr) request_idx(c + cstep, last);
       __builtin_amdgcn_sched_barrier(0);
       if (ABL & 16) {
 #pragma unroll
@@ -199,6 +207,7 @@
     }
     const int tn = t + (int)gridDim.x;
     int c0n = 0, c1n = 0, row0n = 0, nrn = 0;
+    const int revn = RGCN_OWN_REVERSE ? rev ^ 1 : 0;
     float4 xn[TQ];
 #pragma unroll
     for (int q = 0; q < TQ; ++q) xn[q] = make_float4(0.f, 0.f, 0.f, 0.f);
@@ -217,7 +226,7 @@
             xn[q] = reinterpret_cast<const float4 *>(X + (size_t)row0n * 16)[tid + q * NT];
           }
         }
-      if (c0n < c1n) request_idx(c0n, c1n - 1);
+      if (c0n < c1n) request_idx(revn ? c0n + (c1n - c0n - 1) / U * U : c0n, c1n - 1);
     }
     float4 gn = make_float4(0.f, 0.f, 0.f, 0.f);
     if (g_i < g_n4) {
@@ -255,9 +264,10 @@
       }
     }
     lds_barrier();
-    t = tn; row0 = row0n; nrows = nrn; c0 = c0n; c1 = c1n;
-  }
-  if (dbias) {
+    t = tn; row0 = row0n; nrows = nrn; c0 = c0n; c1 = c1n; rev = revn;
+  }
+  if (ABL & 32) return;
+  if (part_db) {
     for (; g_i < g_n4; g_i += g_step) {
       float4 gn;
       if constexpr (BF) gn = bf16x4_widen(reinterpret_cast<const uint2 *>(G)[g_i]);
@@ -275,20 +285,109 @@
       float a = 0.f;
       const float *all = reinterpret_cast<const float *>(lds + xs_off);
       for (int i = 0; i < NW; ++i) a += all[i * BW_SCR2 + tid];
-      atomicAdd(dbias + tid, a);
-    }
-  }
+      part_db[(size_t)blockIdx.x * 16 + tid] = a;
+    }
+  }
+  float4 *po = reinterpret_cast<float4 *>(part + (size_t)blockIdx.x * (NW * K * 256) + (size_t)(wave * K) * 256) + lane;
 #pragma unroll
   for (int li = 0; li < K; ++li) {
     const int r = __builtin_amdgcn_readfirstlane(unit_rel[wave * K + li]);
-    if (r >= 0) {
-      float *o = dWout + (size_t)r * 256 + (4 * k) * 16 + m;
-      atomicAdd(o, li < 8 ? accs[(4 * li) & 31] : acc8[0]);
-      atomicAdd(o + 16, li < 8 ? accs[(4 * li + 1) & 31] : acc8[1]);
-      atomicAdd(o + 32, li < 8 ? accs[(4 * li + 2) & 31] : acc8[2]);
-      atomicAdd(o + 48, li < 8 ? accs[(4 * li + 3) & 31] : acc8[3]);
-    }
-  }
+    if (r >= 0)
+      po[li * 64] = li < 8 ? make_float4(accs[(4 * li) & 31], accs[(4 * li + 1) & 31], accs[(4 * li + 2) & 31], accs[(4 * li + 3) & 31])
+                           : make_float4(acc8[0], acc8[1], acc8[2], acc8[3]);
+  }
+}
+
+constexpr int OWN_RED_G = 64;
+template <int NU>
+__global__ __launch_bounds__(16 * OWN_RED_G) void bwd_own_reduce_kernel(const float *__restrict__ part, const float *__restrict__ part_db,
+                                                                       const int *__restrict__ unit_rel, int n_blocks, int R,
+                                                                       float *__restrict__ dW, float *__restrict__ db) {
+  __shared__ float4 red[OWN_RED_G][16];
+  const int tid = threadIdx.x, f = tid & 15, g = tid >> 4;
+  const int r = (int)blockIdx.x >> 2, quarter = (int)blockIdx.x & 3;
+  float4 s = make_float4(0.f, 0.f, 0.f, 0.f);
+  if (r < R) {
+    const float4 *p4 = reinterpret_cast<const float4 *>(part) + quarter * 16 + f;
+    for (int u = 0; u < NU; ++u) {
+      if (unit_rel[u] != r) continue;
+#pragma unroll 4
+      for (int b = g; b < n_blocks; b += OWN_RED_G) {
+        const float4 v = p4[((size_t)b * NU + u) * 64];
+        s.x += v.x; s.y += v.y; s.z += v.z; s.w += v.w;
+      }
+    }
+  } else {
+    for (int b = g; b < n_blocks; b += OWN_RED_G) s.x += part_db[(size_t)b * 16 + f];
+  }
+  red[g][f] = s;
+  __syncthreads();
+#pragma unroll
+  for (int h = OWN_RED_G / 2; h > 0; h >>= 1) {
+    if (g < h) {
+      const float4 a = red[g][f], b = red[g + h][f];
+      red[g][f] = make_float4(a.x + b.x, a.y + b.y, a.z + b.z, a.w + b.w);
+    }
+    __syncthreads();
+  }
+  if (g == 0) {
+    const float4 a = red[0][f];
+    if (r < R) {
+      const int ln = quarter * 16 + f;
+      float *o = dW + (size_t)r * 256 + (4 * (ln >> 4)) * 16 + (ln & 15);
+      o[0] = a.x; o[16] = a.y; o[32] = a.z; o[48] = a.w;
+    } else {
+      db[f] = a.x;
+    }
+  }
+}
+
+#ifdef RGCN_ABLATIONS
+constexpr int OWN_MAX_DEV = 64, OWN_N_KERN = 3 + 7;
+#else
+constexpr int OWN_MAX_DEV = 64, OWN_N_KERN = 3;
+#endif
+struct OwnDev { int n_cu; bool raised[OWN_N_KERN]; };
+OwnDev own_dev_tab[OWN_MAX_DEV];
+
+hipError_t own_dev(OwnDev **out) {
+  int dev = 0;
+  hipError_t e = hipGetDevice(&dev);
+  if (e != hipSuccess) return e;
+  if (dev < 0 || dev >= OWN_MAX_DEV) return hipErrorInvalidDevice;
+  OwnDev *d = &own_dev_tab[dev];
+  if (!d->n_cu) {
+    int v = 0;
+    e = hipDeviceGetAttribute(&v, hipDeviceAttributeMultiprocessorCount, dev);
+    if (e != hipSuccess) return e;
+    d->n_cu = v > 0 ? v : 256;
+  }
+  *out = d;
+  return hipSuccess;
+}
+
+size_t own_ws_floats(unsigned n_blocks) { return (size_t)n_blocks * (OWN_PART + 16); }
+
+template <typename KernT>
+hipError_t own_launch(KernT kern, int slot, OwnDev *d, hipStream_t st, const float *G, const float *X, const float *Wt_packed, float *dX, float *dW,
+                      const void *rec, const int32_t *own_ptr, const int32_t *unit_rel, int64_t n_tiles, int32_t tile_rows, int64_t n_dst, int32_t R,
+                      float *dbias, int64_t n_src, void *workspace, bool reduce = true) {
+  const size_t lds = bwd_own_lds(tile_rows);
+  const unsigned n_blocks = (unsigned)std::min<int64_t>(n_tiles, d->n_cu);
+  float *part = static_cast<float *>(workspace);
+  float *part_db = dbias ? part + (size_t)n_blocks * OWN_PART : nullptr;
+  if (lds > 64 * 1024 && !d->raised[slot]) {
+    hipError_t e = hipFuncSetAttribute(reinterpret_cast<const void *>(kern), hipFuncAttributeMaxDynamicSharedMemorySize, OWN_LDS_MAX);
+    if (e != hipSuccess) return e;
+    d->raised[slot] = true;
+  }
+  hipLaunchKernelGGL(kern, dim3(n_blocks), dim3(64 * OWN_NW), lds, st, G, X, Wt_packed, dX, part, static_cast<const char *>(rec), own_ptr, (int)n_tiles,
+                     tile_rows, (int)n_dst, part_db, (int)n_src, unit_rel);
+  hipError_t e = hipGetLastError();
+  if (e != hipSuccess || !reduce) return e;
+  hipLaunchKernelGGL(bwd_own_reduce_kernel<OWN_UNITS>, dim3(4u * (unsigned)R + (dbias ? 1u : 0u)), dim3(16 * OWN_RED_G), 0, st, part, part_db, unit_rel,
+                     (int)n_blocks, R, dW, dbias);
+  return hipGetLastError();
 }
 
 }
@@ -297,69 +396,57 @@
 extern "C" int32_t rgcn_bwd_own_units(void) { return OWN_NW * OWN_K; }
 extern "C" int32_t rgcn_bwd_own_max_rows(void) { return OWN_MAX_ROWS; }
 
+extern "C" int64_t rgcn_bwd_own_workspace_bytes(int64_t n_tiles) {
+  OwnDev *d = nullptr;
+  if (n_tiles <= 0 || own_dev(&d) != hipSuccess) return -1;
+  return (int64_t)(own_ws_floats((unsigned)std::min<int64_t>(n_tiles, d->n_cu)) * sizeof(float));
+}
+
 extern "C" int rgcn_bwd_own_f32(const float *G, const float *X, const float *Wt_packed, float *dX, float *dW, const void *rec,
                                 const int32_t *own_ptr, const int32_t *unit_rel, int64_t n_tiles, int32_t tile_rows, int64_t n_dst,
-                                int32_t R, int32_t flags, float *dbias, int64_t n_src, void *stream) {
-  if (!G || !X || !Wt_packed || !dX || !dW || !rec || !own_ptr || !unit_rel || n_tiles <= 0 || tile_rows <= 0 || n_dst <= 0 || R <= 0 ||
-      R > 0xFFFF || n_dst > INT32_MAX || n_tiles * (int64_t)OWN_NW >= INT32_MAX) {
+                                int32_t R, int32_t flags, float *dbias, int64_t n_src, void *workspace, void *stream) {
+  if (!G || !X || !Wt_packed || !dX || !dW || !rec || !own_ptr || !unit_rel || !workspace || n_tiles <= 0 || tile_rows <= 0 || n_dst <= 0 ||
+      R <= 0 || R > 0xFFFF || n_dst > INT32_MAX || n_tiles * (int64_t)OWN_NW >= INT32_MAX) {
     rgcn_set_error("bwd_own: bad argument");
+    return RGCN_EINVAL;
+  }
+  if (n_src <= 0 || n_src >= (int64_t(1) << 26)) {
+    rgcn_set_error("bwd_own: 0 < n_src < 2^26 (the records address G rows as src << 6 in 32 bits)");
     return RGCN_EINVAL;
   }
   if (tile_rows > rgcn_bwd_own_max_rows()) {
     rgcn_set_error("bwd_own: tiles of at most %d rows (got %d)", rgcn_bwd_own_max_rows(), tile_rows);
     return RGCN_EUNSUPPORTED;
   }
-  if (dbias && (n_src <= 0 || n_src >= (int64_t(1) << 29))) { rgcn_set_error("bwd_own: dbias needs 0 < n_src < 2^29"); return RGCN_EINVAL; }
   hipStream_t st = (hipStream_t)stream;
-  static int n_cu = 0;
-  if (!n_cu) {
-    int dev = 0, v = 0;
-    HIP_TRY(hipGetDevice(&dev));
-    HIP_TRY(hipDeviceGetAttribute(&v, hipDeviceAttributeMultiprocessorCount, dev));
-    n_cu = v > 0 ? v : 256;
-  }
-  if (dbias == dW + (size_t)R * 256) {
-    HIP_TRY(zero_async(dW, ((size_t)R * 256 + 16) * sizeof(float), st));
-  } else {
-    HIP_TRY(zero_async(dW, (size_t)R * 256 * sizeof(float), st));
-    if (dbias) HIP_TRY(zero_async(dbias, 16 * sizeof(float), st));
-  }
-  const size_t lds = bwd_own_lds(tile_rows);
-  const unsigned n_blocks = (unsigned)std::min<int64_t>(n_tiles, n_cu);
-  auto launch = [&](auto kern, bool &raised) -> hipError_t {
-    if (lds > 64 * 1024 && !raised) {
-      hipError_t e = hipFuncSetAttribute(reinterpret_cast<const void *>(kern), hipFuncAttributeMaxDynamicSharedMemorySize, OWN_LDS_MAX);
-      if (e != hipSuccess) return e;
-      raised = true;
-    }
-    hipLaunchKernelGGL(kern, dim3(n_blocks), dim3(64 * OWN_NW), lds, st, G, X, Wt_packed, dX, dW, static_cast<const char *>(rec), own_ptr, (int)n_tiles,
-                       tile_rows, (int)n_dst, dbias, (int)n_src, unit_rel);
-    return hipGetLastError();
-  };
+  OwnDev *d = nullptr;
+  HIP_TRY(own_dev(&d));
+#define OWN_ARGS d, st, G, X, Wt_packed, dX, dW, rec, own_ptr, unit_rel, n_tiles, tile_rows, n_dst, R, dbias, n_src, workspace
 #ifdef RGCN_ABLATIONS
   {
     const int ABLV = rgcn_option_value(RGCN_OPT_BWD_ABL);
-    static bool a[8] = {false, false, false, false, false, false, false, false};
-    if (ABLV == 2) HIP_TRY(launch(bwd_own_d16_kernel<false, OWN_NW, OWN_K, 2>, a[1]));
-    else if (ABLV == 4) HIP_TRY(launch(bwd_own_d16_kernel<false, OWN_NW, OWN_K, 4>, a[3]));
-    else if (ABLV == 8) HIP_TRY(launch(bwd_own_d16_kernel<false, OWN_NW, OWN_K, 8>, a[4]));
-    else if (ABLV == 16) HIP_TRY(launch(bwd_own_d16_kernel<false, OWN_NW, OWN_K, 16>, a[5]));
-    else if (ABLV == 6) HIP_TRY(launch(bwd_own_d16_kernel<false, OWN_NW, OWN_K, 6>, a[6]));
-    else HIP_TRY(launch(bwd_own_d16_kernel<false, OWN_NW, OWN_K, 0>, a[7]));
+    if (ABLV == 2) HIP_TRY(own_launch(bwd_own_d16_kernel<false, OWN_NW, OWN_K, 2>, 3, OWN_ARGS));
+    else if (ABLV == 4) HIP_TRY(own_launch(bwd_own_d16_kernel<false, OWN_NW, OWN_K, 4>, 4, OWN_ARGS));
+    else if (ABLV == 8) HIP_TRY(own_launch(bwd_own_d16_kernel<false, OWN_NW, OWN_K, 8>, 5, OWN_ARGS));
+    else if (ABLV == 16) HIP_TRY(own_launch(bwd_own_d16_kernel<false, OWN_NW, OWN_K, 16>, 6, OWN_ARGS));
+    else if (ABLV == 6) HIP_TRY(own_launch(bwd_own_d16_kernel<false, OWN_NW, OWN_K, 6>, 7, OWN_ARGS));
+    else if (ABLV == 32) HIP_TRY(own_launch(bwd_own_d16_kernel<false, OWN_NW, OWN_K, 32>, 8, OWN_ARGS, false));
+    else HIP_TRY(own_launch(bwd_own_d16_kernel<false, OWN_NW, OWN_K, 0>, 9, OWN_ARGS));
     return RGCN_OK;
   }
 #endif
-  static bool r0 = false, r1 = false;
-  if (flags & RGCN_F_RELU) HIP_TRY(launch(bwd_own_d16_kernel<true, OWN_NW, OWN_K>, r0));
-  else HIP_TRY(launch(bwd_own_d16_kernel<false, OWN_NW, OWN_K>, r1));
+  if (flags & RGCN_F_RELU) HIP_TRY(own_launch(bwd_own_d16_kernel<true, OWN_NW, OWN_K>, 0, OWN_ARGS));
+  else HIP_TRY(own_launch(bwd_own_d16_kernel<false, OWN_NW, OWN_K>, 1, OWN_ARGS));
+#undef OWN_ARGS
   return RGCN_OK;
 }
 
 extern "C" int rgcn_bwd_own_bf16(const uint16_t *G, const uint16_t *X, const float *Wt_packed, uint16_t *dX, float *dW, const void *rec,
                                  const int32_t *own_ptr, const int32_t *unit_rel, int64_t n_tiles, int32_t tile_rows, int64_t n_dst,
-                                 int32_t R, int32_t flags, float *dbias, int64_t n_src, void *stream) {
-  if (!G || !X || !Wt_packed || !dX || !dW || !rec || !own_ptr || !unit_rel || n_tiles <= 0 || tile_rows <= 0 || n_dst <= 0 || R <= 0 ||
-      R > 0xFFFF || n_dst > INT32_MAX || n_tiles * (int64_t)OWN_NW >= INT32_MAX || n_src <= 0 || n_src >= (int64_t(1) << 26) || flags != 0) {
+                                 int32_t R, int32_t flags, float *dbias, int64_t n_src, void *workspace, void *stream) {
+  if (!G || !X || !Wt_packed || !dX || !dW || !rec || !own_ptr || !unit_rel || !workspace || n_tiles <= 0 || tile_rows <= 0 || n_dst <= 0 ||
+      R <= 0 || R > 0xFFFF || n_dst > INT32_MAX || n_tiles * (int64_t)OWN_NW >= INT32_MAX || n_src <= 0 || n_src >= (int64_t(1) << 26) ||
+      flags != 0) {
     rgcn_set_error("bwd_own_bf16: bad argument (the records address G rows as src << 6 in 32 bits: n_src < 2^26; no flags)");
     return RGCN_EINVAL;
   }
@@ -367,34 +454,10 @@
     rgcn_set_error("bwd_own_bf16: tiles of at most %d rows (got %d)", rgcn_bwd_own_max_rows(), tile_rows);
     return RGCN_EUNSUPPORTED;
   }
-  hipStream_t st = (hipStream_t)stream;
-  static int n_cu = 0;
-  if (!n_cu) {
-    int dev = 0, v = 0;
-    HIP_TRY(hipGetDevice(&dev));
-    HIP_TRY(hipDeviceGetAttribute(&v, hipDeviceAttributeMultiprocessorCount, dev));
-    n_cu = v > 0 ? v : 256;
-  }
-  if (dbias == dW + (size_t)R * 256) {
-    HIP_TRY(zero_async(dW, ((size_t)R * 256 + 16) * sizeof(float), st));
-  } else {
-    HIP_TRY(zero_async(dW, (size_t)R * 256 * sizeof(float), st));
-    if (dbias) HIP_TRY(zero_async(dbias, 16 * sizeof(float), st));
-  }
-  const size_t lds = bwd_own_lds(tile_rows);
-  const unsigned n_blocks = (unsigned)std::min<int64_t>(n_tiles, n_cu);
-  auto launch = [&](auto kern, bool &raised) -> hipError_t {
-    if (lds > 64 * 1024 && !raised) {
-      hipError_t e = hipFuncSetAttribute(reinterpret_cast<const void *>(kern), hipFuncAttributeMaxDynamicSharedMemorySize, OWN_LDS_MAX);
-      if (e != hipSuccess) return e;
-      raised = true;
-    }
-    hipLaunchKernelGGL(kern, dim3(n_blocks), dim3(64 * OWN_NW), lds, st, reinterpret_cast<const float *>(G), reinterpret_cast<const float *>(X),
-                       Wt_packed, reinterpret_cast<float *>(dX), dW, static_cast<const char *>(rec), own_ptr, (int)n_tiles, tile_rows, (int)n_dst,
-                       dbias, (int)n_src, unit_rel);
-    return hipGetLastError();
-  };
-  static bool r1 = false;
-  HIP_TRY(launch(bwd_own_d16_kernel<false, OWN_NW, OWN_K, 0, true>, r1));
+  OwnDev *d = nullptr;
+  HIP_TRY(own_dev(&d));
+  HIP_TRY(own_launch(bwd_own_d16_kernel<false, OWN_NW, OWN_K, 0, true>, 2, d, (hipStream_t)stream, reinterpret_cast<const float *>(G),
+                     reinterpret_cast<const float *>(X), Wt_packed, reinterpret_cast<float *>(dX), dW, rec, own_ptr, unit_rel, n_tiles, tile_rows,
+                     n_dst, R, dbias, n_src, workspace));
   return RGCN_OK;
 }
diff --git a/torch-rgcn_amd/torch_rgcn/_native.py b/torch-rgcn_amd/torch_rgcn/_native.py
--- a/torch-rgcn_amd/torch_rgcn/_native.py
+++ b/torch-rgcn_amd/torch_rgcn/_native.py
@@ -37,6 +37,7 @@
         L.rgcn_colsum_scratch_floats.restype = ctypes.c_int64
         L.rgcn_gemm_scratch_floats.restype = ctypes.c_int64
         L.rgcn_basis_sum_workspace_bytes.restype = ctypes.c_int64
+        L.rgcn_bwd_own_workspace_bytes.restype = ctypes.c_int64
         L.rgcn_last_error.restype = ctypes.c_char_p
         _lib = L
         defaults = {}
@@ -432,6 +433,49 @@
     return p
 
 
+_OWN_REFINE_ABOVE = 1.04
+_OWN_REFINE_GOAL = 1.005
+_OWN_REFINE_RELS = 12
+
+
+def _own_lpt_loads(counts, parts, n_waves, per_wave):
+    import heapq
+    units = sorted((-float(counts[r]) / int(parts[r]) for r in range(len(counts)) for _ in range(int(parts[r]))))
+    load, used = [0.0] * n_waves, [0] * n_waves
+    heap = [(0.0, i) for i in range(n_waves)]
+    for neg in units:
+        _, w = heapq.heappop(heap)
+        load[w] -= neg
+        used[w] += 1
+        if used[w] < per_wave:
+            heapq.heappush(heap, (load[w], w))
+    mean = max(1.0, sum(load) / n_waves)
+    return max(load) / mean, sum((x - mean) ** 2 for x in load)
+
+
+def _own_refine(counts, parts, n_waves, per_wave):
+    slots = n_waves * per_wave
+    parts = parts.copy()
+    cand = sorted(range(len(counts)), key=lambda r: (-int(counts[r]), r))[:_OWN_REFINE_RELS]
+    cur = _own_lpt_loads(counts, parts, n_waves, per_wave)
+    while cur[0] > _OWN_REFINE_GOAL:
+        best = None
+        for r in cand:
+            was = int(parts[r])
+            for q in range(2, 9):
+                if q == was or int(parts.sum()) - was + q > slots:
+                    continue
+                parts[r] = q
+                s = _own_lpt_loads(counts, parts, n_waves, per_wave)
+                if best is None or (round(s[0], 3), s[1]) < (round(best[0][0], 3), best[0][1]):
+                    best = (s, r, q)
+            parts[r] = was
+        if best is None or (round(best[0][0], 3), best[0][1]) >= (round(cur[0], 3), cur[1]):
+            break
+        cur, parts[best[1]] = best[0], best[2]
+    return parts
+
+
 def own_relations(counts, n_waves, per_wave):
     import heapq
     counts = np.asarray(counts, dtype=np.int64)
@@ -451,6 +495,8 @@
         parts[r] += 1
         units += 1
         heapq.heapreplace(heap, (-float(counts[r]) / parts[r], r))
+    if R and _own_lpt_loads(counts, parts, n_waves, per_wave)[0] > _OWN_REFINE_ABOVE:
+        parts = _own_refine(counts, parts, n_waves, per_wave)
     unit_base = np.cumsum(parts) - parts
     U = int(parts.sum())
     usize = np.concatenate([np.full(parts[r], counts[r] / parts[r]) for r in range(R)]) if R else np.zeros(0)
@@ -1402,27 +1448,38 @@
 def bwd_own_rows(n_nodes, device=None):
     if n_nodes < _BLK_MIN_NODES:
         return 0
-    cap = min(bwd_own_geometry()[2], int(routes.get("own_rows_cap", "789")))
+    cap = min(bwd_own_geometry()[2], int(routes.get("own_rows_cap", "767")))
     n_cu = torch.cuda.get_device_properties(device if device is not None else torch.cuda.current_device()).multi_processor_count
     per_cu = -(-n_nodes // (n_cu * cap))
     return -(-n_nodes // (n_cu * per_cu))
+
+
+def _bwd_own_workspace(plan, dev):
+    with _on(dev):
+        need = int(lib().rgcn_bwd_own_workspace_bytes(c_i64(plan.n_tiles)))
+    if need <= 0:
+        raise NativeLibraryError("rgcn_bwd_own_workspace_bytes failed")
+    return torch.empty(need, dtype=torch.uint8, device=dev)
 
 
 def bwd_own(G, X, W, plan, relu=False, want_db=False):
     _req(G, "grad_output"); _req(X, "features"); _req(W, "weights")
     assert W.shape[1:] == (16, 16) and G.shape == (plan.n_src, 16) and X.shape == (plan.n_dst, 16) and W.shape[0] == plan.num_rels
     assert getattr(plan, "own_ptr", None) is not None, "bwd_own: a plan made with build_softwin_plan(own_waves=...)"
+    assert plan.n_src < 1 << 26, "bwd_own: the records address G rows as src << 6 in 32 bits"
     dev = G.device
     Wtp = pack_w16t(W)
     dX = torch.empty((plan.n_dst, 16), device=dev, dtype=torch.float32)
-    buf = torch.empty(W.numel() + 16, device=dev, dtype=torch.float32)
-    dW, db = buf[:W.numel()].view_as(W), buf[W.numel():]
+    dW = torch.empty_like(W, memory_format=torch.contiguous_format)
+    db = torch.empty(16, device=dev, dtype=torch.float32) if want_db else None
+    ws = _bwd_own_workspace(plan, dev)
     rec = _blk_rec(plan)
     with _on(dev), _timed("bwd_fused"):
         _check(lib().rgcn_bwd_own_f32(_dp(G), _dp(X), _dp(Wtp), _dp(dX), _dp(dW), _dp(rec), _dp(plan.own_ptr), _dp(plan.unit_rel),
                                       c_i64(plan.n_tiles), c_i32(plan.tile_rows), c_i64(plan.n_dst), c_i32(W.shape[0]),
-                                      c_i32(F_RELU if relu else 0), _dp(db) if want_db else None, c_i64(plan.n_src), _stream(dev)), "bwd_own")
-    return (dX, dW, db if want_db else None)
+                                      c_i32(F_RELU if relu else 0), _dp(db) if want_db else None, c_i64(plan.n_src), _dp(ws), _stream(dev)),
+               "bwd_own")
+    return (dX, dW, db)
 
 
 def bwd_own_bf16(G, X, W, plan, relu=False, want_db=False):
@@ -1432,14 +1489,16 @@
     dev = G.device
     Wtp = pack_w16t(W)
     dX = torch.empty((plan.n_dst, 16), device=dev, dtype=torch.bfloat16)
-    buf = torch.empty(W.numel() + 16, device=dev, dtype=torch.float32)
-    dW, db = buf[:W.numel()].view_as(W), buf[W.numel():]
+    dW = torch.empty_like(W, memory_format=torch.contiguous_format)
+    db = torch.empty(16, device=dev, dtype=torch.float32) if want_db else None
+    ws = _bwd_own_workspace(plan, dev)
     rec = _blk_rec(plan)
     with _on(dev), _timed("bwd_own_bf16"):
         _check(lib().rgcn_bwd_own_bf16(_dp(G), _dp(X), _dp(Wtp), _dp(dX), _dp(dW), _dp(rec), _dp(plan.own_ptr), _dp(plan.unit_rel),
                                        c_i64(plan.n_tiles), c_i32(plan.tile_rows), c_i64(plan.n_dst), c_i32(W.shape[0]),
-                                       c_i32(F_RELU if relu else 0), _dp(db) if want_db else None, c_i64(plan.n_src), _stream(dev)), "bwd_own_bf16")
-    return (dX, dW, db if want_db else None)
+                                       c_i32(F_RELU if relu else 0), _dp(db) if want_db else None, c_i64(plan.n_src), _dp(ws), _stream(dev)),
+               "bwd_own_bf16")
+    return (dX, dW, db)
 
 
 def bwd_fused_relu_ok(plan, diag4=False):
```

After: 6.569 billion edges/s. About the same (-1.0%).
